# lidq92/LBDRN-MSIC

Measured on AMD Instinct MI355X. Metric: Mpixels/s encode+decode (and bpp/PSNR parity) on D2/K5/bc64/nl2, higher is better.
Workload: dtype f32; 1 GPU; synthetic 8-band 2048x2048 uint16 tile per step, K=5 D=2 bc=64 nl=2 bs=8192 e=10 (BASELINE.json configs[1] by default); encode fit + 16-bit weight truncation + decode; tiles_per_gpu=50, tiles_in_flight_per_gpu=4, tiles_per_launch=2, parallelism=image-sharded x1

## Files before the change

### include/lbdrn_hip.h

```cpp
#ifndef LBDRN_HIP_H
#define LBDRN_HIP_H

#include <stddef.h>
#include <stdint.h>

#ifdef __cplusplus
extern "C" {
#endif
#if defined(__GNUC__)
#pragma GCC visibility push(default)
#endif

#define LBDRN_ABI_VERSION 2

typedef enum lbdrn_status {
    LBDRN_OK = 0,
    LBDRN_E_ARG = -1,
    LBDRN_E_DEVICE = -2,
    LBDRN_E_UNSUPPORTED = -3,
    LBDRN_E_WORKSPACE = -4
} lbdrn_status;

typedef struct lbdrn_geom {
    int32_t C, H, W;
    int32_t K;
    int32_t D;
    int32_t msb_max;
    int32_t use_colors;
    int32_t relative;
    int32_t P;
    int32_t reserved;
    const float *rowtab;
    const float *coltab;
} lbdrn_geom;

typedef struct lbdrn_net {
    int32_t F, bc, C, nl;
    int32_t act;
} lbdrn_net;
enum { LBDRN_ACT_SINE = 0, LBDRN_ACT_RELU = 1 };

const char *lbdrn_last_error(void);
int lbdrn_abi_version(void);
int lbdrn_device_check(void);
int64_t lbdrn_param_count(const lbdrn_net *net);
int32_t lbdrn_feature_dim(const lbdrn_geom *g);

int lbdrn_split_bits(const uint16_t *img, int32_t C, int32_t H, int32_t W, int32_t K,
                     uint16_t *msb, int32_t *msb_max, void *stream);

int lbdrn_labels(const uint16_t *img, int32_t C, int32_t H, int32_t W, int32_t K,
                 const int64_t *idx, int64_t n, float *labels, void *stream);

int lbdrn_features(const lbdrn_geom *g, const uint16_t *msb, const int64_t *idx, int64_t n,
                   float *features, void *stream);

size_t lbdrn_forward_workspace(const lbdrn_net *net, int64_t B);
int lbdrn_forward(const lbdrn_net *net, const float *params, const float *x, int64_t B, float *y,
                  void *workspace, size_t workspace_bytes, void *stream);

size_t lbdrn_tape_bytes(const lbdrn_net *net, int64_t B);
int lbdrn_forward_tape(const lbdrn_net *net, const float *params, const float *x, int64_t B, float *y,
                       void *tape, size_t tape_bytes, void *stream);
size_t lbdrn_backward_workspace(const lbdrn_net *net, int64_t B);
int lbdrn_backward(const lbdrn_net *net, const float *params, const float *x, int64_t B, const void *tape,
                   size_t tape_bytes, const float *y, const float *dy, float *grads, float *dx, void *workspace,
                   size_t workspace_bytes, void *stream);

#define LBDRN_PATH_AUTO 0
#define LBDRN_PATH_GENERIC 1
#define LBDRN_PATH_MFMA 2
size_t lbdrn_apply_workspace(const lbdrn_geom *g, const lbdrn_net *net);
int lbdrn_decode_fused(const lbdrn_geom *g, const lbdrn_net *net, const uint16_t *msb,
                       const float *params, uint16_t *out, float *y_out, void *workspace,
                       size_t workspace_bytes, int32_t path, void *stream);

#define LBDRN_EVAL_BACKGROUND 0x200
#define LBDRN_EVAL_FAST 0x400
#define LBDRN_EVAL_X16 0x1000
int lbdrn_eval_sse(const lbdrn_geom *g, const lbdrn_net *net, const uint16_t *img,
                   const uint16_t *msb, const float *params, double *sse, void *workspace,
                   size_t workspace_bytes, int32_t path, void *stream);

size_t lbdrn_train_workspace(const lbdrn_geom *g, const lbdrn_net *net, int32_t batch_size);
#define LBDRN_TRAIN_ALONE 0x800
int lbdrn_train_prepare(const lbdrn_geom *g, const lbdrn_net *net, const uint16_t *img,
                        const uint16_t *msb, int32_t batch_size, void *workspace,
                        size_t workspace_bytes, int32_t path, void *stream);
int lbdrn_train_epoch(const lbdrn_geom *g, const lbdrn_net *net, const uint16_t *img,
                      const uint16_t *msb, const int64_t *perm, int64_t n, int32_t batch_size,
                      float *params, float *exp_avg, float *exp_avg_sq, int64_t adam_step0,
                      double lr, float *losses, void *workspace, size_t workspace_bytes,
                      int32_t path, void *stream);

int lbdrn_train_group_max(void);
int32_t lbdrn_train_group_size(const lbdrn_geom *g, const lbdrn_net *net);
int32_t lbdrn_train_step_features(const lbdrn_geom *g, const lbdrn_net *net);
int lbdrn_train_epoch_group(int32_t count, const lbdrn_geom *const *g, const lbdrn_net *net,
                            const uint16_t *const *img, const uint16_t *const *msb, const int64_t *const *perm,
                            int64_t n, int32_t batch_size, float *const *params, float *const *exp_avg,
                            float *const *exp_avg_sq, int64_t adam_step0, double lr, float *const *losses,
                            void *const *workspace, size_t workspace_bytes, int32_t path, void *stream);

int lbdrn_train_profile_mode(int32_t mode);

size_t lbdrn_randperm_workspace(int64_t n, int32_t count);
int lbdrn_randperm(const uint64_t *seeds, int32_t count, int64_t n, int64_t *perm, void *workspace,
                   size_t workspace_bytes, void *stream);
int64_t lbdrn_mt19937_jump_poly(int32_t segment, uint32_t *poly624);

size_t lbdrn_plane_bound(int32_t C, int32_t H, int32_t W);
size_t lbdrn_plane_workspace(int32_t C, int32_t H, int32_t W);
int lbdrn_plane_encode(const uint16_t *planes, int32_t C, int32_t H, int32_t W, void *body, size_t body_capacity,
                       uint64_t *body_bytes, void *workspace, size_t workspace_bytes, void *stream);
int lbdrn_plane_decode(const void *body, size_t body_bytes, int32_t C, int32_t H, int32_t W, uint16_t *planes,
                       int32_t *status, void *workspace, size_t workspace_bytes, void *stream);

int64_t lbdrn_jp2k_block_count(int32_t C, int32_t H, int32_t W);
size_t lbdrn_jp2k_bound(int32_t C, int32_t H, int32_t W);
size_t lbdrn_jp2k_workspace(int32_t C, int32_t H, int32_t W);
int lbdrn_jp2k_encode(const uint16_t *planes, int32_t C, int32_t H, int32_t W, int32_t bits, void *out, size_t capacity,
                      size_t *nbytes, void *workspace, size_t workspace_bytes, void *stream);

size_t lbdrn_weights_bound(int64_t n);
int lbdrn_weights_encode(const float *values, int64_t n, int32_t precision, void *out, size_t capacity,
                         size_t *nbytes);
int lbdrn_weights_info(const void *stream, size_t nbytes, int64_t *n, int32_t *precision);
int lbdrn_weights_decode(const void *stream, size_t nbytes, float *values, int64_t capacity);

int lbdrn_train_step(const lbdrn_net *net, const float *x, const float *t, int32_t B,
                     float *params, float *exp_avg, float *exp_avg_sq, int64_t adam_step,
                     double lr, int32_t apply_adam, float *loss, float *grads, void *workspace,
                     size_t workspace_bytes, void *stream);

#if defined(__GNUC__)
#pragma GCC visibility pop
#endif
#ifdef __cplusplus
}
#endif
#endif
```

### lbdrn-msic_amd/csrc/cabi.hip

```cpp
#include <string>

#include "common.hpp"

namespace lbdrn {
const char* last_error();
bool mfma_train_supported(const lbdrn_geom& g, const lbdrn_net& net, int bs = 0);
int mfma_train_step_features(const lbdrn_geom& g, const lbdrn_net& net);
bool mfma_train_takes_groups(const lbdrn_geom& g, const lbdrn_net& net);
size_t mfma_train_workspace(const lbdrn_geom& g, const lbdrn_net& net, int bs);
int mfma_train_prepare(const lbdrn_geom& g, const lbdrn_net& net, const uint16_t* img,
                       const uint16_t* msb, int bs, void* ws, size_t ws_bytes, hipStream_t s);
int mfma_train_epoch(const lbdrn_geom& g, const lbdrn_net& net, const uint16_t* img,
                     const uint16_t* msb, const int64_t* perm, int64_t n, int bs, float* params,
                     float* m, float* v, int64_t step0, double lr, float* losses, void* ws,
                     size_t ws_bytes, hipStream_t s, bool alone);
int train_profile_mode(int mode);
size_t randperm_workspace(int64_t n, int count);
size_t plane_bound(int C, int H, int W);
size_t plane_workspace(int C, int H, int W);
int plane_encode(const uint16_t* planes, int C, int H, int W, void* body, size_t body_cap, uint64_t* body_bytes,
                 void* ws, size_t ws_bytes, hipStream_t s);
int plane_decode(const void* body, size_t body_bytes, int C, int H, int W, uint16_t* planes, int* status, void* ws,
                 size_t ws_bytes, hipStream_t s);
int64_t mt19937_jump_poly(int segment, uint32_t* out);
int randperm_batch(const uint64_t* seeds, int count, int64_t n, int64_t* out, void* ws, size_t ws_bytes,
                   hipStream_t s);
int64_t jp2k_block_count(int C, int H, int W);
size_t jp2k_bound(int C, int H, int W);
size_t jp2k_workspace(int C, int H, int W);
int jp2k_encode(const uint16_t* planes, int C, int H, int W, int bits, uint8_t* out, size_t cap, size_t* nbytes, void* ws,
                size_t ws_bytes, hipStream_t s);
size_t weights_bound(int64_t n);
int weights_encode(const float* values, int64_t n, int precision, uint8_t* out, size_t cap, size_t* nbytes);
int weights_info(const uint8_t* in, size_t nbytes, int64_t* n, int* precision);
int weights_decode(const uint8_t* in, size_t nbytes, float* values, int64_t cap);
}

using namespace lbdrn;

static int device_ok()
{
    static thread_local int cached = 1;
    static thread_local char why[384] = "";
    if (cached < 0) set_error("%s", why);
    if (cached != 1) return cached;
    int n = 0;
    hipError_t e = hipGetDeviceCount(&n);
    if (e != hipSuccess || n < 1) {
        snprintf(why, sizeof(why), "no HIP device available (%s); liblbdrn_hip has no CPU path",
                 e == hipSuccess ? "device count 0" : hipGetErrorString(e));
        set_error("%s", why);
        return cached = LBDRN_E_DEVICE;
    }
    int dev = 0;
    hipDeviceProp_t prop;
    if (hipGetDevice(&dev) != hipSuccess || hipGetDeviceProperties(&prop, dev) != hipSuccess) {
        snprintf(why, sizeof(why), "cannot query the current HIP device");
        set_error("%s", why);
        return cached = LBDRN_E_DEVICE;
    }
    if (std::string(prop.gcnArchName).rfind("gfx950", 0) != 0) {
        snprintf(why, sizeof(why), "device %d is %s; this library is built for gfx950 (MI355X) only", dev, prop.gcnArchName);
        set_error("%s", why);
        return cached = LBDRN_E_DEVICE;
    }
    return cached = 0;
}

#define NEED_DEVICE()                  \
    do {                               \
        if (int rc_ = device_ok()) return rc_; \
    } while (0)

static int net_matches(const lbdrn_geom* g, const lbdrn_net* net)
{
    LBDRN_REQUIRE(net->F == feature_dim(*g), "net.F=%d but the geometry yields %d features", net->F,
                  feature_dim(*g));
    LBDRN_REQUIRE(net->C == g->C, "net.C=%d but the image has %d bands", net->C, g->C);
    LBDRN_REQUIRE(g->msb_max >= 0 && g->msb_max <= 65535, "msb_max=%d out of range", g->msb_max);
    return 0;
}

static int workspace_fits(const char* what, const void* ws, size_t have, size_t need)
{
    if (!ws || have < need) {
        set_error("%s workspace too small: %zu < %zu", what, have, need);
        return LBDRN_E_WORKSPACE;
    }
    return 0;
}

extern "C" {

const char* lbdrn_last_error(void) { return last_error(); }
int lbdrn_abi_version(void) { return LBDRN_ABI_VERSION; }
int lbdrn_device_check(void) { return device_ok(); }

int64_t lbdrn_param_count(const lbdrn_net* net)
{
    if (check_net(net)) return LBDRN_E_ARG;
    return param_count(*net);
}

int32_t lbdrn_feature_dim(const lbdrn_geom* g)
{
    if (!g) return LBDRN_E_ARG;
    return feature_dim(*g);
}

int lbdrn_split_bits(const uint16_t* img, int32_t C, int32_t H, int32_t W, int32_t K, uint16_t* msb,
                     int32_t* msb_max, void* stream)
{
    LBDRN_REQUIRE(img && msb_max, "img and msb_max must not be null");
    LBDRN_REQUIRE(C >= 1 && H >= 1 && W >= 1 && K >= 1 && K <= 15, "bad arguments C=%d H=%d W=%d K=%d", C, H, W, K);
    NEED_DEVICE();
    return generic_split_bits(img, C, H, W, K, msb, msb_max, (hipStream_t)stream);
}

int lbdrn_labels(const uint16_t* img, int32_t C, int32_t H, int32_t W, int32_t K, const int64_t* idx,
                 int64_t n, float* labels, void* stream)
{
    LBDRN_REQUIRE(img && labels, "img and labels must not be null");
    LBDRN_REQUIRE(C >= 1 && H >= 1 && W >= 1 && K >= 1 && K <= 15 && n >= 0, "bad arguments");
    LBDRN_REQUIRE(idx || n <= (int64_t)H * W, "n exceeds the pixel count");
    NEED_DEVICE();
    return generic_labels(img, C, H, W, K, idx, n, labels, (hipStream_t)stream);
}

int lbdrn_features(const lbdrn_geom* g, const uint16_t* msb, const int64_t* idx, int64_t n,
                   float* features, void* stream)
{
    if (int rc = check_geom(g)) return rc;
    LBDRN_REQUIRE(msb && features && n >= 0, "msb/features null or n negative");
    LBDRN_REQUIRE(idx || n <= (int64_t)g->H * g->W, "n exceeds the pixel count");
    NEED_DEVICE();
    return generic_features(*g, msb, idx, n, 0, features, (hipStream_t)stream);
}

size_t lbdrn_forward_workspace(const lbdrn_net* net, int64_t B)
{
    if (check_net(net) || B < 0) return 0;
    return generic_forward_workspace(*net, B);
}

int lbdrn_forward(const lbdrn_net* net, const float* params, const float* x, int64_t B, float* y,
                  void* workspace, size_t workspace_bytes, void* stream)
{
    if (int rc = check_net(net)) return rc;
    LBDRN_REQUIRE(params && x && y && B >= 0, "null pointer or negative batch");
    NEED_DEVICE();
    return generic_forward(*net, params, x, B, y, workspace, workspace_bytes, (hipStream_t)stream);
}

size_t lbdrn_tape_bytes(const lbdrn_net* net, int64_t B)
{
    if (check_net(net) || B < 0) return 0;
    return generic_tape_bytes(*net, B);
}

int lbdrn_forward_tape(const lbdrn_net* net, const float* params, const float* x, int64_t B, float* y, void* tape,
                       size_t tape_bytes, void* stream)
{
    if (int rc = check_net(net)) return rc;
    LBDRN_REQUIRE(params && x && y && B >= 0, "null pointer or negative batch");
    NEED_DEVICE();
    return generic_forward_tape(*net, params, x, B, y, tape, tape_bytes, (hipStream_t)stream);
}

size_t lbdrn_backward_workspace(const lbdrn_net* net, int64_t B)
{
    if (check_net(net) || B < 0) return 0;
    return generic_backward_workspace(*net, B);
}

int lbdrn_backward(const lbdrn_net* net, const float* params, const float* x, int64_t B, const void* tape,
                   size_t tape_bytes, const float* y, const float* dy, float* grads, float* dx, void* workspace,
                   size_t workspace_bytes, void* stream)
{
    if (int rc = check_net(net)) return rc;
    LBDRN_REQUIRE(params && x && y && dy && grads && B >= 0, "null pointer or negative batch");
    NEED_DEVICE();
    return generic_backward(*net, params, x, B, tape, tape_bytes, y, dy, grads, dx, workspace, workspace_bytes,
                            (hipStream_t)stream);
}

size_t lbdrn_apply_workspace(const lbdrn_geom* g, const lbdrn_net* net)
{
    if (check_geom(g) || check_net(net)) return 0;
    size_t a = generic_apply_workspace(*g, *net);
    size_t b = mfma_apply_supported(*g, *net) ? mfma_apply_workspace(*g, *net) : 0;
    return a > b ? a : b;
}

static int pick_apply(const lbdrn_geom* g, const lbdrn_net* net, int32_t path, bool* use_mfma)
{
    const bool ok = mfma_apply_supported(*g, *net);
    if (path == LBDRN_PATH_MFMA && !ok) {
        set_error("fused MFMA apply kernel does not support bc=%d nl=%d C=%d D=%d", net->bc, net->nl,
                  net->C, g->D);
        return LBDRN_E_UNSUPPORTED;
    }
    LBDRN_REQUIRE(path >= LBDRN_PATH_AUTO && path <= LBDRN_PATH_MFMA, "unknown path %d", path);
    *use_mfma = ok && path != LBDRN_PATH_GENERIC;
    return 0;
}

int lbdrn_decode_fused(const lbdrn_geom* g, const lbdrn_net* net, const uint16_t* msb,
                       const float* params, uint16_t* out, float* y_out, void* workspace,
                       size_t workspace_bytes, int32_t path, void* stream)
{
    if (int rc = check_geom(g)) return rc;
    if (int rc = check_net(net)) return rc;
    if (int rc = net_matches(g, net)) return rc;
    LBDRN_REQUIRE(msb && params && out, "msb, params and out must not be null");
    NEED_DEVICE();
    bool use_mfma = false;
    if (int rc = pick_apply(g, net, path, &use_mfma)) return rc;
    if (int rc = workspace_fits("apply", workspace, workspace_bytes, lbdrn_apply_workspace(g, net))) return rc;
    if (use_mfma)
        return mfma_decode(*g, *net, msb, params, out, y_out, workspace, workspace_bytes, (hipStream_t)stream);
    return generic_decode(*g, *net, msb, params, out, y_out, workspace, workspace_bytes, (hipStream_t)stream);
}

int lbdrn_eval_sse(const lbdrn_geom* g, const lbdrn_net* net, const uint16_t* img, const uint16_t* msb,
                   const float* params, double* sse, void* workspace, size_t workspace_bytes,
                   int32_t path, void* stream)
{
    if (int rc = check_geom(g)) return rc;
    if (int rc = check_net(net)) return rc;
    if (int rc = net_matches(g, net)) return rc;
    LBDRN_REQUIRE(img && msb && params && sse, "img, msb, params and sse must not be null");
    NEED_DEVICE();
    const bool background = (path & LBDRN_EVAL_BACKGROUND) != 0, fast = (path & LBDRN_EVAL_FAST) != 0;
    const bool x16 = fast && (path & LBDRN_EVAL_X16) != 0;
    path &= ~(LBDRN_EVAL_BACKGROUND | LBDRN_EVAL_FAST | LBDRN_EVAL_X16);
    bool use_mfma = false;
    if (int rc = pick_apply(g, net, path, &use_mfma)) return rc;
    if (int rc = workspace_fits("apply", workspace, workspace_bytes, lbdrn_apply_workspace(g, net))) return rc;
    if (use_mfma)
        return mfma_eval_sse(*g, *net, img, msb, params, sse, workspace, workspace_bytes, background, fast, x16,
                             (hipStream_t)stream);
    return generic_eval_sse(*g, *net, img, msb, params, sse, workspace, workspace_bytes, (hipStream_t)stream);
}

size_t lbdrn_train_workspace(const lbdrn_geom* g, const lbdrn_net* net, int32_t batch_size)
{
    if (check_geom(g) || check_net(net) || batch_size < 1) return 0;
    size_t a = generic_train_workspace(*net, batch_size);
    size_t b = mfma_train_supported(*g, *net, batch_size) ? mfma_train_workspace(*g, *net, batch_size) : 0;
    return a > b ? a : b;
}

int lbdrn_train_prepare(const lbdrn_geom* g, const lbdrn_net* net, const uint16_t* img,
                        const uint16_t* msb, int32_t batch_size, void* workspace, size_t workspace_bytes,
                        int32_t path, void* stream)
{
    if (int rc = check_geom(g)) return rc;
    if (int rc = check_net(net)) return rc;
    if (int rc = net_matches(g, net)) return rc;
    LBDRN_REQUIRE(img && msb && batch_size >= 1, "null pointer or bad batch size");
    LBDRN_REQUIRE(path >= LBDRN_PATH_AUTO && path <= LBDRN_PATH_MFMA, "unknown path %d", path);
    NEED_DEVICE();
    const bool ok = mfma_train_supported(*g, *net, batch_size);
    if (path == LBDRN_PATH_MFMA && !ok) {
        set_error("fused MFMA train kernel does not support this shape or minibatch size");
        return LBDRN_E_UNSUPPORTED;
    }
    if (int rc = workspace_fits("train", workspace, workspace_bytes, lbdrn_train_workspace(g, net, batch_size))) return rc;
    if (ok && path != LBDRN_PATH_GENERIC)
        return mfma_train_prepare(*g, *net, img, msb, batch_size, workspace, workspace_bytes, (hipStream_t)stream);
    return 0;
}

int lbdrn_train_epoch(const lbdrn_geom* g, const lbdrn_net* net, const uint16_t* img,
                      const uint16_t* msb, const int64_t* perm, int64_t n, int32_t batch_size,
                      float* params, float* exp_avg, float* exp_avg_sq, int64_t adam_step0, double lr,
                      float* losses, void* workspace, size_t workspace_bytes, int32_t path,
                      void* stream)
{
    if (int rc = check_geom(g)) return rc;
    if (int rc = check_net(net)) return rc;
    if (int rc = net_matches(g, net)) return rc;
    LBDRN_REQUIRE(img && msb && perm && params && exp_avg && exp_avg_sq, "null pointer");
    LBDRN_REQUIRE(n >= 0 && batch_size >= 1 && adam_step0 >= 0, "bad n/batch_size/adam_step0");
    NEED_DEVICE();
    const bool alone = (path & LBDRN_TRAIN_ALONE) != 0;
    path &= ~LBDRN_TRAIN_ALONE;
    const bool ok = mfma_train_supported(*g, *net, batch_size);
    if (path == LBDRN_PATH_MFMA && !ok) {
        set_error("fused MFMA train kernel does not support this shape or minibatch size");
        return LBDRN_E_UNSUPPORTED;
    }
    LBDRN_REQUIRE(path >= LBDRN_PATH_AUTO && path <= LBDRN_PATH_MFMA, "unknown path %d", path);
    if (int rc = workspace_fits("train", workspace, workspace_bytes, lbdrn_train_workspace(g, net, batch_size))) return rc;
    if (ok && path != LBDRN_PATH_GENERIC)
        return mfma_train_epoch(*g, *net, img, msb, perm, n, batch_size, params, exp_avg, exp_avg_sq,
                                adam_step0, lr, losses, workspace, workspace_bytes, (hipStream_t)stream, alone);
    return generic_train_epoch(*g, *net, img, msb, perm, n, batch_size, params, exp_avg, exp_avg_sq,
                               adam_step0, lr, losses, workspace, workspace_bytes, (hipStream_t)stream);
}

int lbdrn_train_group_max(void) { return 4; }

int32_t lbdrn_train_group_size(const lbdrn_geom* g, const lbdrn_net* net)
{
    if (!g || !net) return 1;
    return mfma_train_takes_groups(*g, *net) ? lbdrn_train_group_max() : 1;
}

int32_t lbdrn_train_step_features(const lbdrn_geom* g, const lbdrn_net* net)
{
    if (!g || !net) return 0;
    return mfma_train_step_features(*g, *net);
}

int lbdrn_train_epoch_group(int32_t count, const lbdrn_geom* const* g, const lbdrn_net* net, const uint16_t* const* img,
                            const uint16_t* const* msb, const int64_t* const* perm, int64_t n, int32_t batch_size,
                            float* const* params, float* const* exp_avg, float* const* exp_avg_sq, int64_t adam_step0,
                            double lr, float* const* losses, void* const* workspace, size_t workspace_bytes, int32_t path,
                            void* stream)
{
    LBDRN_REQUIRE(count >= 1 && count <= lbdrn_train_group_max(), "group of %d fits (1..%d)", count, lbdrn_train_group_max());
    LBDRN_REQUIRE(g && img && msb && perm && params && exp_avg && exp_avg_sq && workspace, "null pointer array");
    if (int rc = check_net(net)) return rc;
    for (int f = 0; f < count; ++f) {
        LBDRN_REQUIRE(g[f] && img[f] && msb[f] && perm[f] && params[f] && exp_avg[f] && exp_avg_sq[f], "null pointer (fit %d)", f);
        if (int rc = check_geom(g[f])) return rc;
        if (int rc = net_matches(g[f], net)) return rc;
        LBDRN_REQUIRE(g[f]->C == g[0]->C && g[f]->H == g[0]->H && g[f]->W == g[0]->W && g[f]->K == g[0]->K &&
                      g[f]->D == g[0]->D && g[f]->P == g[0]->P && g[f]->use_colors == g[0]->use_colors &&
                      g[f]->relative == g[0]->relative, "the fits of a group must have one shape (fit %d differs)", f);
    }
    LBDRN_REQUIRE(n >= 0 && batch_size >= 1 && adam_step0 >= 0, "bad n/batch_size/adam_step0");
    const int32_t hint = count == 1 ? (path & LBDRN_TRAIN_ALONE) : 0;
    path &= ~LBDRN_TRAIN_ALONE;
    LBDRN_REQUIRE(path >= LBDRN_PATH_AUTO && path <= LBDRN_PATH_MFMA, "unknown path %d", path);
    NEED_DEVICE();
    for (int f = 0; f < count; ++f)
        if (int rc = workspace_fits("train", workspace[f], workspace_bytes, lbdrn_train_workspace(g[f], net, batch_size))) return rc;
    if (count > 1 && path != LBDRN_PATH_GENERIC && mfma_train_supported(*g[0], *net, batch_size)) {
        const int rc = mfma_train_epoch_group(count, *g[0], *net, perm, n, batch_size, params, exp_avg, exp_avg_sq,
                                              adam_step0, lr, losses, workspace, workspace_bytes, (hipStream_t)stream, false);
        if (rc != LBDRN_E_UNSUPPORTED) return rc;
    }
    for (int f = 0; f < count; ++f)
        if (int rc = lbdrn_train_epoch(g[f], net, img[f], msb[f], perm[f], n, batch_size, params[f], exp_avg[f],
                                       exp_avg_sq[f], adam_step0, lr, losses ? losses[f] : nullptr, workspace[f],
                                       workspace_bytes, path | hint, stream))
            return rc;
    return 0;
}

int lbdrn_train_profile_mode(int32_t mode)
{
    LBDRN_REQUIRE(mode >= 0 && mode <= 5, "mode must be 0 .. 5");
    return train_profile_mode(mode);
}

size_t lbdrn_randperm_workspace(int64_t n, int32_t count)
{
    if (n < 0 || count < 1 || count > 32) return 0;
    return randperm_workspace(n, count);
}

int lbdrn_randperm(const uint64_t* seeds, int32_t count, int64_t n, int64_t* perm, void* workspace,
                   size_t workspace_bytes, void* stream)
{
    LBDRN_REQUIRE(n >= 0 && (perm || n == 0), "bad n or null output");
    NEED_DEVICE();
    return randperm_batch(seeds, count, n, perm, workspace, workspace_bytes, (hipStream_t)stream);
}

int64_t lbdrn_mt19937_jump_poly(int32_t segment, uint32_t* poly624)
{
    LBDRN_REQUIRE(poly624, "null output");
    return mt19937_jump_poly(segment, poly624);
}

size_t lbdrn_plane_bound(int32_t C, int32_t H, int32_t W) { return plane_bound(C, H, W); }
size_t lbdrn_plane_workspace(int32_t C, int32_t H, int32_t W) { return plane_workspace(C, H, W); }

int lbdrn_plane_encode(const uint16_t* planes, int32_t C, int32_t H, int32_t W, void* body, size_t body_capacity,
                       uint64_t* body_bytes, void* workspace, size_t workspace_bytes, void* stream)
{
    LBDRN_REQUIRE(C >= 1 && H >= 1 && W >= 1 && C <= 65535, "bad raster geometry");
    NEED_DEVICE();
    return plane_encode(planes, C, H, W, body, body_capacity, body_bytes, workspace, workspace_bytes,
                        (hipStream_t)stream);
}

int lbdrn_plane_decode(const void* body, size_t body_bytes, int32_t C, int32_t H, int32_t W, uint16_t* planes,
                       int32_t* status, void* workspace, size_t workspace_bytes, void* stream)
{
    LBDRN_REQUIRE(C >= 1 && H >= 1 && W >= 1 && C <= 65535, "bad raster geometry");
    NEED_DEVICE();
    return plane_decode(body, body_bytes, C, H, W, planes, status, workspace, workspace_bytes, (hipStream_t)stream);
}

int64_t lbdrn_jp2k_block_count(int32_t C, int32_t H, int32_t W) { return jp2k_block_count(C, H, W); }
size_t lbdrn_jp2k_bound(int32_t C, int32_t H, int32_t W) { return jp2k_bound(C, H, W); }
size_t lbdrn_jp2k_workspace(int32_t C, int32_t H, int32_t W) { return jp2k_workspace(C, H, W); }

int lbdrn_jp2k_encode(const uint16_t* planes, int32_t C, int32_t H, int32_t W, int32_t bits, void* out, size_t capacity,
                      size_t* nbytes, void* workspace, size_t workspace_bytes, void* stream)
{
    if (int rc = device_ok()) return rc;
    return jp2k_encode(planes, C, H, W, bits, (uint8_t*)out, capacity, nbytes, workspace, workspace_bytes, (hipStream_t)stream);
}

size_t lbdrn_weights_bound(int64_t n) { return n < 0 ? 0 : weights_bound(n); }

int lbdrn_weights_encode(const float* values, int64_t n, int32_t precision, void* out, size_t capacity, size_t* nbytes)
{
    LBDRN_REQUIRE((values || n == 0) && out && nbytes && n >= 0 && n < ((int64_t)1 << 32), "null pointer or bad count");
    LBDRN_REQUIRE(precision == 0 || (precision >= 2 && precision <= 32), "precision %d is not 0 or 2..32", precision);
    return weights_encode(values, n, precision, (uint8_t*)out, capacity, nbytes);
}

int lbdrn_weights_info(const void* stream, size_t nbytes, int64_t* n, int32_t* precision)
{
    LBDRN_REQUIRE(stream && n && precision, "null pointer");
    int prec = 0;
    const int rc = weights_info((const uint8_t*)stream, nbytes, n, &prec);
    *precision = prec;
    return rc;
}

int lbdrn_weights_decode(const void* stream, size_t nbytes, float* values, int64_t capacity)
{
    LBDRN_REQUIRE(stream && (values || capacity == 0) && capacity >= 0, "null pointer or bad capacity");
    return weights_decode((const uint8_t*)stream, nbytes, values, capacity);
}

int lbdrn_train_step(const lbdrn_net* net, const float* x, const float* t, int32_t B, float* params,
                     float* exp_avg, float* exp_avg_sq, int64_t adam_step, double lr,
                     int32_t apply_adam, float* loss, float* grads, void* workspace,
                     size_t workspace_bytes, void* stream)
{
    if (int rc = check_net(net)) return rc;
    LBDRN_REQUIRE(x && t && params, "x, t and params must not be null");
    LBDRN_REQUIRE(!apply_adam || (exp_avg && exp_avg_sq && adam_step >= 1), "Adam state missing or adam_step < 1");
    NEED_DEVICE();
    return generic_train_step(*net, x, t, B, params, exp_avg, exp_avg_sq, adam_step, lr, apply_adam,
                              loss, grads, workspace, workspace_bytes, (hipStream_t)stream);
}

}
```

### lbdrn-msic_amd/csrc/train_mfma.hip

```cpp
#include <atomic>
#include <cmath>
#include <cstdlib>
#include <utility>
#include <vector>

#include "common.hpp"
#include "lbdrn_math.hpp"

namespace lbdrn {

typedef float f32x4 __attribute__((ext_vector_type(4)));

constexpr int MAX_GROUP = 4;
constexpr int TB = 32;
constexpr int TBC = 64;
constexpr int HP = 68;
constexpr int TP = 36;
constexpr int OP = 20;
constexpr int RED_SLICES = 8;
constexpr int RED_LANES = 32;
constexpr int SLAB_ROT = 4;
constexpr int TRAIN_THREADS = 512;

constexpr int WB = 64;
constexpr int WAVE_THREADS = 256;
constexpr int WOP = 16;
__host__ __device__ constexpr int wave_xp(int LQ) { return LQ == 16 ? 80 : LQ == 32 ? 144 : LQ == 48 || LQ == 52 ? 208 : 272; }
constexpr int TBC_W = 64;
constexpr int WPT = 68;

struct FeatMap {
    int Fe;
    int zP, zs2, zc;
};
__host__ __device__ __forceinline__ int feat_of_slot(int j, const FeatMap& m)
{
    if (m.zs2 == 0 || j < m.zP) return j;
    const int cj = j - m.zP, c = cj / (m.zs2 - 1), r = cj - c * (m.zs2 - 1);
    return m.zP + c * m.zs2 + r + (r >= m.zc ? 1 : 0);
}
__host__ __device__ __forceinline__ int slot_of_feat(int k, const FeatMap& m)
{
    if (m.zs2 == 0 || k < m.zP) return k;
    const int ck = k - m.zP, c = ck / m.zs2, r = ck - c * m.zs2;
    if (r == m.zc) return -1;
    return m.zP + c * (m.zs2 - 1) + r - (r > m.zc ? 1 : 0);
}

static FeatMap centre_skipping_map(const lbdrn_geom& g, const lbdrn_net& net)
{
    const int side = 2 * g.D + 1;
    if (g.use_colors && g.relative && g.D > 0 && net.F == 2 * g.P + g.C * side * side)
        return FeatMap{net.F - g.C, 2 * g.P, side * side, g.D * side + g.D};
    return FeatMap{net.F, 0, 0, 0};
}

struct TrainPlan {
    FeatMap fm;
    int LQ;
    int XP;
    int NT0;
    int RP;
    int64_t NP;
    int64_t offW[5], offB[5];
    int pk_w0, pk_wh, pk_wl, pack_floats;
    int wave;
    int pk_wht, pk_wlt;
    int w_dp, w_df;
    int wave_lds_floats;
    int sl_hid, sl_out, sl_bias, slab_floats;
    int lds_x, lds_xt, lds_h, lds_ht, lds_z, lds_zt, lds_zo, lds_zot, lds_pix, lds_red, lds_floats;
};

__host__ __device__ constexpr int stream_rp(int LQ);
constexpr int SPLIT_WIDE_LQ = 96;
struct StreamLds;
static int stream_lds_total(int LQ, int NL);

static bool make_train_plan(const lbdrn_geom& g, const lbdrn_net& net, TrainPlan* out)
{
    if ((net.act != LBDRN_ACT_SINE && net.act != LBDRN_ACT_RELU) || net.bc != TBC || net.nl < 1 || net.nl > 3 || net.C > 16 || net.F < 1) return false;
    if (net.act == LBDRN_ACT_RELU && net.nl > 2) return false;
    TrainPlan p;
    p.RP = (net.F + net.C + 3) / 4 * 4;
    p.LQ = 0;
    p.fm = FeatMap{net.F, 0, 0, 0};
    int kind = net.nl <= 2 ? 2 : 0;
    if (kind == 2) {
        p.fm = centre_skipping_map(g, net);
        for (int lq : {16, 24, 32, 48, 52, 64})
            if (p.fm.Fe <= 4 * lq) { p.LQ = lq; break; }
        if (!p.LQ && net.nl == 2 && p.fm.Fe <= 4 * SPLIT_WIDE_LQ) p.LQ = SPLIT_WIDE_LQ;
        if (!p.LQ || (p.LQ != SPLIT_WIDE_LQ && (size_t)stream_lds_total(p.LQ, net.nl) * 4 > 160 * 1024)) { kind = 0; p.LQ = 0; p.fm = FeatMap{net.F, 0, 0, 0}; }
    }
    if (kind != 2 && net.act != LBDRN_ACT_SINE) return false;
    if (kind != 2)
        for (int lq : {16, 32, 52, 64})
            if (net.F <= 4 * lq && p.RP <= 4 * lq + 4) { p.LQ = lq; break; }
    if (!p.LQ) return false;
    p.XP = 4 * p.LQ + 4;
    p.NT0 = p.LQ == SPLIT_WIDE_LQ ? SPLIT_WIDE_LQ / 4 : (p.fm.Fe + 15) / 16;
    if (kind != 2 && 16 * p.NT0 > p.XP) return false;
    p.NP = param_count(net);
    int64_t o = 0;
    for (int l = 0; l < net.nl; ++l) {
        int nin = l ? TBC : net.F;
        p.offW[l] = o; o += (int64_t)TBC * nin;
        p.offB[l] = o; o += TBC;
    }
    p.offW[net.nl] = o; o += (int64_t)net.C * TBC;
    p.offB[net.nl] = o;
    int k = 0;
    p.pk_w0 = k; k += 4 * p.LQ * 64;
    p.pk_wh = k; k += (net.nl - 1) * 4 * 16 * 64;
    p.pk_wl = k; k += 16 * 64;
    p.pk_wht = k; k += (net.nl - 1) * 4 * 16 * 64;
    p.pk_wlt = k; k += 16 * 64;
    p.pack_floats = k;
    p.w_dp = p.w_df = 0;
    p.wave_lds_floats = 0;
    if (kind == 2) {
        p.RP = stream_rp(p.LQ);
        p.wave_lds_floats = p.LQ == SPLIT_WIDE_LQ ? 0 : stream_lds_total(p.LQ, net.nl);
    }
    p.wave = kind;
    int s = 4 * p.NT0 * 256;
    p.sl_hid = s; s += (net.nl - 1) * 16 * 256;
    p.sl_out = s; s += 4 * 256;
    p.sl_bias = s; s += net.nl * TBC + 16;
    p.slab_floats = (s + 127) / 128 * 128;
    int f = 0;
    p.lds_x = f; f += TB * p.XP;
    p.lds_xt = f; f += 16 * p.NT0 * TP;
    p.lds_h = f; f += net.nl * TB * HP;
    p.lds_ht = f; f += net.nl * TBC * TP;
    p.lds_z = f; f += net.nl * TB * HP;
    p.lds_zt = f; f += net.nl * TBC * TP;
    p.lds_zo = f; f += TB * OP;
    p.lds_zot = f; f += 16 * TP;
    p.lds_pix = f; f += TB;
    p.lds_red = f; f += 16;
    p.lds_floats = f;
    if (kind == 0 && (size_t)f * 4 > 160 * 1024) return false;
    *out = p;
    return true;
}

struct WidePlan;
static bool make_wide_plan(const lbdrn_geom& g, const lbdrn_net& net, WidePlan* out);
static bool wide_supported(const lbdrn_geom& g, const lbdrn_net& net);
static size_t wide_workspace(const lbdrn_geom& g, const lbdrn_net& net, int bs);

static bool slabs_addressable(const TrainPlan& p, int bs);

bool mfma_train_supported(const lbdrn_geom& g, const lbdrn_net& net, int bs)
{
    TrainPlan p;
    if (make_train_plan(g, net, &p)) return bs <= 0 || slabs_addressable(p, bs);
    return wide_supported(g, net);
}

bool mfma_train_takes_groups(const lbdrn_geom& g, const lbdrn_net& net)
{
    TrainPlan p;
    return make_train_plan(g, net, &p) && p.wave == 2;
}


struct TrainWsLayout {
    size_t off_rows, off_pack, off_slab, slab_bytes, off_loss, off_stage, stage_bytes, off_map, total;
};

static TrainWsLayout train_ws_layout(const lbdrn_geom& g, const lbdrn_net& net, const TrainPlan& p, int bs)
{
    TrainWsLayout L;
    size_t o = 0;
    L.off_rows = o; o += align_up((size_t)g.H * g.W * p.RP * sizeof(float), 256);
    L.off_pack = o; o += align_up((size_t)p.pack_floats * sizeof(float), 256);
    const size_t nwg = std::max((size_t)(bs + TB - 1) / TB, 2 * ((size_t)(bs + WB - 1) / WB));
    L.slab_bytes = align_up(nwg * (size_t)p.slab_floats * sizeof(float), 256);
    L.off_slab = o; o += SLAB_ROT * L.slab_bytes;
    L.off_loss = o; o += align_up(nwg * sizeof(double), 256);
    L.stage_bytes = align_up(align_up((size_t)bs, WB) * p.RP * sizeof(float), 256);
    L.off_stage = o; o += 2 * L.stage_bytes;
    L.off_map = o; o += align_up((size_t)p.slab_floats * 4 * sizeof(int), 256);
    L.total = o;
    return L;
}

static bool slabs_addressable(const TrainPlan& p, int bs)
{
    const size_t nwg = std::max((size_t)(bs + TB - 1) / TB, 2 * ((size_t)(bs + WB - 1) / WB));
    return nwg * (size_t)p.slab_floats * sizeof(float) < ((size_t)1 << 31);
}

size_t mfma_train_workspace(const lbdrn_geom& g, const lbdrn_net& net, int bs)
{
    TrainPlan p;
    if (!make_train_plan(g, net, &p)) return wide_workspace(g, net, bs);
    return train_ws_layout(g, net, p, bs).total;
}


__device__ __forceinline__ int row_source(int pos, int LQs, int F, int C, const FeatMap& fm)
{
    if (LQs == 0) return pos < fm.Fe ? feat_of_slot(pos, fm) : pos < fm.Fe + C ? F + (pos - fm.Fe) : -1;
    const int g = pos >> 4;
    if (g < (LQs >> 2)) {
        const int j = ((pos >> 2) & 3) * LQs + 4 * g + (pos & 3);
        return j < fm.Fe ? feat_of_slot(j, fm) : -1;
    }
    const int ch = pos - 4 * LQs;
    return ch < C ? F + ch : -1;
}

__global__ void __launch_bounds__(256)
    k_build_rows(lbdrn_geom g, int F, int RP, int LQs, FeatMap fm, const uint16_t* __restrict__ msb,
                 const uint16_t* __restrict__ img, float* __restrict__ rows)
{
    const int64_t HW = (int64_t)g.H * g.W;
    const int64_t e = (int64_t)blockIdx.x * blockDim.x + threadIdx.x;
    if (e >= HW * RP) return;
    const int64_t pix = e / RP;
    const int f = row_source((int)(e - pix * RP), LQs, F, g.C, fm);
    const int y = (int)(pix / g.W), x = (int)(pix - (int64_t)y * g.W);
    float v = 0.0f;
    if (f < 0) {
    } else if (f < g.P) {
        v = g.rowtab[(int64_t)y * g.P + f];
    } else if (f < 2 * g.P) {
        v = g.coltab[(int64_t)x * g.P + (f - g.P)];
    } else if (f < F) {
        const int side = 2 * g.D + 1;
        int cf = f - 2 * g.P;
        int c = cf / (side * side);
        int r = cf - c * side * side;
        int dy = r / side, dx = r - dy * side;
        const uint16_t* pl = msb + (int64_t)c * HW;
        const float mx = (float)g.msb_max;
        int yy = reflect_fast(y + dy - g.D, g.H), xx = reflect_fast(x + dx - g.D, g.W);
        v = (float)pl[(int64_t)yy * g.W + xx] / mx;
        if (g.relative && g.D > 0) v = v - (float)pl[pix] / mx;
    } else if (f < F + g.C) {
        const int mask = (1 << g.K) - 1;
        v = (float)((int)img[(int64_t)(f - F) * HW + pix] & mask) / (float)mask;
    }
    rows[e] = v;
}

constexpr int BR_TW = 32;
__global__ void __launch_bounds__(256)
    k_build_rows_tiled(lbdrn_geom g, int F, int RP, int LQs, FeatMap fm, const uint16_t* __restrict__ msb,
                       const uint16_t* __restrict__ img, float* __restrict__ rows)
{
    extern __shared__ float br_lds[];
    const int side = 2 * g.D + 1, SW = BR_TW + 2 * g.D;
    const int ncolor = F - 2 * g.P;
    float* tile = br_lds;
    int* nbo = reinterpret_cast<int*>(br_lds + g.C * side * SW);
    int* cto = nbo + ncolor;
    const int64_t HW = (int64_t)g.H * g.W;
    const int tiles_x = (g.W + BR_TW - 1) / BR_TW;
    const int y = blockIdx.x / tiles_x, x0 = (blockIdx.x - y * tiles_x) * BR_TW;
    const int tw = min(BR_TW, g.W - x0);
    const int tid = threadIdx.x;
    if (g.use_colors) {
        const float mx = (float)g.msb_max;
        const int total = g.C * side * SW;
        for (int e = tid; e < total; e += 256) {
            const int c = e / (side * SW), r = e - c * side * SW;
            const int sy = r / SW, sx = r - sy * SW;
            const int yy = reflect_fast(y + sy - g.D, g.H), xx = reflect_fast(min(x0 + sx - g.D, g.W - 1 + g.D), g.W);
            tile[e] = (float)msb[(int64_t)c * HW + (int64_t)yy * g.W + xx] / mx;
        }
        for (int k = tid; k < ncolor; k += 256) {
            const int c = k / (side * side), r = k - c * side * side;
            const int dy = r / side, dx = r - dy * side;
            nbo[k] = (c * side + dy) * SW + dx;
            cto[k] = (c * side + g.D) * SW + g.D;
        }
    }
    __syncthreads();
    const bool rel = g.relative && g.D > 0;
    int2* ptab = reinterpret_cast<int2*>(cto + ncolor);
    float* labs = reinterpret_cast<float*>(ptab + RP);
    {
        const int lmask = (1 << g.K) - 1;
        const float lmaskf = (float)lmask;
        for (int e = tid; e < g.C * BR_TW; e += 256) {
            const int c = e / BR_TW, px = e - c * BR_TW;
            labs[e] = (float)((int)img[(int64_t)c * HW + (int64_t)y * g.W + min(x0 + px, g.W - 1)] & lmask) / lmaskf;
        }
    }
    for (int pos = tid; pos < RP; pos += 256) {
        const int f = row_source(pos, LQs, F, g.C, fm);
        int2 t = make_int2(-1, 0);
        if (f < 0) {
        } else if (f < g.P) t = make_int2(-2, f);
        else if (f < 2 * g.P) t = make_int2(-3, f - g.P);
        else if (f < F) t = make_int2(nbo[f - 2 * g.P], rel ? cto[f - 2 * g.P] : -1);
        else if (f < F + g.C) t = make_int2(-4, f - F);
        ptab[pos] = t;
    }
    __syncthreads();
    float* out = rows + ((int64_t)y * g.W + x0) * RP;
    auto value = [&](int pos, int pix) -> float {
        const int2 t = ptab[pos];
        if (t.x >= 0) {
            const float nb = tile[t.x + pix];
            return t.y >= 0 ? nb - tile[t.y + pix] : nb;
        }
        if (t.x == -1) return 0.0f;
        if (t.x == -2) return g.rowtab[(int64_t)y * g.P + t.y];
        if (t.x == -3) return g.coltab[(int64_t)(x0 + pix) * g.P + t.y];
        return labs[t.y * BR_TW + pix];
    };
    if ((RP & 3) == 0) {
        const int RQ = RP >> 2;
        int pix = tid / RQ, pq = tid - pix * RQ;
        const int dp = 256 / RQ, dq = 256 - dp * RQ;
        while (pix < tw) {
            const int pos = 4 * pq;
            const float4 v = make_float4(value(pos, pix), value(pos + 1, pix), value(pos + 2, pix), value(pos + 3, pix));
            *reinterpret_cast<float4*>(out + (int64_t)pix * RP + pos) = v;
            pix += dp;
            pq += dq;
            if (pq >= RQ) { pq -= RQ; pix += 1; }
        }
    } else {
        int pix = tid / RP, pos = tid - pix * RP;
        const int dp = 256 / RP, df = 256 - dp * RP;
        for (int e = tid; pix < tw; e += 256) {
            out[e] = value(pos, pix);
            pix += dp;
            pos += df;
            if (pos >= RP) { pos -= RP; pix += 1; }
        }
    }
}

__device__ __forceinline__ int2 frag_pos(int64_t idx, const TrainPlan& p, int F, int nl, int C)
{
    if (idx < p.offB[0]) {
        int n = (int)(idx / F), k = slot_of_feat((int)(idx - (int64_t)n * F), p.fm);
        if (k < 0) return make_int2(-1, -1);
        int q = k / p.LQ, s = k - q * p.LQ;
        return make_int2(p.pk_w0 + ((((n >> 4) * (p.LQ >> 2) + (s >> 2)) * 64 + q * 16 + (n & 15)) * 4 + (s & 3)), -1);
    }
    for (int l = 1; l < nl; ++l) {
        if (idx >= p.offW[l] && idx < p.offB[l]) {
            int e = (int)(idx - p.offW[l]);
            int n = e >> 6, k = e & 63;
            if (!p.wave) {
                int sq = k & 15;
                return make_int2(p.pk_wh + (((((l - 1) * 4 + (n >> 4)) * 4 + (sq >> 2)) * 64 + (k >> 4) * 16 + (n & 15)) * 4 + (sq & 3)), -1);
            }
            const int fwd = p.pk_wh + (((((l - 1) * 4 + (n >> 4)) * 4 + (k >> 4)) * 64 + ((k >> 2) & 3) * 16 + (n & 15)) * 4 + (k & 3));
            const int bwd = p.pk_wht + (((((l - 1) * 4 + (k >> 4)) * 4 + (n >> 4)) * 64 + ((n >> 2) & 3) * 16 + (k & 15)) * 4 + (n & 3));
            return make_int2(fwd, bwd);
        }
    }
    if (idx >= p.offW[nl] && idx < p.offB[nl]) {
        int e = (int)(idx - p.offW[nl]);
        int c = e >> 6, k = e & 63;
        if (!p.wave) {
            int sq = k & 15;
            return make_int2(p.pk_wl + (((sq >> 2) * 64 + (k >> 4) * 16 + c) * 4 + (sq & 3)), -1);
        }
        const int fwd = p.pk_wl + (((k >> 4) * 64 + ((k >> 2) & 3) * 16 + c) * 4 + (k & 3));
        const int bwd = p.pk_wlt + (((k >> 4) * 64 + (c >> 2) * 16 + (k & 15)) * 4 + (c & 3));
        return make_int2(fwd, bwd);
    }
    return make_int2(-1, -1);
}

__device__ __forceinline__ int64_t slab_to_param(int e, const TrainPlan& p, int F, int nl, int C)
{
    if (e >= p.sl_bias) {
        int b = e - p.sl_bias;
        if (b < nl * TBC) return p.offB[b >> 6] + (b & 63);
        int ch = b - nl * TBC;
        return ch < C ? p.offB[nl] + ch : -1;
    }
    const int tile = e >> 8, lane = (e >> 2) & 63, r = e & 3;
    const int row = 4 * (lane >> 4) + r, col = lane & 15;
    if (e < p.sl_hid) {
        int w = tile / p.NT0, nt = tile - w * p.NT0;
        int k = 16 * nt + col;
        return k < p.fm.Fe ? p.offW[0] + (int64_t)(16 * w + row) * F + feat_of_slot(k, p.fm) : -1;
    }
    if (e < p.sl_out) {
        int t2 = tile - 4 * p.NT0;
        int l = 1 + (t2 >> 4), w = (t2 >> 2) & 3, nt = t2 & 3;
        return p.offW[l] + (int64_t)(16 * w + row) * TBC + 16 * nt + col;
    }
    int w = tile - (p.sl_out >> 8);
    return row < C ? p.offW[nl] + (int64_t)row * TBC + 16 * w + col : -1;
}

__global__ void __launch_bounds__(256)
    k_pack_train(const float* __restrict__ params, TrainPlan p, int F, int nl, int C, float* __restrict__ packed)
{
    int64_t idx = (int64_t)blockIdx.x * blockDim.x + threadIdx.x;
    if (idx >= p.NP) return;
    const int2 pos = frag_pos(idx, p, F, nl, C);
    if (pos.x >= 0) packed[pos.x] = params[idx];
    if (pos.y >= 0) packed[pos.y] = params[idx];
}

__global__ void __launch_bounds__(256)
    k_build_map(TrainPlan p, int F, int nl, int C, int4* __restrict__ map)
{
    int e = blockIdx.x * blockDim.x + threadIdx.x;
    if (e >= p.slab_floats) return;
    int64_t idx = e < p.sl_bias + nl * TBC + 16 ? slab_to_param(e, p, F, nl, C) : -1;
    const int2 pos = idx >= 0 ? frag_pos(idx, p, F, nl, C) : make_int2(-1, -1);
    map[e] = make_int4((int)idx, pos.x, pos.y, 0);
}

constexpr int RED_AUX = 0x00;
#ifdef LBDRN_TIMELINE
constexpr int TL_SLOTS = 2048;
__device__ __forceinline__ void timeline_store(unsigned long long* tl, int slot, bool drain)
{
    if (!tl || slot >= TL_SLOTS) return;
    unsigned long long t;
    if (drain) asm volatile("s_waitcnt vmcnt(0)" ::: "memory");
    asm volatile("s_memrealtime %0\n\ts_waitcnt lgkmcnt(0)" : "=s"(t)::"memory");
    tl[slot] = t;
}
#endif
struct ReduceFit {
    const float* slabs;
    float *params, *m, *v, *packed;
    const double* loss_part;
    float* loss_out;
};
struct ReduceArgs {
    ReduceFit fit[MAX_GROUP];
    unsigned long long* tl;
    int nloss;
};

__global__ void __launch_bounds__(RED_SLICES * RED_LANES)
    k_reduce_adam(ReduceArgs R, int nwg, int slab_floats, const int4* __restrict__ map, float step_size, float bc2_sqrt,
                  double loss_count, int pairs)
{
    __shared__ __attribute__((aligned(16))) float part[RED_SLICES][4 * RED_LANES];
    __builtin_amdgcn_s_setprio(3);
#ifdef LBDRN_TIMELINE
    if (threadIdx.x == 0 && blockIdx.x == 0 && blockIdx.y == 0) timeline_store(R.tl, 1, false);
#endif
    const ReduceFit& F = R.fit[blockIdx.y];
    const float* __restrict__ slabs = F.slabs;
    float* __restrict__ params = F.params;
    float* __restrict__ m = F.m;
    float* __restrict__ v = F.v;
    float* __restrict__ packed = F.packed;
    const int l16 = threadIdx.x % RED_LANES, slice = threadIdx.x / RED_LANES;
    const int base = blockIdx.x * (4 * RED_LANES);
    int4 me = make_int4(-1, -1, -1, 0);
    float pm = 0.f, pv = 0.f, pp = 0.f;
    if (threadIdx.x < 4 * RED_LANES) {
        me = map[base + threadIdx.x];
        const int j = me.x < 0 ? 0 : me.x;
        pm = m[j]; pv = v[j]; pp = params[j];
    }
    const int per = (nwg + RED_SLICES - 1) / RED_SLICES;
    const int w0 = slice * per, w1 = min(nwg, w0 + per);
    float4 acc = make_float4(0.f, 0.f, 0.f, 0.f);
    const __amdgpu_buffer_rsrc_t srs = __builtin_amdgcn_make_buffer_rsrc(const_cast<float*>(slabs), (short)0,
                                                                         (int)((size_t)nwg * (pairs ? 2 : 1) * slab_floats * 4), 0x00020000);
    const int voff = (base + 4 * l16) * 4;
    auto slab4 = [&](int slab) -> float4 {
        typedef int v4i __attribute__((ext_vector_type(4)));
        const v4i x = __builtin_amdgcn_raw_buffer_load_b128(srs, voff + slab * slab_floats * 4, 0, RED_AUX);
        return make_float4(__int_as_float(x[0]), __int_as_float(x[1]), __int_as_float(x[2]), __int_as_float(x[3]));
    };
    int w = w0;
    if (pairs) {
        for (; w + 8 <= w1; w += 8) {
            float4 t[8], o[8];
#pragma unroll
            for (int u = 0; u < 8; ++u) {
                t[u] = slab4(2 * (w + u));
                o[u] = slab4(2 * (w + u) + 1);
            }
#pragma unroll
            for (int u = 0; u < 8; ++u) { acc.x += t[u].x + o[u].x; acc.y += t[u].y + o[u].y; acc.z += t[u].z + o[u].z; acc.w += t[u].w + o[u].w; }
        }
        for (; w < w1; ++w) {
            const float4 t = slab4(2 * w), o = slab4(2 * w + 1);
            acc.x += t.x + o.x; acc.y += t.y + o.y; acc.z += t.z + o.z; acc.w += t.w + o.w;
        }
    }
    for (; w + 16 <= w1; w += 16) {
        float4 t[16];
#pragma unroll
        for (int u = 0; u < 16; ++u) t[u] = slab4(w + u);
#pragma unroll
        for (int u = 0; u < 16; ++u) { acc.x += t[u].x; acc.y += t[u].y; acc.z += t[u].z; acc.w += t[u].w; }
    }
    for (; w < w1; ++w) {
        const float4 t = slab4(w);
        acc.x += t.x; acc.y += t.y; acc.z += t.z; acc.w += t.w;
    }
    *reinterpret_cast<float4*>(&part[slice][4 * l16]) = acc;
    __syncthreads();
    if (threadIdx.x < 4 * RED_LANES && me.x >= 0) {
        float g = part[0][threadIdx.x];
#pragma unroll
        for (int s = 1; s < RED_SLICES; ++s) g += part[s][threadIdx.x];
        const float w1c = (float)(1.0 - 0.9), b2 = 0.999f, w2c = (float)(1.0 - 0.999), eps = 1e-8f;
        float mi = pm + w1c * (g - pm);
        float vi = pv * b2 + w2c * (g * g);
        float denom = __builtin_sqrtf(vi) / bc2_sqrt + eps;
        float pi = pp + (-step_size) * (mi / denom);
        m[me.x] = mi;
        v[me.x] = vi;
        params[me.x] = pi;
        if (me.y >= 0) packed[me.y] = pi;
        if (me.z >= 0) packed[me.z] = pi;
    }
    if (blockIdx.x == 0 && threadIdx.x == 0 && F.loss_out) {
        double s = 0.0;
        if (pairs) for (int k = 0; k + 1 < R.nloss; k += 2) s += F.loss_part[k] + F.loss_part[k + 1];
        else for (int k = 0; k < R.nloss; ++k) s += F.loss_part[k];
        *F.loss_out = (float)(s / loss_count);
    }
#ifdef LBDRN_TIMELINE
    __syncthreads();
    if (threadIdx.x == 0 && blockIdx.y == 0) timeline_store(R.tl, 514 + blockIdx.x, true);
#endif
}

static void launch_reduce(const ReduceArgs& R, int blocks, int count, bool pairs, int nwg, int slab_floats, const int4* map,
                          float step_size, float bc2_sqrt, double loss_count, hipStream_t s)
{
    k_reduce_adam<<<dim3((unsigned)blocks, (unsigned)count), RED_SLICES * RED_LANES, 0, s>>>(R, nwg, slab_floats, map, step_size, bc2_sqrt,
                                                                                            loss_count, pairs ? 1 : 0);
}


struct TrainFit {
    const float* rows;
    const int64_t* perm;
    const float* params;
    const float* packed;
    float* slabs;
    double* loss_part;
};
struct TrainArgs {
    lbdrn_net net;
    TrainPlan p;
    int64_t npix;
    int batch_n;
    float inv;
    TrainFit fit[MAX_GROUP];
    const float* stage_in;
    float* stage_out;
    const int64_t* perm_next;
    int next_n;
    int touch_row_bytes;
    unsigned long long* stamps;
    unsigned long long* tl;
};
constexpr int TOUCH_ROW_BYTES = 256;


#ifdef LBDRN_TRAIN_STAMPS
#define STAMP(k)                                                                        \
    do {                                                                                \
        __builtin_amdgcn_sched_barrier(0);                                              \
        asm volatile("s_memtime %0\n\ts_waitcnt lgkmcnt(0)" : "=s"(stamp[k])::"memory"); \
        __builtin_amdgcn_sched_barrier(0);                                              \
    } while (0)
#else
#define STAMP(k)
#endif

#define MFMA16(a, b, c) __builtin_amdgcn_mfma_f32_16x16x4f32((a), (b), (c), 0, 0, 0)

typedef int v4i32 __attribute__((ext_vector_type(4)));
struct WtBuf {
    __amdgpu_buffer_rsrc_t r;
    float* base;
    __device__ __forceinline__ WtBuf(float* p, size_t bytes) : base(p)
    {
        r = __builtin_amdgcn_make_buffer_rsrc(p, (short)0, (int)bytes, 0x00020000);
    }
    __device__ __forceinline__ void store_plain(int float_off, float a, float b, float c, float d) const
    {
        *reinterpret_cast<float4*>(base + float_off) = make_float4(a, b, c, d);
    }
    __device__ __forceinline__ void store(int float_off, float a, float b, float c, float d) const
    {
        v4i32 v = {__float_as_int(a), __float_as_int(b), __float_as_int(c), __float_as_int(d)};
        __builtin_amdgcn_raw_buffer_store_b128(v, r, float_off * 4, 0, 16 );
    }
};

template <int N>
__device__ __forceinline__ void lds_load(const float* src, float (&dst)[N])
{
#pragma unroll
    for (int g = 0; g < N / 4; ++g) {
        float4 v = *reinterpret_cast<const float4*>(src + 4 * g);
        dst[4 * g] = v.x; dst[4 * g + 1] = v.y; dst[4 * g + 2] = v.z; dst[4 * g + 3] = v.w;
    }
}

template <int LQ, int NL>
__global__ void __launch_bounds__(TRAIN_THREADS, 2) k_train_mfma(TrainArgs A)
{
    extern __shared__ __attribute__((aligned(16))) float lds[];
    const TrainPlan& p = A.p;
    const TrainFit& Ft = A.fit[0];
    const int tid = threadIdx.x, lane = tid & 63, w8 = tid >> 6;
    const int w = w8 & 3, st = w8 >> 2;
    const int i = lane & 15, q = lane >> 4;
    const int C = A.net.C, F = A.net.F;
    constexpr int XP = 4 * LQ + 4;
    float* Xs = lds + p.lds_x;
    float* XT = lds + p.lds_xt;
    float* Hs = lds + p.lds_h;
    float* HT = lds + p.lds_ht;
    float* Zs = lds + p.lds_z;
    float* ZT = lds + p.lds_zt;
    float* Zo = lds + p.lds_zo;
    float* ZoT = lds + p.lds_zot;
    int* pixs = reinterpret_cast<int*>(lds + p.lds_pix);
    double* red = reinterpret_cast<double*>(lds + p.lds_red);
    const int wg = blockIdx.x;
    const int first = wg * TB;
    const int nvalid = min(TB, A.batch_n - first);
    const int srow = i + 16 * st;
    float* slab = Ft.slabs + (size_t)wg * p.slab_floats;
    const WtBuf slabw(slab, (size_t)p.slab_floats * 4);
#ifdef LBDRN_TRAIN_STAMPS
    unsigned long long stamp[16] = {};
    asm volatile("s_memrealtime %0\n\ts_waitcnt lgkmcnt(0)" : "=s"(stamp[12])::"memory");
#endif
    STAMP(0);

    const bool staged = A.stage_in != nullptr;
    int64_t mypix = 0;
    if (!staged && tid < TB) mypix = Ft.perm[first + min(tid, nvalid - 1)];
    const int rs = tid >> 4, rsub = tid & 15;
    constexpr int NLD = (XP / 4 + 15) / 16;
    const int rp4 = p.RP >> 2;
    float4 v[NLD];
    if (staged) {
        const float* src = A.stage_in + ((size_t)wg * TB + rs) * p.RP;
#pragma unroll
        for (int u = 0; u < NLD; ++u) v[u] = *reinterpret_cast<const float4*>(src + 4 * min(rsub + 16 * u, rp4 - 1));
    }
    int64_t nextpix = -1;
    if (A.stage_out && first < A.next_n) nextpix = A.perm_next[min(first + rs, A.next_n - 1)];

    float a0[LQ];
    {
        const float4* wf0 = reinterpret_cast<const float4*>(Ft.packed + p.pk_w0) + (size_t)w * (LQ / 4) * 64 + lane;
#pragma unroll
        for (int g = 0; g < LQ / 4; ++g) {
            const float4 t = wf0[g * 64];
            a0[4 * g] = t.x; a0[4 * g + 1] = t.y; a0[4 * g + 2] = t.z; a0[4 * g + 3] = t.w;
        }
    }
    float ah[NL > 1 ? NL - 1 : 1][16];
#pragma unroll
    for (int l = 1; l < NL; ++l) {
        const float4* wfh = reinterpret_cast<const float4*>(Ft.packed + p.pk_wh) + (size_t)((l - 1) * 4 + w) * 4 * 64 + lane;
#pragma unroll
        for (int g = 0; g < 4; ++g) {
            const float4 t = wfh[g * 64];
            ah[l - 1][4 * g] = t.x; ah[l - 1][4 * g + 1] = t.y; ah[l - 1][4 * g + 2] = t.z; ah[l - 1][4 * g + 3] = t.w;
        }
    }
    float al[16];
    {
        const float4* wfl = reinterpret_cast<const float4*>(Ft.packed + p.pk_wl) + lane;
#pragma unroll
        for (int g = 0; g < 4; ++g) {
            const float4 t = wfl[g * 64];
            al[4 * g] = t.x; al[4 * g + 1] = t.y; al[4 * g + 2] = t.z; al[4 * g + 3] = t.w;
        }
    }
    float atl[4];
#pragma unroll
    for (int s = 0; s < 4; ++s) {
        int ch = 4 * q + s;
        atl[s] = ch < C ? Ft.params[p.offW[NL] + (int64_t)ch * TBC + 16 * w + i] : 0.0f;
    }
    float ath[NL > 1 ? NL - 1 : 1][16];
#pragma unroll
    for (int l = 1; l < NL; ++l)
#pragma unroll
        for (int s = 0; s < 16; ++s) ath[l - 1][s] = Ft.params[p.offW[l] + (int64_t)(16 * q + s) * TBC + 16 * w + i];
    f32x4 bias[NL];
#pragma unroll
    for (int l = 0; l < NL; ++l) {
        float4 b4 = *reinterpret_cast<const float4*>(Ft.params + p.offB[l] + 16 * w + 4 * q);
        bias[l][0] = b4.x; bias[l][1] = b4.y; bias[l][2] = b4.z; bias[l][3] = b4.w;
    }
    f32x4 bias_last;
#pragma unroll
    for (int r = 0; r < 4; ++r) bias_last[r] = (4 * q + r) < C ? Ft.params[p.offB[NL] + 4 * q + r] : 0.0f;

    if (!staged) {
        if (tid < TB) {
            int64_t pix = mypix < 0 ? 0 : (mypix >= A.npix ? A.npix - 1 : mypix);
            pixs[tid] = (int)pix;
        }
        __syncthreads();
    }
    STAMP(1);
    float4 vnext[NLD];
    {
        const int s = rs, sub = rsub;
        float* xr = Xs + s * XP;
        const int nt16 = 16 * p.NT0;
        if (!staged) {
            const float* src = Ft.rows + (size_t)pixs[s] * p.RP;
#pragma unroll
            for (int u = 0; u < NLD; ++u) v[u] = *reinterpret_cast<const float4*>(src + 4 * min(sub + 16 * u, rp4 - 1));
        }
        {
            const int64_t np = nextpix < 0 ? 0 : (nextpix >= A.npix ? A.npix - 1 : nextpix);
            const float* nsrc = Ft.rows + (size_t)np * p.RP;
#pragma unroll
            for (int u = 0; u < NLD; ++u) vnext[u] = *reinterpret_cast<const float4*>(nsrc + 4 * min(sub + 16 * u, rp4 - 1));
        }
#pragma unroll
        for (int u = 0; u < NLD; ++u) {
            const int c4 = sub + 16 * u;
            if (c4 < rp4) {
                *reinterpret_cast<float4*>(xr + 4 * c4) = v[u];
                const float e4[4] = {v[u].x, v[u].y, v[u].z, v[u].w};
#pragma unroll
                for (int e = 0; e < 4; ++e)
                    if (4 * c4 + e < nt16) XT[(4 * c4 + e) * TP + s] = e4[e];
            }
        }
        for (int f = p.RP + sub; f < XP; f += 16) xr[f] = 0.0f;
        for (int f = p.RP + sub; f < nt16; f += 16) XT[f * TP + s] = 0.0f;
    }
    __syncthreads();
    STAMP(2);

    f32x4 acc = bias[0];
    {
        float bx[LQ];
        lds_load<LQ>(Xs + srow * XP + q * LQ, bx);
#pragma unroll
        for (int s = 0; s < LQ; ++s) acc = MFMA16(a0[s], bx[s], acc);
    }
    STAMP(3);
    f32x4 cs[NL];
    auto activate_store = [&](int l) {
        float hv[4];
#pragma unroll
        for (int r = 0; r < 4; ++r) {
            float sn, co;
            canon_sincos(30.0f * acc[r], sn, co);
            hv[r] = sn;
            cs[l][r] = co;
        }
        *reinterpret_cast<float4*>(Hs + (size_t)l * TB * HP + srow * HP + 16 * w + 4 * q) =
            make_float4(hv[0], hv[1], hv[2], hv[3]);
#pragma unroll
        for (int r = 0; r < 4; ++r) HT[(size_t)l * TBC * TP + (16 * w + 4 * q + r) * TP + srow] = hv[r];
    };
    activate_store(0);
    __syncthreads();
    STAMP(4);

#pragma unroll
    for (int l = 1; l < NL; ++l) {
        acc = bias[l];
        float bh[16];
        lds_load<16>(Hs + (size_t)(l - 1) * TB * HP + srow * HP + 16 * q, bh);
#pragma unroll
        for (int s = 0; s < 16; ++s) acc = MFMA16(ah[l - 1][s], bh[s], acc);
        activate_store(l);
        __syncthreads();
    }
    STAMP(5);

    double lsum = 0.0;
    if (w == 0) {
        f32x4 oe = bias_last, oo = {0.f, 0.f, 0.f, 0.f};
        float bo[16];
        lds_load<16>(Hs + (size_t)(NL - 1) * TB * HP + srow * HP + 16 * q, bo);
#pragma unroll
        for (int s = 0; s < 16; s += 2) {
            oe = MFMA16(al[s], bo[s], oe);
            oo = MFMA16(al[s + 1], bo[s + 1], oo);
        }
        const bool live = srow < nvalid;
        const float* labrow = Xs + srow * XP + F + 4 * q;
        float dzo[4];
#pragma unroll
        for (int r = 0; r < 4; ++r) {
            const bool ok = live && (4 * q + r) < C;
            float y = canon_sigmoid(oe[r] + oo[r]);
            float d = y - (ok ? labrow[r] : 0.0f);
            lsum += ok ? (double)(d * d) : 0.0;
            dzo[r] = ok ? ((2.0f * d) * A.inv) * (y * (1.0f - y)) : 0.0f;
        }
        *reinterpret_cast<float4*>(Zo + srow * OP + 4 * q) = make_float4(dzo[0], dzo[1], dzo[2], dzo[3]);
#pragma unroll
        for (int r = 0; r < 4; ++r) ZoT[(4 * q + r) * TP + srow] = dzo[r];
        for (int o = 32; o > 0; o >>= 1) lsum += __shfl_down(lsum, o);
        if (lane == 0) red[st] = lsum;
    }
    __syncthreads();
    if (tid == 0) Ft.loss_part[wg] = red[0] + red[1];
    STAMP(6);
    if (nextpix >= 0) {
        const WtBuf stw(A.stage_out + (size_t)wg * TB * p.RP, (size_t)TB * p.RP * 4);
#pragma unroll
        for (int u = 0; u < NLD; ++u) {
            const int c4 = rsub + 16 * u;
            if (c4 < rp4) stw.store(rs * p.RP + 4 * c4, vnext[u].x, vnext[u].y, vnext[u].z, vnext[u].w);
        }
    }

    auto backprop_store = [&](int l) {
        float dz[4];
#pragma unroll
        for (int r = 0; r < 4; ++r) dz[r] = (acc[r] * cs[l][r]) * 30.0f;
        *reinterpret_cast<float4*>(Zs + (size_t)l * TB * HP + srow * HP + 16 * w + 4 * q) =
            make_float4(dz[0], dz[1], dz[2], dz[3]);
#pragma unroll
        for (int r = 0; r < 4; ++r) ZT[(size_t)l * TBC * TP + (16 * w + 4 * q + r) * TP + srow] = dz[r];
    };

    {
        const f32x4 zero = {0.f, 0.f, 0.f, 0.f};
        acc = zero;
        float bz[4];
        lds_load<4>(Zo + srow * OP + 4 * q, bz);
#pragma unroll
        for (int s = 0; s < 4; ++s) acc = MFMA16(atl[s], bz[s], acc);
        backprop_store(NL - 1);
    }
    __syncthreads();
#pragma unroll
    for (int l = NL - 1; l >= 1; --l) {
        const f32x4 zero = {0.f, 0.f, 0.f, 0.f};
        acc = zero;
        float bz[16];
        lds_load<16>(Zs + (size_t)l * TB * HP + srow * HP + 16 * q, bz);
#pragma unroll
        for (int s = 0; s < 16; ++s) acc = MFMA16(ath[l - 1][s], bz[s], acc);
        backprop_store(l - 1);
        __syncthreads();
    }
    STAMP(7);

    auto grad_tiles = [&](const float* zt, const float* bt, int ntiles, int out, bool early) {
        float az[8];
        lds_load<8>(zt + (16 * w + i) * TP + 8 * q, az);
        for (int nt = st; nt < ntiles; nt += 4) {
            const int nt1 = nt + 2;
            const bool two = nt1 < ntiles;
            float b0[8], b1[8];
            lds_load<8>(bt + (16 * nt + i) * TP + 8 * q, b0);
            lds_load<8>(bt + (16 * (two ? nt1 : nt) + i) * TP + 8 * q, b1);
            const f32x4 zero = {0.f, 0.f, 0.f, 0.f};
            f32x4 g0 = zero, g1 = zero;
#pragma unroll
            for (int s = 0; s < 8; ++s) {
                g0 = MFMA16(az[s], b0[s], g0);
                g1 = MFMA16(az[s], b1[s], g1);
            }
            if (early) {
                slabw.store(out + ((w * ntiles + nt) * 64 + lane) * 4, g0[0], g0[1], g0[2], g0[3]);
                if (two) slabw.store(out + ((w * ntiles + nt1) * 64 + lane) * 4, g1[0], g1[1], g1[2], g1[3]);
            } else {
                slabw.store_plain(out + ((w * ntiles + nt) * 64 + lane) * 4, g0[0], g0[1], g0[2], g0[3]);
                if (two) slabw.store_plain(out + ((w * ntiles + nt1) * 64 + lane) * 4, g1[0], g1[1], g1[2], g1[3]);
            }
        }
    };
    grad_tiles(ZT, XT, p.NT0, 0, true);
    STAMP(10);
#pragma unroll
    for (int l = 1; l < NL; ++l)
        grad_tiles(ZT + (size_t)l * TBC * TP, HT + (size_t)(l - 1) * TBC * TP, 4, p.sl_hid + (l - 1) * 16 * 256, false);
    if (st == 0) {
        float az[8], bv[8];
        lds_load<8>(ZoT + i * TP + 8 * q, az);
        lds_load<8>(HT + (size_t)(NL - 1) * TBC * TP + (16 * w + i) * TP + 8 * q, bv);
        const f32x4 zero = {0.f, 0.f, 0.f, 0.f};
        f32x4 g0 = zero, g1 = zero;
#pragma unroll
        for (int s = 0; s < 8; s += 2) {
            g0 = MFMA16(az[s], bv[s], g0);
            g1 = MFMA16(az[s + 1], bv[s + 1], g1);
        }
        slabw.store_plain(p.sl_out + (w * 64 + lane) * 4, g0[0] + g1[0], g0[1] + g1[1], g0[2] + g1[2], g0[3] + g1[3]);
    }
    STAMP(11);
    for (int u = tid; u < NL * TBC + 16; u += TRAIN_THREADS) {
        float zz[TB];
        lds_load<TB>(u < NL * TBC ? ZT + (size_t)u * TP : ZoT + (size_t)(u - NL * TBC) * TP, zz);
        float v = 0.0f;
#pragma unroll
        for (int s = 0; s < TB; ++s) v += zz[s];
        slab[p.sl_bias + u] = v;
    }
    for (int u = p.sl_bias + NL * TBC + 16 + tid; u < p.slab_floats; u += TRAIN_THREADS) slab[u] = 0.0f;
    STAMP(8);
#ifdef LBDRN_TRAIN_STAMPS
    asm volatile("s_waitcnt vmcnt(0)" ::: "memory");
    STAMP(9);
    asm volatile("s_memrealtime %0\n\ts_waitcnt lgkmcnt(0)" : "=s"(stamp[13])::"memory");
    if (tid == 0 && A.stamps)
        for (int k = 0; k < 16; ++k) A.stamps[(size_t)wg * 16 + k] = stamp[k];
#endif
}

__device__ __forceinline__ float train_sigmoid(float z) { return fast_sigmoid(z); }
template <int ACT> __device__ __forceinline__ void train_act(float z, float& h, float& d);
template <int ACT> __device__ __forceinline__ float train_act_back(float dh, float d)
{
    if constexpr (ACT == LBDRN_ACT_RELU) return d != 0.0f ? dh : 0.0f;
    else return (dh * d) * 30.0f;
}
__device__ __forceinline__ void train_sincos(float x, float& sn, float& cs) { fast_sincos(x, sn, cs); }
template <int ACT> __device__ __forceinline__ void train_act(float z, float& h, float& d)
{
    if constexpr (ACT == LBDRN_ACT_RELU) { h = z > 0.0f ? z : 0.0f; d = z > 0.0f ? 1.0f : 0.0f; }
    else train_sincos(30.0f * z, h, d);
}

__device__ __forceinline__ float row_sum16(float x)
{
    x += __int_as_float(__builtin_amdgcn_update_dpp(0, __float_as_int(x), 0x111, 0xf, 0xf, true));
    x += __int_as_float(__builtin_amdgcn_update_dpp(0, __float_as_int(x), 0x112, 0xf, 0xf, true));
    x += __int_as_float(__builtin_amdgcn_update_dpp(0, __float_as_int(x), 0x114, 0xf, 0xf, true));
    x += __int_as_float(__builtin_amdgcn_update_dpp(0, __float_as_int(x), 0x118, 0xf, 0xf, true));
    return x;
}

__device__ __forceinline__ float wave_sum(float x)
{
    const int xi = __float_as_int(row_sum16(x));
    const float a = __int_as_float(__builtin_amdgcn_readlane(xi, 15)), b = __int_as_float(__builtin_amdgcn_readlane(xi, 31));
    const float c = __int_as_float(__builtin_amdgcn_readlane(xi, 47)), d = __int_as_float(__builtin_amdgcn_readlane(xi, 63));
    return (a + b) + (c + d);
}

template <class K>
static int configure_lds_once(K kern, int bytes, std::atomic<unsigned long long>& configured)
{
    int dev = 0;
    (void)hipGetDevice(&dev);
    const unsigned long long bit = 1ull << (dev & 63);
    if (!(configured.load(std::memory_order_relaxed) & bit)) {
        LBDRN_HIP_TRY(hipFuncSetAttribute(reinterpret_cast<const void*>(kern), hipFuncAttributeMaxDynamicSharedMemorySize, bytes));
        configured.fetch_or(bit, std::memory_order_relaxed);
    }
    return 0;
}

static thread_local int g_prof_mode = 0;
int train_profile_mode(int mode)
{
    g_prof_mode = mode;
    return 0;
}

#include "train_stream.inc"

static int stream_lds_total(int LQ, int NL) { return stream_lds(LQ, NL).total; }

#include "train_split.inc"

#include "train_wide.inc"

int mfma_train_step_features(const lbdrn_geom& g, const lbdrn_net& net)
{
    TrainPlan p;
    if (make_train_plan(g, net, &p)) return p.fm.Fe;
    WidePlan wp;
    return make_wide_plan(g, net, &wp) ? wide_plan_features(wp) : net.F;
}

static bool wide_supported(const lbdrn_geom& g, const lbdrn_net& net)
{
    WidePlan p;
    return make_wide_plan(g, net, &p);
}
static size_t wide_workspace(const lbdrn_geom& g, const lbdrn_net& net, int bs)
{
    WidePlan p;
    if (!make_wide_plan(g, net, &p)) return 0;
    return wide_ws_layout(g, net, p, bs).total;
}


template <int LQ, int NL>
static int launch_train(const TrainArgs& A, int nwg, hipStream_t s)
{
    auto kern = k_train_mfma<LQ, NL>;
    const size_t lds_bytes = (size_t)A.p.lds_floats * 4;
    static std::atomic<unsigned long long> configured{0};
    if (int rc = configure_lds_once(kern, 160 * 1024, configured)) return rc;
    kern<<<nwg, TRAIN_THREADS, lds_bytes, s>>>(A);
    LBDRN_LAUNCH_CHECK();
    return 0;
}

template <int LQ>
static int dispatch_nl(const TrainArgs& A, int nwg, hipStream_t s)
{
    if (A.net.nl == 1) return launch_train<LQ, 1>(A, nwg, s);
    if (A.net.nl == 2) return launch_train<LQ, 2>(A, nwg, s);
    return launch_train<LQ, 3>(A, nwg, s);
}

template <int LQ, int NL, int NT0C, int ACT>
static int launch_stream_act(const TrainArgs& A, int nwg, int count, hipStream_t s)
{
    auto kern = k_train_stream<LQ, NL, STREAM_PD, NT0C, ACT>;
    static std::atomic<unsigned long long> configured{0};
    if (int rc = configure_lds_once(kern, A.p.wave_lds_floats * 4, configured)) return rc;
    kern<<<dim3((unsigned)nwg, (unsigned)count), STREAM_THREADS, (size_t)A.p.wave_lds_floats * 4, s>>>(A);
    LBDRN_LAUNCH_CHECK();
    return 0;
}

template <int LQ, int NL, int NT0C>
static int launch_stream(const TrainArgs& A, int nwg, int count, hipStream_t s)
{
    return A.net.act == LBDRN_ACT_RELU ? launch_stream_act<LQ, NL, NT0C, LBDRN_ACT_RELU>(A, nwg, count, s)
                                       : launch_stream_act<LQ, NL, NT0C, LBDRN_ACT_SINE>(A, nwg, count, s);
}

static int dispatch_stream(const TrainArgs& A, int nwg, int count, hipStream_t s)
{
    const bool one = A.net.nl == 1;
    switch (A.p.LQ) {
        case 16: return one ? launch_stream<16, 1, 0>(A, nwg, count, s) : launch_stream<16, 2, 0>(A, nwg, count, s);
        case 24:
            if (!one && A.p.NT0 == 6) return launch_stream<24, 2, 6>(A, nwg, count, s);
            return one ? launch_stream<24, 1, 0>(A, nwg, count, s) : launch_stream<24, 2, 0>(A, nwg, count, s);
        case 32: return one ? launch_stream<32, 1, 0>(A, nwg, count, s) : launch_stream<32, 2, 0>(A, nwg, count, s);
        case 48:
            if (!one && A.p.NT0 == 12) return launch_stream<48, 2, 12>(A, nwg, count, s);
            return one ? launch_stream<48, 1, 0>(A, nwg, count, s) : launch_stream<48, 2, 0>(A, nwg, count, s);
        case 52:
            if (!one && A.p.NT0 == 13) return launch_stream<52, 2, 13>(A, nwg, count, s);
            return one ? launch_stream<52, 1, 0>(A, nwg, count, s) : launch_stream<52, 2, 0>(A, nwg, count, s);
        default:
            if (!one && A.p.NT0 == 16) return launch_stream<64, 2, 16>(A, nwg, count, s);
            return one ? launch_stream<64, 1, 0>(A, nwg, count, s) : launch_stream<64, 2, 0>(A, nwg, count, s);
    }
}

static bool split_available(const TrainPlan& p, const lbdrn_net& net)
{
    return p.wave == 2 && net.nl == 2 && ((p.LQ == 48 && p.NT0 == 12) || (p.LQ == 64 && p.NT0 == 16) || (p.LQ == 24 && p.NT0 == 6) ||
                                          (p.LQ == SPLIT_WIDE_LQ && p.NT0 == SPLIT_WIDE_LQ / 4));
}
static bool split_only(const TrainPlan& p) { return p.LQ == SPLIT_WIDE_LQ; }

template <int LQ, int NT0C, int ACT>
static int launch_split_act(const TrainArgs& A, int nwg, int count, hipStream_t s)
{
    auto kern = k_train_split<LQ, NT0C, ACT>;
    constexpr int bytes = split_lds(LQ).total * 4;
    static std::atomic<unsigned long long> configured{0};
    if (int rc = configure_lds_once(kern, bytes, configured)) return rc;
    kern<<<dim3((unsigned)nwg, (unsigned)count), WAVE_THREADS, (size_t)bytes, s>>>(A);
    LBDRN_LAUNCH_CHECK();
    return 0;
}

template <int LQ, int NT0C>
static int launch_split(const TrainArgs& A, int nwg, int count, hipStream_t s)
{
    return A.net.act == LBDRN_ACT_RELU ? launch_split_act<LQ, NT0C, LBDRN_ACT_RELU>(A, nwg, count, s)
                                       : launch_split_act<LQ, NT0C, LBDRN_ACT_SINE>(A, nwg, count, s);
}

static int dispatch_split(const TrainArgs& A, int nwg, int count, hipStream_t s)
{
    if (A.p.LQ == SPLIT_WIDE_LQ) return launch_split<SPLIT_WIDE_LQ, SPLIT_WIDE_LQ / 4>(A, nwg, count, s);
    return A.p.LQ == 48 ? launch_split<48, 12>(A, nwg, count, s) : A.p.LQ == 24 ? launch_split<24, 6>(A, nwg, count, s) : launch_split<64, 16>(A, nwg, count, s);
}

static int dispatch_train(const TrainArgs& A, int nwg, int count, hipStream_t s)
{
    if (A.p.wave == 2) return dispatch_stream(A, nwg, count, s);
    switch (A.p.LQ) {
        case 16: return dispatch_nl<16>(A, nwg, s);
        case 32: return dispatch_nl<32>(A, nwg, s);
        case 52: return dispatch_nl<52>(A, nwg, s);
        default: return dispatch_nl<64>(A, nwg, s);
    }
}

int mfma_train_prepare(const lbdrn_geom& g, const lbdrn_net& net, const uint16_t* img,
                       const uint16_t* msb, int bs, void* ws, size_t ws_bytes, hipStream_t s)
{
    TrainPlan p;
    size_t need = 0, off_rows = 0;
    int LQs = 0;
    if (make_train_plan(g, net, &p)) {
        const TrainWsLayout L = train_ws_layout(g, net, p, bs);
        need = L.total; off_rows = L.off_rows;
        if (p.wave == 2) LQs = p.LQ;
    } else {
        WidePlan wp;
        if (!make_wide_plan(g, net, &wp)) {
            set_error("shape not supported by the MFMA train kernels");
            return LBDRN_E_UNSUPPORTED;
        }
        const WideWsLayout L = wide_ws_layout(g, net, wp, bs);
        need = L.total; off_rows = L.off_rows;
        p.RP = wp.RP;
        p.fm = wp.fm;
    }
    if (!ws || ws_bytes < need) {
        set_error("train workspace too small: %zu < %zu", ws_bytes, need);
        return LBDRN_E_WORKSPACE;
    }
    float* rows = (float*)((char*)ws + off_rows);
    const int64_t total = (int64_t)g.H * g.W * p.RP;
    LBDRN_REQUIRE((total + 255) / 256 < ((int64_t)1 << 31), "image too large for one launch");
    const int side = 2 * g.D + 1;
    const size_t ncol = (size_t)std::max(net.F - 2 * g.P, 0);
    const size_t tile_lds = ((size_t)g.C * side * (BR_TW + 2 * g.D) + 2 * ncol + 2 * (size_t)p.RP + (size_t)g.C * BR_TW) * 4;
    const int64_t nblk = (int64_t)g.H * ((g.W + BR_TW - 1) / BR_TW);
    if (tile_lds <= 48 * 1024 && g.D < g.H && g.D < g.W && nblk < ((int64_t)1 << 31)) {
        k_build_rows_tiled<<<(unsigned)nblk, 256, tile_lds, s>>>(g, net.F, p.RP, LQs, p.fm, msb, img, rows);
    } else {
        k_build_rows<<<(unsigned)((total + 255) / 256), 256, 0, s>>>(g, net.F, p.RP, LQs, p.fm, msb, img, rows);
    }
    LBDRN_LAUNCH_CHECK();
    return 0;
}


int mfma_train_epoch_group(int count, const lbdrn_geom& g, const lbdrn_net& net, const int64_t* const* perm, int64_t n,
                           int bs, float* const* params, float* const* m, float* const* v, int64_t step0, double lr,
                           float* const* losses, void* const* ws, size_t ws_bytes, hipStream_t s, bool alone)
{
    TrainArgs A;
    if (!make_train_plan(g, net, &A.p)) {
        if (count != 1) { set_error("groups of fits run on the bc = 64 fused step only"); return LBDRN_E_UNSUPPORTED; }
        return wide_train_epoch(g, net, perm[0], n, bs, params[0], m[0], v[0], step0, lr, losses ? losses[0] : nullptr,
                                ws[0], ws_bytes, s);
    }
    if (count < 1 || count > MAX_GROUP || (count > 1 && A.p.wave != 2)) {
        set_error("a group of %d fits is not supported by this shape's train kernel", count);
        return LBDRN_E_UNSUPPORTED;
    }
    if (!slabs_addressable(A.p, bs)) {
        set_error("minibatch of %d rows: one step's gradient slabs pass 2 GiB, the fused step does not address them", bs);
        return LBDRN_E_UNSUPPORTED;
    }
    const TrainWsLayout L = train_ws_layout(g, net, A.p, bs);
    if (ws_bytes < L.total) {
        set_error("train workspace too small: %zu < %zu", ws_bytes, L.total);
        return LBDRN_E_WORKSPACE;
    }
    A.net = net; A.npix = (int64_t)g.H * g.W;
    ReduceArgs R;
    for (int f = 0; f < MAX_GROUP; ++f) {
        const int k = f < count ? f : 0;
        if (!ws[k]) { set_error("null train workspace"); return LBDRN_E_WORKSPACE; }
        float* packed = (float*)((char*)ws[k] + L.off_pack);
        A.fit[f].rows = (float*)((char*)ws[k] + L.off_rows);
        A.fit[f].params = params[k];
        A.fit[f].packed = packed;
        A.fit[f].slabs = (float*)((char*)ws[k] + L.off_slab);
        A.fit[f].loss_part = (double*)((char*)ws[k] + L.off_loss);
        A.fit[f].perm = perm[k];
        R.fit[f].slabs = A.fit[f].slabs; R.fit[f].params = params[k]; R.fit[f].m = m[k]; R.fit[f].v = v[k];
        R.fit[f].packed = packed; R.fit[f].loss_part = A.fit[f].loss_part; R.fit[f].loss_out = nullptr;
        if (f < count) {
            LBDRN_HIP_TRY(hipMemsetAsync(packed, 0, (size_t)A.p.pack_floats * sizeof(float), s));
            k_pack_train<<<(unsigned)((A.p.NP + 255) / 256), 256, 0, s>>>(params[k], A.p, net.F, net.nl, net.C, packed);
            LBDRN_LAUNCH_CHECK();
        }
    }
    int4* map = (int4*)((char*)ws[0] + L.off_map);
    k_build_map<<<(unsigned)((A.p.slab_floats + 255) / 256), 256, 0, s>>>(A.p, net.F, net.nl, net.C, map);
    LBDRN_LAUNCH_CHECK();
    float* stage[2] = {(float*)((char*)ws[0] + L.off_stage), (float*)((char*)ws[0] + L.off_stage + L.stage_bytes)};
    A.stamps = nullptr;
#ifdef LBDRN_TRAIN_STAMPS
    const int max_wg = (bs + TB - 1) / TB;
    LBDRN_HIP_TRY(hipMalloc(&A.stamps, (size_t)max_wg * 8 * 16 * sizeof(unsigned long long)));
#endif
    A.tl = nullptr; R.tl = nullptr;
#ifdef LBDRN_TIMELINE
    const int tl_steps = (int)((n + bs - 1) / bs);
    unsigned long long* tl_buf = nullptr;
    {
        LBDRN_HIP_TRY(hipMalloc(&tl_buf, (size_t)tl_steps * TL_SLOTS * sizeof(unsigned long long)));
        LBDRN_HIP_TRY(hipMemset(tl_buf, 0, (size_t)tl_steps * TL_SLOTS * sizeof(unsigned long long)));
    }
#endif
    const int rows_per_wg = A.p.wave ? WB : TB;
    const bool split = (alone && count == 1 && split_available(A.p, net)) || split_only(A.p);
    const int red_blocks = A.p.slab_floats / (4 * RED_LANES);
    int64_t step = step0;
    int si = 0;
    for (int64_t first = 0; first < n; first += bs, ++si) {
        const int B = (int)std::min<int64_t>(bs, n - first);
        const int nwg = (B + rows_per_wg - 1) / rows_per_wg;
        for (int f = 0; f < MAX_GROUP; ++f) {
            const int k = f < count ? f : 0;
            A.fit[f].perm = perm[k] + first;
            R.fit[f].loss_out = (f < count && losses && losses[k]) ? losses[k] + si : nullptr;
        }
        A.batch_n = B;
        for (int f = 0; f < MAX_GROUP; ++f) {
            const int k = f < count ? f : 0;
            A.fit[f].slabs = (float*)((char*)ws[k] + L.off_slab + (size_t)(si % SLAB_ROT) * L.slab_bytes);
            R.fit[f].slabs = A.fit[f].slabs;
        }
#ifdef LBDRN_TIMELINE
        A.tl = tl_buf + (size_t)TL_SLOTS * si; R.tl = A.tl;
#endif
        A.inv = 1.0f / ((float)B * (float)net.C);
        const int64_t nextB = std::max<int64_t>(0, std::min<int64_t>(bs, n - first - bs));
        A.stage_in = si > 0 ? stage[si & 1] : nullptr;
        A.stage_out = nextB > 0 ? stage[(si + 1) & 1] : nullptr;
        if (A.p.wave) A.stage_in = nullptr, A.stage_out = nullptr;
        A.perm_next = perm[0] + first + bs;
        A.next_n = (int)nextB;
        A.touch_row_bytes = (alone && count == 1) ? TOUCH_ROW_BYTES : 0;
        const bool split_now = split && (B >= 2 || split_only(A.p));
        auto train_launch = [&]() { return split_now ? dispatch_split(A, 2 * nwg, count, s) : dispatch_train(A, nwg, count, s); };
        if (int rc = train_launch()) return rc;
        if (g_prof_mode == 2)
            if (int rc = train_launch()) return rc;
        ++step;
        const double bc1 = 1.0 - std::pow(0.9, (double)step), bc2 = 1.0 - std::pow(0.999, (double)step);
        R.nloss = split_now ? 2 * nwg : nwg;
        if (g_prof_mode != 3 && g_prof_mode != 4)
                launch_reduce(R, red_blocks, count, split_now, nwg, A.p.slab_floats, map, (float)(lr / bc1), (float)std::sqrt(bc2), (double)B * net.C, s);
        if (g_prof_mode == 1) {
            ReduceArgs R0 = R;
            for (int f = 0; f < MAX_GROUP; ++f) R0.fit[f].loss_out = nullptr;
            launch_reduce(R0, red_blocks, count, split_now, nwg, A.p.slab_floats, map, 0.0f, (float)std::sqrt(bc2), (double)B * net.C, s);
        }
        LBDRN_LAUNCH_CHECK();
    }
#ifdef LBDRN_TIMELINE
    {
        LBDRN_HIP_TRY(hipStreamSynchronize(s));
        std::vector<unsigned long long> h((size_t)tl_steps * TL_SLOTS);
        LBDRN_HIP_TRY(hipMemcpy(h.data(), tl_buf, h.size() * sizeof(unsigned long long), hipMemcpyDeviceToHost));
        (void)hipFree(tl_buf);
        double tr = 0, g1 = 0, rd = 0, g2 = 0; int cnt = 0;
        auto last = [&](int k, int lo, int hi) { unsigned long long m = 0; for (int j = lo; j < hi; ++j) m = std::max(m, h[(size_t)k * TL_SLOTS + j]); return m; };
        for (int k = 8; k + 1 < tl_steps; ++k) {
            const unsigned long long ts = h[(size_t)k * TL_SLOTS], rs = h[(size_t)k * TL_SLOTS + 1], te = last(k, 2, 514), re = last(k, 514, TL_SLOTS);
            const unsigned long long ts2 = h[(size_t)(k + 1) * TL_SLOTS];
            tr += (double)(te - ts); g1 += (double)((long long)(rs - te)); rd += (double)(re - rs); g2 += (double)((long long)(ts2 - re));
            ++cnt;
        }
        const double u = 0.01 / std::max(cnt, 1);
        fprintf(stderr, "[lbdrn timeline] per step over %d steps: train first start -> last end %.2f us | -> reduce starts %.2f | reduce %.2f | -> next train starts %.2f | step %.2f us\n",
                cnt, tr * u, g1 * u, rd * u, g2 * u, (tr + g1 + rd + g2) * u);
    }
#endif
#ifdef LBDRN_TRAIN_STAMPS
    if (A.p.wave) {
        LBDRN_HIP_TRY(hipStreamSynchronize(s));
        const int nw = ((int)std::min<int64_t>(bs, n) + rows_per_wg - 1) / rows_per_wg * 4 * (A.p.wave == 2 ? count : 1) * (split ? 2 : 1);
        std::vector<unsigned long long> h((size_t)nw * 16);
        LBDRN_HIP_TRY(hipMemcpy(h.data(), A.stamps, h.size() * sizeof(unsigned long long), hipMemcpyDeviceToHost));
        (void)hipFree(A.stamps);
        double d[14] = {}, clk = 0, span = 0;
        unsigned long long t0min = ~0ull, t1max = 0;
        for (int k = 0; k < nw; ++k) {
            for (int j = 1; j <= 13; ++j) d[j] += (double)(h[k * 16 + j] - h[k * 16 + j - 1]);
            clk += (double)(h[k * 16 + 13] - h[k * 16 + 0]) / (double)(h[k * 16 + 15] - h[k * 16 + 14]) * 100.0;
            span += (double)(h[k * 16 + 13] - h[k * 16 + 0]);
            t0min = std::min(t0min, h[k * 16 + 14]);
            t1max = std::max(t1max, h[k * 16 + 15]);
        }
        if (split)
            fprintf(stderr, "[lbdrn stamps, split kernel] clock %.0f MHz; wave lifetime %.0f cycles; first start -> last end %.2f us; "
                            "mean cycles: requests out %.0f | layer 0 (waits for W0 and the rows in it) %.0f | act0 %.0f | barrier, h0 read %.0f | hidden + act1 %.0f | "
                            "barrier, h1 read %.0f | out + loss %.0f | dh1, dz1 parked %.0f | barrier, dh0, dz0 parked %.0f | barrier, gradient operands read %.0f | "
                            "gradient products, stores, bias sums %.0f | drain %.0f\n",
                    clk / nw, span / nw, (double)(t1max - t0min) / 100.0, d[1] / nw, d[2] / nw, d[3] / nw, d[4] / nw, d[5] / nw, d[6] / nw,
                    d[7] / nw, d[8] / nw, d[9] / nw, d[10] / nw, (d[11] + d[12]) / nw, d[13] / nw);
        else
        fprintf(stderr, A.p.wave == 2 ?
                        "[lbdrn stamps, stream kernel] clock %.0f MHz; wave lifetime %.0f cycles; first start -> last end %.2f us; "
                        "mean cycles: indices + first requests out %.0f | first stage landed %.0f | layer 0 under the stream %.0f | all landed, barrier %.0f | "
                        "act0 %.0f | hidden+act %.0f | out+loss %.0f | backward %.0f | barrier 3 %.0f | dW0 strips %.0f | dW tail+hidden %.0f | "
                        "bias sums %.0f | drain %.0f\n" :
                        "[lbdrn stamps, wave kernel] clock %.0f MHz; wave lifetime %.0f cycles; first start -> last end %.2f us; "
                        "mean cycles: W0 DMA + rows->LDS %.0f | barrier 1 %.0f | small-matrix requests + layer0 %.0f | barrier 2 %.0f | "
                        "act0 %.0f | hidden+act %.0f | out+loss %.0f | backward %.0f | barrier 3 %.0f | dW0 strips %.0f | dW tail+hidden %.0f | "
                        "bias sums %.0f | drain %.0f\n",
                clk / nw, span / nw, (double)(t1max - t0min) / 100.0, d[1] / nw, d[2] / nw, d[3] / nw, d[4] / nw, d[5] / nw, d[6] / nw,
                d[7] / nw, d[8] / nw, d[9] / nw, d[10] / nw, d[11] / nw, d[12] / nw, d[13] / nw);
    } else {
        LBDRN_HIP_TRY(hipStreamSynchronize(s));
        std::vector<unsigned long long> h((size_t)max_wg * 16);
        LBDRN_HIP_TRY(hipMemcpy(h.data(), A.stamps, h.size() * sizeof(unsigned long long), hipMemcpyDeviceToHost));
        (void)hipFree(A.stamps);
        double sum[12] = {}, d10 = 0, d11 = 0, d8 = 0, clk = 0;
        for (int wq = 0; wq < max_wg; ++wq) {
            for (int k = 1; k < 10; ++k)
                if (k != 8) sum[k] += (double)(h[wq * 16 + k] - h[wq * 16 + (k == 9 ? 8 : k - 1)]);
            d10 += (double)(h[wq * 16 + 10] - h[wq * 16 + 7]);
            d11 += (double)(h[wq * 16 + 11] - h[wq * 16 + 10]);
            d8 += (double)(h[wq * 16 + 8] - h[wq * 16 + 11]);
            clk += (double)(h[wq * 16 + 9] - h[wq * 16 + 0]) / (double)(h[wq * 16 + 13] - h[wq * 16 + 12]) * 100.0;
        }
        fprintf(stderr, "[lbdrn stamps] in-kernel clock %.0f MHz; mean cycles/phase: perm %.0f rows %.0f L0 %.0f act0 %.0f "
                        "hidden %.0f out+loss %.0f backprop %.0f dW0 %.0f dWhid+out %.0f bias %.0f drain %.0f\n",
                clk / max_wg, sum[1] / max_wg, sum[2] / max_wg, sum[3] / max_wg, sum[4] / max_wg, sum[5] / max_wg,
                sum[6] / max_wg, sum[7] / max_wg, d10 / max_wg, d11 / max_wg, d8 / max_wg, sum[9] / max_wg);
    }
#endif
    return 0;
}

int mfma_train_epoch(const lbdrn_geom& g, const lbdrn_net& net, const uint16_t* img,
                     const uint16_t* msb, const int64_t* perm, int64_t n, int bs, float* params,
                     float* m, float* v, int64_t step0, double lr, float* losses, void* ws,
                     size_t ws_bytes, hipStream_t s, bool alone)
{
    return mfma_train_epoch_group(1, g, net, &perm, n, bs, &params, &m, &v, step0, lr, &losses, &ws, ws_bytes, s, alone);
}

}
```

### lbdrn-msic_amd/csrc/train_split.inc

```
constexpr int SPB = 32;
constexpr int SP_HP = 68;
constexpr int SP_OP = 20;
constexpr int SP_PT = 36;
constexpr int SP_SM = 40;

constexpr int SP_RING = 12;
__host__ __device__ constexpr bool split_ring(int LQ) { return LQ > 64; }
__host__ __device__ constexpr int split_w0_groups(int LQ) { return split_ring(LQ) ? SP_RING : LQ / 4; }
__host__ __device__ constexpr int split_small_through(int k, int SPI) { return k * SPI < SP_SM / 4 ? k * SPI : SP_SM / 4; }

struct SplitLds { int w0, sm, x, xt, h0, red, idx, bias, h1, e, zo, zt, total; };
__host__ __device__ constexpr SplitLds split_lds(int LQ)
{
    SplitLds L{};
    const int G0 = LQ / 4, RG = split_w0_groups(LQ);
    int o = 0;
    const int over = 2 * SPB * SP_HP + SPB * SP_OP + 2 * 64 * SP_PT;
    L.w0 = o; o += RG * 4 * 256 > over ? RG * 4 * 256 : over;
    L.sm = o; o += SP_SM * 256;
    L.xt = (G0 + 1) * SGP + 16;
    L.x = o; o += 2 * L.xt;
    L.h0 = o; o += SPB * SP_HP;
    L.red = o; o += 4 + 4 * 16 + 12;
    L.idx = o; o += 4 * 256;
    L.bias = o; o += 4 * 64;
    L.total = o;
    int a = L.w0;
    L.h1 = a; a += SPB * SP_HP;
    L.e = a; a += SPB * SP_HP;
    L.zo = a; a += SPB * SP_OP;
    L.zt = a; a += 2 * 64 * SP_PT;
    if (a > L.sm) L.total = -1;
    return L;
}

__device__ __forceinline__ float split_sum8(float x)
{
    x += __int_as_float(__builtin_amdgcn_update_dpp(0, __float_as_int(x), 0x111, 0xf, 0xf, true));
    x += __int_as_float(__builtin_amdgcn_update_dpp(0, __float_as_int(x), 0x112, 0xf, 0xf, true));
    x += __int_as_float(__builtin_amdgcn_update_dpp(0, __float_as_int(x), 0x118, 0xf, 0xf, true));
    return x;
}
__host__ __device__ constexpr int split_slot(int r) { return (r & ~5) | ((r & 1) << 2) | ((r >> 2) & 1); }

__host__ __device__ constexpr int split_row_requests(int lo, int hi, int u)
{
    int c = 0;
    for (int g = lo; g < hi; ++g) c += (g & 1) == u;
    return c;
}

template <int LQ, int NT0C, int ACT>
__global__ void __launch_bounds__(WAVE_THREADS, 1) k_train_split(TrainArgs A)
{
    extern __shared__ __attribute__((aligned(16))) float lds[];
    const TrainPlan& p = A.p;
    const TrainFit& F = A.fit[blockIdx.y];
    constexpr int NL = 2, G0 = LQ / 4, NGR = G0 + 1, HP = SP_HP, OP = SP_OP, PT = SP_PT, RPM = stream_rp(LQ);
    constexpr SplitLds L = split_lds(LQ);
    static_assert(L.total > 0 && L.total * 4 <= 160 * 1024, "LDS map does not fit");
    static_assert(16 * NT0C == 4 * LQ && G0 >= 4, "the first layer's strips fill its slots");
    constexpr int NFS = NT0C / 4, REM = NT0C % 4, NIT = NFS + REM, GA = split_w0_groups(LQ) / 2;
    static_assert(NFS >= 1 && REM <= 2, "strip counts of the shapes this is instantiated for");
    constexpr int SPI = (SP_SM / 4 + G0 - 2) / (G0 - 1);
    constexpr bool RING = split_ring(LQ);
    constexpr int RG = split_w0_groups(LQ), HR = RG / 2, W0B = RG - GA;
    static_assert(!RING || (G0 == 2 * RG && GA == HR), "the ring holds half of W_0, its quarters land one behind the other");
    const int tid = threadIdx.x, lane = tid & 63;
    const int wv = __builtin_amdgcn_readfirstlane(tid >> 6);
    const int st = wv >> 1, uh = wv & 1;
    const int i = lane & 15, q = lane >> 4;
    const int C = A.net.C;
    const float* W0s = lds + L.w0;
    const float* SMs = lds + L.sm;
    const float* Xs = lds + L.x;
    float* H0 = lds + L.h0;
    float* H1 = lds + L.h1;
    float* E = lds + L.e;
    float* Zo = lds + L.zo;
    float* ZT = lds + L.zt;
    float* red = lds + L.red;
    const unsigned lds0 = (unsigned)(size_t)(__attribute__((address_space(3))) void*)lds;
    const int wg = blockIdx.x, grp = wg >> 1, par = wg & 1;
    const int qb = (i >> 2) & 1, jr = (i & 3) + 4 * (i >> 3);
    const int rho = 16 * (2 * st + qb) + 2 * jr + par;
    const int grow = grp * WB + rho;
    const bool live = grow < A.batch_n;
    const int srow = 16 * st + i;
    const int sig = 8 * (2 * st + qb) + jr;
    const int t0 = 2 * uh;
    float* slab = F.slabs + (size_t)wg * p.slab_floats;
    const WtBuf slabw(slab, (size_t)p.slab_floats * 4);
#ifdef LBDRN_TRAIN_STAMPS
    unsigned long long stamp[16] = {};
    asm volatile("s_memrealtime %0\n\ts_waitcnt lgkmcnt(0)" : "=s"(stamp[14])::"memory");
#endif
#ifdef LBDRN_TIMELINE
    if (lane == 0 && wv == 0 && wg == 0 && blockIdx.y == 0) timeline_store(A.tl, 0, false);
#endif
    STAMP(0);

    {
        const void* a0 = F.perm; const void* a1 = F.params; const void* a2 = F.packed; const void* a3 = F.rows;
        int b0 = p.pk_w0, b1 = p.pk_wh, b2 = p.pk_wht, b3 = p.pk_wl, b4 = p.pk_wlt, b5 = A.batch_n;
        long long c0 = p.offB[0], c1 = p.offB[1], c2 = p.offB[2], c3 = A.npix;
        asm volatile("" ::"s"(a0), "s"(a1), "s"(a2), "s"(a3), "s"(b0), "s"(b1), "s"(b2), "s"(b3), "s"(b4), "s"(b5), "s"(c0), "s"(c1), "s"(c2), "s"(c3));
    }
    if constexpr (RING) {
        const int64_t* isrc = F.perm + min(grp * WB + lane, A.batch_n - 1);
        stream_dma_dword(reinterpret_cast<const float*>(isrc), lds0 + 4u * (unsigned)(L.idx + 256 * wv));
    } else {
        const int64_t* isrc = F.perm + min(grp * WB + 2 * (lane & 31), A.batch_n - 2);
        stream_dma(reinterpret_cast<const float*>(isrc), lds0 + 4u * (unsigned)(L.idx + 256 * wv));
    }
    {
        const int l = wv < 3 ? wv : 2, n = l < 2 ? 64 : C;
        const float* bsrc = F.params + p.offB[l] + min(lane, n - 1);
        stream_dma_dword(bsrc, lds0 + 4u * (unsigned)(L.bias + 64 * wv));
    }
    const float* fsrc = F.packed + lane * 4;
    auto w0_requests = [&](int g_lo, int g_hi) {
#pragma unroll
        for (int g = g_lo; g < g_hi; ++g)
            stream_dma(fsrc + p.pk_w0 + 256 * (wv * G0 + g), lds0 + 4u * (unsigned)(L.w0 + ((g % RG) * 4 + wv) * 256));
    };
    w0_requests(0, GA);
    stream_wait_vm<GA + 1>();
    int64_t raw;
    if constexpr (RING) {
        raw = reinterpret_cast<const int*>(lds + L.idx + 256 * wv)[min(grow, A.batch_n - 1) - grp * WB];
    } else {
        const int g = min(grow, A.batch_n - 1), l = (g - grp * WB) >> 1;
        const int pos = 2 * l + (g - min(grp * WB + 2 * l, A.batch_n - 2));
        raw = reinterpret_cast<const int64_t*>(lds + L.idx + 256 * wv)[pos];
    }
    const int pix = (int)(raw < 0 ? 0 : (raw >= A.npix ? A.npix - 1 : raw));
    const float* rsrc = F.rows + (size_t)__shfl(pix, 16 * q + split_slot(lane >> 2)) * RPM + 4 * (lane & 3);
    auto row_requests = [&](int g_lo, int g_hi) {
#pragma unroll
        for (int g = g_lo; g < g_hi; ++g)
            if ((g & 1) == uh) stream_dma(rsrc + 16 * g, lds0 + 4u * (unsigned)(L.x + st * L.xt + g * SGP));
    };
    row_requests(0, GA);
    w0_requests(GA, RG);
    row_requests(GA, NGR);
    auto small_request = [&](int b) {
        const int blk = 4 * b + wv;
        const int src = blk < 16 ? p.pk_wh + 256 * blk : blk < 32 ? p.pk_wht + 256 * (blk - 16) : blk < 36 ? p.pk_wl + 256 * (blk - 32) : p.pk_wlt + 256 * (blk - 36);
        stream_dma(fsrc + src, lds0 + 4u * (unsigned)(L.sm + 256 * blk));
    };
    long long touched = 0;
    if (A.next_n > 0 && wv == 0 && lane < 8) touched = F.perm[A.batch_n + min(grp * WB + 8 * lane, A.next_n - 1)];
    STAMP(1);
    constexpr int ROWS_B0 = split_row_requests(GA, NGR, 0), ROWS_B1 = split_row_requests(GA, NGR, 1);
    if (uh == 0) stream_wait_vm<W0B + ROWS_B0>(); else stream_wait_vm<W0B + ROWS_B1>();
    stream_barrier();
    STAMP(2);

    auto sel4 = [](const float4& x, int e) -> float { return e == 0 ? x.x : e == 1 ? x.y : e == 2 ? x.z : x.w; };
    f32x4 bias0[2], bias1[2], bias_last;
    {
        const float* B = lds + L.bias;
#pragma unroll
        for (int tt = 0; tt < 2; ++tt) {
            const float4 b4 = *reinterpret_cast<const float4*>(B + 16 * (t0 + tt) + 4 * q);
            const float4 c4 = *reinterpret_cast<const float4*>(B + 64 + 16 * (t0 + tt) + 4 * q);
            bias0[tt][0] = b4.x; bias0[tt][1] = b4.y; bias0[tt][2] = b4.z; bias0[tt][3] = b4.w;
            bias1[tt][0] = c4.x; bias1[tt][1] = c4.y; bias1[tt][2] = c4.z; bias1[tt][3] = c4.w;
        }
        const float4 l4 = *reinterpret_cast<const float4*>(B + 128 + 4 * q);
        bias_last[0] = 4 * q + 0 < C ? l4.x : 0.0f; bias_last[1] = 4 * q + 1 < C ? l4.y : 0.0f;
        bias_last[2] = 4 * q + 2 < C ? l4.z : 0.0f; bias_last[3] = 4 * q + 3 < C ? l4.w : 0.0f;
    }
    f32x4 acc[2] = {bias0[0], bias0[1]};
    {
        const float* wbase = W0s + t0 * 256 + lane * 4;
        const float* xbase = Xs + st * L.xt + (4 * split_slot(i) + q) * 4;
        float4 aq[2][2], bq[2];
        auto reads = [&](int g) {
            aq[g & 1][0] = *reinterpret_cast<const float4*>(wbase + (g % RG) * 1024);
            aq[g & 1][1] = *reinterpret_cast<const float4*>(wbase + (g % RG) * 1024 + 256);
            bq[g & 1] = *reinterpret_cast<const float4*>(xbase + g * SGP);
        };
        auto mfmas = [&](int g) {
#pragma unroll
            for (int e = 0; e < 4; ++e)
#pragma unroll
                for (int tt = 0; tt < 2; ++tt) acc[tt] = MFMA16(sel4(aq[g & 1][tt], e), sel4(bq[g & 1], e), acc[tt]);
        };
        reads(0);
#pragma unroll
        for (int g = 1; g < G0; ++g) {
            if (g == GA) {
                stream_wait_vm<((GA - 1) * SPI < SP_SM / 4 ? (GA - 1) * SPI : SP_SM / 4)>();
                stream_barrier();
            }
            if constexpr (RING) {
                if (g == GA + 1 || g == 2 * HR + 1) {
                    asm volatile("s_waitcnt lgkmcnt(0)" ::: "memory");
                    stream_barrier();
                    const int q0 = g == GA + 1 ? 2 * HR : 3 * HR;
                    w0_requests(q0, q0 + HR);
                }
                if (g == 2 * HR) {
                    stream_wait_vm<split_small_through(2 * HR - 1, SPI) - split_small_through(GA, SPI)>();
                    stream_barrier();
                }
                if (g == 3 * HR) {
                    stream_wait_vm<split_small_through(3 * HR - 1, SPI) - split_small_through(2 * HR, SPI)>();
                    stream_barrier();
                }
            }
#pragma unroll
            for (int b = (g - 1) * SPI; b < g * SPI; ++b)
                if (b < SP_SM / 4) small_request(b);
            reads(g);
            mfmas(g - 1);
#pragma unroll
            for (int k = 0; k < 3; ++k) {
                __builtin_amdgcn_sched_group_barrier(0x100, 1, 0);
                __builtin_amdgcn_sched_group_barrier(0x008, 2, 0);
            }
            __builtin_amdgcn_sched_group_barrier(0x008, 2, 0);
            __builtin_amdgcn_sched_barrier(0);
        }
        mfmas(G0 - 1);
        __builtin_amdgcn_sched_barrier(0);
    }
    const float4 lab = *reinterpret_cast<const float4*>(Xs + st * L.xt + G0 * SGP + (4 * split_slot(i) + q) * 4);
    STAMP(3);
    float hf[4][4];
    f32x4 cs[NL][2];
    auto activate = [&](int l, float* H) {
#pragma unroll
        for (int tt = 0; tt < 2; ++tt) {
            float sn[4];
#pragma unroll
            for (int r = 0; r < 4; ++r) {
                float co;
                train_act<ACT>(acc[tt][r], sn[r], co);
                cs[l][tt][r] = co;
            }
            *reinterpret_cast<float4*>(H + srow * HP + 16 * (t0 + tt) + 4 * q) = make_float4(sn[0], sn[1], sn[2], sn[3]);
        }
    };
    auto all_units = [&](const float* H, float (&dst)[4][4]) {
#pragma unroll
        for (int t = 0; t < 4; ++t) {
            const float4 x = *reinterpret_cast<const float4*>(H + srow * HP + 16 * t + 4 * q);
            dst[t][0] = x.x; dst[t][1] = x.y; dst[t][2] = x.z; dst[t][3] = x.w;
        }
    };
    auto small = [&](int blk) -> float4 { return *reinterpret_cast<const float4*>(SMs + 256 * blk + lane * 4); };
    activate(0, H0);
    stream_wait_vm<0>();
    __syncthreads();
    all_units(H0, hf);
    float4 wh[2][4];
#pragma unroll
    for (int tt = 0; tt < 2; ++tt)
#pragma unroll
        for (int tk = 0; tk < 4; ++tk) wh[tt][tk] = small((t0 + tt) * 4 + tk);
    STAMP(4);

    acc[0] = bias1[0]; acc[1] = bias1[1];
#pragma unroll
    for (int tk = 0; tk < 4; ++tk)
#pragma unroll
        for (int r = 0; r < 4; ++r)
#pragma unroll
            for (int tt = 0; tt < 2; ++tt) acc[tt] = MFMA16(sel4(wh[tt][tk], r), hf[tk][r], acc[tt]);
    float4 wl[4], wlt[2];
#pragma unroll
    for (int tk = 0; tk < 4; ++tk) wl[tk] = small(32 + tk);
#pragma unroll
    for (int tt = 0; tt < 2; ++tt) wlt[tt] = small(36 + t0 + tt);
    activate(1, H1);
    STAMP(5);
    __syncthreads();
    all_units(H1, hf);
    STAMP(6);

    float dzo[4];
    {
        f32x4 oe = bias_last, oo = {0.f, 0.f, 0.f, 0.f};
#pragma unroll
        for (int tk = 0; tk < 4; ++tk) {
            const float4 x = wl[tk];
            oe = MFMA16(x.x, hf[tk][0], oe);
            oo = MFMA16(x.y, hf[tk][1], oo);
            oe = MFMA16(x.z, hf[tk][2], oe);
            oo = MFMA16(x.w, hf[tk][3], oo);
        }
        const float labv[4] = {lab.x, lab.y, lab.z, lab.w};
        float lsum = 0.0f;
#pragma unroll
        for (int r = 0; r < 4; ++r) {
            const bool ok = live && (4 * q + r) < C;
            const float y = train_sigmoid(oe[r] + oo[r]);
            const float d = y - ((4 * q + r) < C ? labv[r] : 0.0f);
            lsum += ok ? d * d : 0.0f;
            dzo[r] = ok ? ((2.0f * d) * A.inv) * (y * (1.0f - y)) : 0.0f;
        }
        if (uh == 0) {
            *reinterpret_cast<float4*>(Zo + srow * OP + 4 * q) = make_float4(dzo[0], dzo[1], dzo[2], dzo[3]);
            const int li = __float_as_int(split_sum8(lsum));
            auto rl = [&](int l) { return __int_as_float(__builtin_amdgcn_readlane(li, l)); };
            const float l0 = (rl(11) + rl(27)) + (rl(43) + rl(59)), l1 = (rl(15) + rl(31)) + (rl(47) + rl(63));
            if (lane == 0) { red[2 * st] = l0; red[2 * st + 1] = l1; }
            float bs[4];
#pragma unroll
            for (int r = 0; r < 4; ++r) bs[r] = split_sum8(dzo[r]);
            if (i == 11 || i == 15)
                *reinterpret_cast<float4*>(red + 4 + 16 * (2 * st + (i == 15)) + 4 * q) = make_float4(bs[0], bs[1], bs[2], bs[3]);
        }
    }
    STAMP(7);

    float dzf[4][4], dzm[2][4];
    auto backprop = [&](int l) {
#pragma unroll
        for (int tt = 0; tt < 2; ++tt)
#pragma unroll
            for (int r = 0; r < 4; ++r) {
                dzm[tt][r] = train_act_back<ACT>(acc[tt][r], cs[l][tt][r]);
                ZT[(size_t)l * 64 * PT + (16 * (t0 + tt) + 4 * q + r) * PT + sig] = dzm[tt][r];
            }
    };
    float4 wht[2][4];
    {
        const f32x4 zero = {0.f, 0.f, 0.f, 0.f};
        acc[0] = zero; acc[1] = zero;
#pragma unroll
        for (int s4 = 0; s4 < 4; ++s4)
#pragma unroll
            for (int tt = 0; tt < 2; ++tt) acc[tt] = MFMA16(sel4(wlt[tt], s4), dzo[s4], acc[tt]);
#pragma unroll
        for (int tt = 0; tt < 2; ++tt)
#pragma unroll
            for (int to = 0; to < 4; ++to) wht[tt][to] = small(16 + (t0 + tt) * 4 + to);
        backprop(1);
#pragma unroll
        for (int tt = 0; tt < 2; ++tt)
            *reinterpret_cast<float4*>(E + srow * HP + 16 * (t0 + tt) + 4 * q) = make_float4(dzm[tt][0], dzm[tt][1], dzm[tt][2], dzm[tt][3]);
    }
    STAMP(8);
    __syncthreads();
    all_units(E, dzf);
    __builtin_amdgcn_sched_barrier(0);

    const int w = wv;
    const int rq = 16 * (q >> 1) + 4 * (q & 1);
    auto ldcol = [&](const float* base, int pitch, float (&dst)[8]) {
#pragma unroll
        for (int j = 0; j < 8; ++j) dst[j] = base[(rq + (j & 3) + 8 * (j >> 2)) * pitch];
    };
    auto ldx = [&](int nt, float (&dst)[8]) {
        const int f = 16 * nt + i;
        const int kq = f / LQ, fl = f - kq * LQ;
        const float* base = Xs + (q >> 1) * L.xt + (fl >> 2) * SGP + kq * 4 + (fl & 3);
#pragma unroll
        for (int j = 0; j < 8; ++j) dst[j] = base[16 * split_slot(4 * (q & 1) + (j & 3) + 8 * (j >> 2))];
    };
    auto ldrow8 = [&](const float* row, float (&dst)[8]) {
#pragma unroll
        for (int g = 0; g < 2; ++g) {
            const float4 x = *reinterpret_cast<const float4*>(row + 4 * g);
            dst[4 * g] = x.x; dst[4 * g + 1] = x.y; dst[4 * g + 2] = x.z; dst[4 * g + 3] = x.w;
        }
    };
    auto put = [&](int off, const f32x4& g) {
        slabw.store(off + lane * 4, g[0], g[1], g[2], g[3]);
    };
    const f32x4 zero4 = {0.f, 0.f, 0.f, 0.f};
    const float* ZT1 = ZT + 64 * PT;
    float az[4][8], a1[4][8], azw[8], a1w[8], ao[8], bo[8], bh[8], bb[NFS][8], br[REM > 0 ? REM : 1][8];
    auto item = [&](auto n_) {
        constexpr int n = decltype(n_)::value;
        if constexpr (n < NFS) ldx(w + 4 * n, bb[n]);
        else if constexpr (n < NIT) ldx(4 * NFS + (n - NFS), br[n - NFS]);
    };
#pragma unroll
    for (int t = 0; t < 4; ++t) ldrow8(ZT1 + (16 * t + i) * PT + 8 * q, a1[t]);
    ldrow8(ZT1 + (16 * w + i) * PT + 8 * q, a1w);
    ldcol(Zo + i, OP, ao);
    ldcol(H1 + 16 * w + i, HP, bo);
    ldcol(H0 + 16 * w + i, HP, bh);
    item(std::integral_constant<int, 0>{});
    {
        acc[0] = zero4; acc[1] = zero4;
#pragma unroll
        for (int to = 0; to < 4; ++to)
#pragma unroll
            for (int r = 0; r < 4; ++r)
#pragma unroll
                for (int tt = 0; tt < 2; ++tt) acc[tt] = MFMA16(sel4(wht[tt][to], r), dzf[to][r], acc[tt]);
        stream_deal<32, 32, 0>();
        backprop(0);
    }
    STAMP(9);
    __syncthreads();
    if (tid == 0) F.loss_part[wg] = ((double)red[0] + (double)red[1]) + ((double)red[2] + (double)red[3]);
    STAMP(10);
#pragma unroll
    for (int t = 0; t < 4; ++t) ldrow8(ZT + (16 * t + i) * PT + 8 * q, az[t]);
    ldrow8(ZT + (16 * w + i) * PT + 8 * q, azw);
    item(std::integral_constant<int, 1>{});
    f32x4 go = zero4, g1[4] = {zero4, zero4, zero4, zero4};
#pragma unroll
    for (int j = 0; j < 8; ++j) {
        go = MFMA16(ao[j], bo[j], go);
#pragma unroll
        for (int t = 0; t < 4; ++t) g1[t] = MFMA16(a1[t][j], bh[j], g1[t]);
    }
    stream_deal<40, (NIT > 1 ? 18 : 10), 0>();
    f32x4 gs[2][4];
    stream_for<NFS>([&](auto k_) {
        constexpr int k = decltype(k_)::value;
#pragma unroll
        for (int t = 0; t < 4; ++t) gs[k & 1][t] = zero4;
        item(std::integral_constant<int, k + 2>{});
#pragma unroll
        for (int j = 0; j < 8; ++j)
#pragma unroll
            for (int t = 0; t < 4; ++t) gs[k & 1][t] = MFMA16(az[t][j], bb[k][j], gs[k & 1][t]);
        if constexpr (k == 0) {
            put(p.sl_out + w * 256, go);
#pragma unroll
            for (int t = 0; t < 4; ++t) put(p.sl_hid + (t * 4 + w) * 256, g1[t]);
            stream_deal<32, (k + 2 < NIT ? 8 : 0), 5>();
        } else {
#pragma unroll
            for (int t = 0; t < 4; ++t) put((t * NT0C + w + 4 * (k - 1)) * 256, gs[(k - 1) & 1][t]);
            stream_deal<32, (k + 2 < NIT ? 8 : 0), 4>();
        }
    });
    if constexpr (REM > 0) {
        f32x4 grem[REM];
#pragma unroll
        for (int r = 0; r < REM; ++r) grem[r] = zero4;
#pragma unroll
        for (int j = 0; j < 8; ++j)
#pragma unroll
            for (int r = 0; r < REM; ++r) grem[r] = MFMA16(azw[j], br[r][j], grem[r]);
#pragma unroll
        for (int t = 0; t < 4; ++t) put((t * NT0C + w + 4 * (NFS - 1)) * 256, gs[(NFS - 1) & 1][t]);
        stream_deal<REM * 8, 0, 4>();
#pragma unroll
        for (int r = 0; r < REM; ++r) put((w * NT0C + 4 * NFS + r) * 256, grem[r]);
    } else {
#pragma unroll
        for (int t = 0; t < 4; ++t) put((t * NT0C + w + 4 * (NFS - 1)) * 256, gs[(NFS - 1) & 1][t]);
    }
    {
        float s0 = 0.f, s1 = 0.f;
#pragma unroll
        for (int j = 0; j < 8; ++j) { s0 += azw[j]; s1 += a1w[j]; }
        s0 += __shfl_xor(s0, 16); s1 += __shfl_xor(s1, 16);
        s0 += __shfl_xor(s0, 32); s1 += __shfl_xor(s1, 32);
        if (lane < 16) {
            slab[p.sl_bias + 16 * w + lane] = s0;
            slab[p.sl_bias + TBC_W + 16 * w + lane] = s1;
        }
    }
    if (w == 3 && lane < 16)
        slab[p.sl_bias + NL * TBC_W + lane] = (red[4 + lane] + red[20 + lane]) + (red[36 + lane] + red[52 + lane]);
    asm volatile("" ::"v"(touched));
    STAMP(11); STAMP(12);
#ifdef LBDRN_TIMELINE
    if (lane == 0 && uh == 0 && blockIdx.y == 0) timeline_store(A.tl, 2 + 2 * wg + st, true);
#endif
#ifdef LBDRN_TRAIN_STAMPS
    asm volatile("s_waitcnt vmcnt(0)" ::: "memory");
    STAMP(13);
    asm volatile("s_memrealtime %0\n\ts_waitcnt lgkmcnt(0)" : "=s"(stamp[15])::"memory");
    if (lane == 0 && A.stamps)
        for (int k = 0; k < 16; ++k) A.stamps[(((size_t)blockIdx.y * gridDim.x + wg) * 4 + wv) * 16 + k] = stamp[k];
#endif
}
```

### lbdrn-msic_amd/csrc/train_stream.inc

```
constexpr int SGP = 260;
__host__ __device__ constexpr int stream_groups(int LQ) { return LQ / 4 + 1; }
__host__ __device__ constexpr int stream_rp(int LQ) { return 16 * stream_groups(LQ); }
__host__ __device__ constexpr int stream_wpx(int LQ)
{
    const int n = stream_groups(LQ) * SGP;
    return n + ((16 - n % 32) + 32) % 32;
}
constexpr int SHP = 68, SOP = 20;
constexpr int SHSZ = WB * SHP + 48;
constexpr int SZOSZ = WB * SOP + 48;
constexpr int SZTSZ = TBC_W * WPT;

constexpr int SRED = 8 + 2 * 64;
struct StreamLds { int x, stage, h0, red, h1, zo, zt, wh, wht, idx, total, small; };
__host__ __device__ constexpr StreamLds stream_lds(int LQ, int NL)
{
    StreamLds L{};
    const int G0 = LQ / 4, NST = (G0 + 2) / 2;
    L.x = 0;
    L.stage = 4 * stream_wpx(LQ);
    const int stage_end = L.stage + 4 * G0 * 256;
    const bool alias = 2 * (NST - 1) - 1 >= (SHSZ + SRED + 1023) / 1024 - 1;
    int r = alias ? L.stage + ((SHSZ + SRED + 3) & ~3) : L.stage;
    L.h1 = r; r += (NL - 1) * SHSZ;
    L.zo = r; r += SZOSZ;
    L.zt = r; r += NL * SZTSZ;
    const int small_floats = (NL - 1) * 16 * 256;
    int total = r > stage_end ? r : stage_end;
    L.small = 0;
    if (NL > 1) {
        const int wht = r > stage_end + small_floats ? r : stage_end + small_floats;
        const int h0_extra = alias ? 0 : SHSZ + SRED;
        if ((wht + small_floats + h0_extra) * 4 <= 160 * 1024) {
            L.small = 1;
            L.wh = stage_end;
            L.wht = wht;
            total = wht + small_floats;
        }
    }
    if (alias) { L.h0 = L.stage; L.red = L.stage + SHSZ; }
    else { L.h0 = total; L.red = total + SHSZ; total += SHSZ + SRED; }
    L.idx = total; total += 256;
    L.total = total;
    return L;
}

__host__ __device__ constexpr int stream_row_cnt(int LQ, int s)
{
    int c = 0;
    for (int g = 2 * s; g < 2 * s + 2; ++g) c += g < LQ / 4 + 1;
    return c;
}
__host__ __device__ constexpr int stream_frag_cnt(int LQ, int s)
{
    int c = 0;
    for (int g = 2 * s; g < 2 * s + 2; ++g) c += g < LQ / 4;
    return c;
}
__host__ __device__ constexpr int stream_small_batch(int LQ, int NL, int PD, int k)
{
    const int NST = (LQ / 4 + 2) / 2;
    if (!stream_lds(LQ, NL).small || k + PD < NST) return 0;
    const int nsw = (NL - 1) * 32, per = (nsw + PD - 1) / PD, done = per * (k + PD - NST);
    return done >= nsw ? 0 : (nsw - done < per ? nsw - done : per);
}
__host__ __device__ constexpr int stream_vg(int LQ, int NL, int k)
{
    const int NST = (LQ / 4 + 2) / 2;
    if (stream_lds(LQ, NL).small) return k == NST - 1 ? 8 : 0;
    const int nv = (NL - 1) * 32 + 8;
    const int per = (nv + NST - 1) / NST, done = per * k;
    return done >= nv ? 0 : (nv - done < per ? nv - done : per);
}
__host__ __device__ constexpr int stream_allow(int LQ, int NL, int PD, int s)
{
    const int NST = (LQ / 4 + 2) / 2;
    int total = 0, last = 0;
    for (int k = 0; k < PD && k < NST; ++k) { total += 4 * stream_frag_cnt(LQ, k); if (k == s) last = total; }
    for (int k = 0; k < PD && k < NST; ++k) { total += 4 * stream_row_cnt(LQ, k); if (k == s) last = total; }
    for (int it = 0; it < s; ++it) {
        if (it + PD < NST) {
            total += 4 * stream_row_cnt(LQ, it + PD) + 4 * stream_frag_cnt(LQ, it + PD);
            if (it + PD == s) last = total;
        } else {
            total += stream_small_batch(LQ, NL, PD, it);
        }
    }
    return total - last;
}

template <int N>
__device__ __forceinline__ void stream_wait_vm()
{
    static_assert(N >= 0 && N < 64, "vmcnt is a 6-bit counter");
    asm volatile("s_waitcnt vmcnt(%0)" ::"n"(N) : "memory");
}
__device__ __forceinline__ void stream_barrier() { asm volatile("s_barrier" ::: "memory"); }
#pragma clang diagnostic push
#pragma clang diagnostic ignored "-Winline-asm"
__device__ __forceinline__ void stream_dma(const float* g, unsigned lds_byte)
{
    asm volatile("s_mov_b32 m0, %0\n\tglobal_load_lds_dwordx4 %1, off" ::"s"(lds_byte), "v"(g) : "memory", "m0");
}
__device__ __forceinline__ void stream_dma_dword(const float* g, unsigned lds_byte)
{
    asm volatile("s_mov_b32 m0, %0\n\tglobal_load_lds_dword %1, off" ::"s"(lds_byte), "v"(g) : "memory", "m0");
}
#pragma clang diagnostic pop
template <int... Is, class F>
__device__ __forceinline__ void stream_for_impl(std::integer_sequence<int, Is...>, F&& f)
{
    (f(std::integral_constant<int, Is>{}), ...);
}
template <int N, class F>
__device__ __forceinline__ void stream_for(F&& f)
{
    stream_for_impl(std::make_integer_sequence<int, N>{}, f);
}

constexpr int TAIL_PLAIN = 1;
constexpr int STREAM_PD = 3;

constexpr int STREAM_THREADS = WAVE_THREADS + 64;

#ifdef LBDRN_STAMP_DW
#define SE(k) do { if ((k) == 9) STAMP(0); } while (0)
#define SD(k) STAMP(k)
#else
#define SE(k) STAMP(k)
#define SD(k)
#endif

template <int M, int R, int S>
__device__ __forceinline__ void stream_deal()
{
    constexpr int RR = R < M ? R : M;
#pragma unroll
    for (int k = 0; k < RR; ++k) {
        __builtin_amdgcn_sched_group_barrier(0x008, 1, 0);
        __builtin_amdgcn_sched_group_barrier(0x100, 1, 0);
    }
    constexpr int left = M - RR, per = S > 0 ? (left / (S + 1) > 0 ? left / (S + 1) : 1) : 0;
#pragma unroll
    for (int k = 0; k < S; ++k) {
        __builtin_amdgcn_sched_group_barrier(0x008, per, 0);
        __builtin_amdgcn_sched_group_barrier(0x040, 1, 0);
    }
    if constexpr (left - S * per > 0) __builtin_amdgcn_sched_group_barrier(0x008, left - S * per, 0);
    __builtin_amdgcn_sched_barrier(0);
}

__device__ __forceinline__ float stream_sum8(float x)
{
    x += __int_as_float(__builtin_amdgcn_update_dpp(0, __float_as_int(x), 0x112, 0xf, 0xf, true));
    x += __int_as_float(__builtin_amdgcn_update_dpp(0, __float_as_int(x), 0x114, 0xf, 0xf, true));
    x += __int_as_float(__builtin_amdgcn_update_dpp(0, __float_as_int(x), 0x118, 0xf, 0xf, true));
    return x;
}
__device__ __forceinline__ f32x4 stream_join(const f32x4& even, const f32x4& odd)
{
    f32x4 g = {even[0] + odd[0], even[1] + odd[1], even[2] + odd[2], even[3] + odd[3]};
    return g;
}

template <int LQ, int NL, int PD, int NT0C, int ACT>
__global__ void __launch_bounds__(STREAM_THREADS, 1) k_train_stream(TrainArgs A)
{
    extern __shared__ __attribute__((aligned(16))) float lds[];
    const TrainPlan& p = A.p;
    const TrainFit& F = A.fit[blockIdx.y];
    constexpr int G0 = LQ / 4, NGR = G0 + 1, NST = (NGR + 1) / 2, WPX = stream_wpx(LQ), RPM = stream_rp(LQ);
    constexpr int HP = SHP, OP = SOP, PT = WPT;
    constexpr StreamLds L = stream_lds(LQ, NL);
    constexpr bool SMALL = L.small != 0;
    constexpr int NH = (NL - 1) * 16;
    static_assert(L.total * 4 <= 160 * 1024, "LDS map does not fit");
    const int tid = threadIdx.x, lane = tid & 63;
    const int w = __builtin_amdgcn_readfirstlane(tid >> 6);
    const int i = lane & 15, q = lane >> 4;
    const int C = A.net.C;
    float* Xs = lds + L.x;
    const float* ST = lds + L.stage;
    float* H0 = lds + L.h0;
    float* red = lds + L.red;
    float* ZT = lds + L.zt;
    float* Zo = lds + L.zo;
    auto Hl = [&](int l) -> float* { return l == 0 ? H0 : lds + L.h1 + (size_t)(l - 1) * SHSZ; };
    const unsigned lds0 = (unsigned)(size_t)(__attribute__((address_space(3))) void*)lds;
    const int wg = blockIdx.x, first = wg * WB;
    const int nvalid = min(WB, A.batch_n - first);
    const int srow = 16 * w + i;
    float* slab = F.slabs + (size_t)wg * p.slab_floats;
    const WtBuf slabw(slab, (size_t)p.slab_floats * 4);
    if (w == 4) {
        const float* fsrc = F.packed + p.pk_w0 + lane * 4;
        auto issue_frags = [&](int s) {
#pragma unroll
            for (int g = 2 * s; g < 2 * s + 2; ++g)
                if (g < G0)
#pragma unroll
                    for (int t = 0; t < 4; ++t) stream_dma(fsrc + 256 * (t * G0 + g), lds0 + 4u * (unsigned)(L.stage + (g * 4 + t) * 256));
        };
        if (A.batch_n >= 2) {
            const int64_t* isrc = F.perm + min(first + 2 * (lane & 31), A.batch_n - 2);
            stream_dma(reinterpret_cast<const float*>(isrc), lds0 + 4u * (unsigned)L.idx);
        } else {
            stream_dma_dword(reinterpret_cast<const float*>(F.perm) + (lane & 1), lds0 + 4u * (unsigned)L.idx);
        }
        stream_for<PD>([&](auto s_) { if (decltype(s_)::value < NST) issue_frags(decltype(s_)::value); });
        {
            constexpr int up = 4 * (stream_frag_cnt(LQ, 0) + (PD > 1 ? stream_frag_cnt(LQ, 1) : 0) + (PD > 2 ? stream_frag_cnt(LQ, 2) : 0) +
                                    (PD > 3 ? stream_frag_cnt(LQ, 3) : 0));
            static_assert(PD <= 4, "prefetch depth");
            stream_wait_vm<up>();
        }
        int64_t raw;
        {
            const int g = min(first + lane, A.batch_n - 1), l = (g - first) >> 1;
            raw = reinterpret_cast<const int64_t*>(lds + L.idx)[2 * l + (g - max(min(first + 2 * l, A.batch_n - 2), 0))];
        }
        const int pix = (int)(raw < 0 ? 0 : (raw >= A.npix ? A.npix - 1 : raw));
        const float* rsrc[4];
#pragma unroll
        for (int v = 0; v < 4; ++v) rsrc[v] = F.rows + (size_t)__shfl(pix, 16 * v + (lane >> 2)) * RPM + 4 * (lane & 3);
        auto issue_rows = [&](int s) {
#pragma unroll
            for (int g = 2 * s; g < 2 * s + 2; ++g)
                if (g < NGR)
#pragma unroll
                    for (int v = 0; v < 4; ++v) stream_dma(rsrc[v] + 16 * g, lds0 + 4u * (unsigned)(L.x + v * WPX + g * SGP));
        };
        stream_for<PD>([&](auto s_) { if (decltype(s_)::value < NST) issue_rows(decltype(s_)::value); });
        auto issue_small = [&](int k) {
            constexpr int nsw = 2 * NH, per = (nsw + PD - 1) / PD;
            const int b = k + PD - NST;
#pragma unroll
            for (int u = 0; u < per; ++u) {
                const int j = b * per + u;
                if (j < NH) stream_dma(F.packed + p.pk_wh + lane * 4 + 256 * j, lds0 + 4u * (unsigned)(L.wh + 256 * j));
                else if (j < nsw) stream_dma(F.packed + p.pk_wht + lane * 4 + 256 * (j - NH), lds0 + 4u * (unsigned)(L.wht + 256 * (j - NH)));
            }
        };
        stream_for<NST>([&](auto s_) {
            constexpr int s = decltype(s_)::value;
            stream_wait_vm<stream_allow(LQ, NL, PD, s)>();
            stream_barrier();
            if (s + PD < NST) { issue_rows(s + PD); issue_frags(s + PD); }
            else if (SMALL) issue_small(s);
        });
        stream_wait_vm<0>();
        stream_barrier();
        if (A.next_n > 0) {
            const long long t = F.perm[A.batch_n + min(first + lane, A.next_n - 1)];
            const int touch_bytes = min(A.touch_row_bytes, RPM * 4);
            if (touch_bytes > 0) {
                const int pn = (int)(t < 0 ? 0 : (t >= A.npix ? A.npix - 1 : t));
                const float* rn = F.rows + (size_t)pn * RPM;
                float acc = 0.f;
#pragma unroll
                for (int k = 0; k < 7; ++k) acc += rn[min(128 * k, touch_bytes - 4) / 4];
                asm volatile("" ::"v"(acc));
            } else {
                asm volatile("" ::"v"(t));
            }
        }
        return;
    }
#ifdef LBDRN_TRAIN_STAMPS
    unsigned long long stamp[16] = {};
    asm volatile("s_memrealtime %0\n\ts_waitcnt lgkmcnt(0)" : "=s"(stamp[14])::"memory");
#endif
#ifdef LBDRN_TIMELINE
    if (lane == 0 && w == 0 && wg == 0 && blockIdx.y == 0) timeline_store(A.tl, 0, false);
#endif
    SE(0);

    f32x4 bias[NL][4];
#pragma unroll
    for (int l = 0; l < NL; ++l)
#pragma unroll
        for (int t = 0; t < 4; ++t) {
            const float4 b4 = *reinterpret_cast<const float4*>(F.params + p.offB[l] + 16 * t + 4 * q);
            bias[l][t][0] = b4.x; bias[l][t][1] = b4.y; bias[l][t][2] = b4.z; bias[l][t][3] = b4.w;
        }
    f32x4 bias_last;
#pragma unroll
    for (int r = 0; r < 4; ++r) bias_last[r] = (4 * q + r) < C ? F.params[p.offB[NL] + 4 * q + r] : 0.0f;
    SE(1);

    const __amdgpu_buffer_rsrc_t wrs = __builtin_amdgcn_make_buffer_rsrc(const_cast<float*>(F.packed), (short)0,
                                                                         p.pack_floats * 4, 0x00020000);
    const int lane16 = lane * 16;
    auto ldw = [&](int float_base, int block) -> float4 {
        const v4i32 x = __builtin_amdgcn_raw_buffer_load_b128(wrs, lane16, float_base * 4 + block * 1024, 0);
        return make_float4(__int_as_float(x[0]), __int_as_float(x[1]), __int_as_float(x[2]), __int_as_float(x[3]));
    };
    float4 wh[NL > 1 ? NL - 1 : 1][4][4];
    float4 wl[4];
    float4 wlt[4];
    float4 wht[NL > 1 ? NL - 1 : 1][4][4];
    auto vg_load = [&](int j) {
        constexpr int NHV = SMALL ? 0 : NH;
        if (j < NHV) wh[j / 16][(j >> 2) & 3][j & 3] = ldw(p.pk_wh, j);
        else if (j < 2 * NHV) { const int k = j - NHV; wht[k / 16][(k >> 2) & 3][k & 3] = ldw(p.pk_wht, k); }
        else if (j < 2 * NHV + 4) wl[j - 2 * NHV] = ldw(p.pk_wl, j - 2 * NHV);
        else if (j < 2 * NHV + 8) wlt[j - 2 * NHV - 4] = ldw(p.pk_wlt, j - 2 * NHV - 4);
    };

    f32x4 acc[4];
#pragma unroll
    for (int t = 0; t < 4; ++t) acc[t] = bias[0][t];
    {
        const float* wbase = ST + lane * 4;
        const float* xbase = Xs + w * WPX + (i * 4 + q) * 4;
        float4 aq[2][4], bq[2];
        auto reads = [&](int g) {
#pragma unroll
            for (int t = 0; t < 4; ++t) aq[g & 1][t] = *reinterpret_cast<const float4*>(wbase + (g * 4 + t) * 256);
            bq[g & 1] = *reinterpret_cast<const float4*>(xbase + g * SGP);
        };
        auto mfmas = [&](int g) {
            const float bx[4] = {bq[g & 1].x, bq[g & 1].y, bq[g & 1].z, bq[g & 1].w};
#pragma unroll
            for (int e = 0; e < 4; ++e)
#pragma unroll
                for (int t = 0; t < 4; ++t) {
                    const float4 x = aq[g & 1][t];
                    acc[t] = MFMA16(e == 0 ? x.x : e == 1 ? x.y : e == 2 ? x.z : x.w, bx[e], acc[t]);
                }
        };
        int vgj = 0;
        stream_for<NST>([&](auto s_) {
            constexpr int s = decltype(s_)::value;
            stream_barrier();
#ifdef LBDRN_TRAIN_STAMPS
            if (s == 0) { SE(1); SE(2); }
#endif
#pragma unroll
            for (int u = 0; u < stream_vg(LQ, NL, s); ++u) vg_load(vgj + u);
            vgj += stream_vg(LQ, NL, s);
            __builtin_amdgcn_sched_barrier(0);
#pragma unroll
            for (int g = 2 * s; g < 2 * s + 2; ++g)
                if (g < G0) {
                    reads(g);
                    if (g > 0) {
                        mfmas(g - 1);
#pragma unroll
                        for (int k = 0; k < 5; ++k) {
                            __builtin_amdgcn_sched_group_barrier(0x100, 1, 0);
                            __builtin_amdgcn_sched_group_barrier(0x008, 2, 0);
                        }
                        __builtin_amdgcn_sched_group_barrier(0x008, 6, 0);
                    }
                    __builtin_amdgcn_sched_barrier(0);
                }
        });
        mfmas(G0 - 1);
        __builtin_amdgcn_sched_barrier(0);
    }
    SE(3);
    float h[4][4];
    f32x4 cs[NL][4];
    auto activate_tile = [&](int l, int t) {
#pragma unroll
        for (int r = 0; r < 4; ++r) {
            float sn, co;
            train_act<ACT>(acc[t][r], sn, co);
            h[t][r] = sn;
            cs[l][t][r] = co;
        }
        *reinterpret_cast<float4*>(Hl(l) + srow * HP + 16 * w + 16 * t + 4 * q) = make_float4(h[t][0], h[t][1], h[t][2], h[t][3]);
    };
    auto activate = [&](int l) {
#pragma unroll
        for (int t = 0; t < 4; ++t) activate_tile(l, t);
    };
    activate_tile(0, 0);
    activate_tile(0, 1);
    __builtin_amdgcn_sched_barrier(0);
    stream_barrier();
    SE(4);
    if constexpr (SMALL) {
#pragma unroll
        for (int l = 1; l < NL; ++l)
#pragma unroll
            for (int j = 0; j < 16; ++j)
                wh[l - 1][j >> 2][j & 3] = *reinterpret_cast<const float4*>(lds + L.wh + ((l - 1) * 16 + j) * 256 + lane * 4);
    }
    activate_tile(0, 2);
    activate_tile(0, 3);
    SE(5);

#pragma unroll
    for (int l = 1; l < NL; ++l) {
#pragma unroll
        for (int t = 0; t < 4; ++t) acc[t] = bias[l][t];
#pragma unroll
        for (int tk = 0; tk < 4; ++tk) {
#pragma unroll
            for (int r = 0; r < 4; ++r)
#pragma unroll
                for (int to = 0; to < 4; ++to) {
                    const float4 x = wh[l - 1][to][tk];
                    const float a = r == 0 ? x.x : r == 1 ? x.y : r == 2 ? x.z : x.w;
                    acc[to] = MFMA16(a, h[tk][r], acc[to]);
                }
        }
        if constexpr (SMALL) {
            if (l == NL - 1) {
                asm volatile("s_waitcnt lgkmcnt(0)" ::: "memory");
                stream_barrier();
            }
        }
        activate(l);
    }
    if constexpr (SMALL) {
#pragma unroll
        for (int l = 1; l < NL; ++l)
#pragma unroll
            for (int j = 0; j < 16; ++j)
                wht[l - 1][j >> 2][j & 3] = *reinterpret_cast<const float4*>(lds + L.wht + ((l - 1) * 16 + j) * 256 + lane * 4);
    }
    SE(6);

    float dzo[4];
    {
        f32x4 oe = bias_last, oo = {0.f, 0.f, 0.f, 0.f};
#pragma unroll
        for (int tk = 0; tk < 4; ++tk) {
            const float4 x = wl[tk];
            oe = MFMA16(x.x, h[tk][0], oe);
            oo = MFMA16(x.y, h[tk][1], oo);
            oe = MFMA16(x.z, h[tk][2], oe);
            oo = MFMA16(x.w, h[tk][3], oo);
        }
        const bool live = srow < nvalid;
        const float4 lab = *reinterpret_cast<const float4*>(Xs + w * WPX + G0 * SGP + (i * 4 + q) * 4);
        const float labv[4] = {lab.x, lab.y, lab.z, lab.w};
        float lsum = 0.0f;
#pragma unroll
        for (int r = 0; r < 4; ++r) {
            const bool ok = live && (4 * q + r) < C;
            const float y = train_sigmoid(oe[r] + oo[r]);
            const float d = y - ((4 * q + r) < C ? labv[r] : 0.0f);
            lsum += ok ? d * d : 0.0f;
            dzo[r] = ok ? ((2.0f * d) * A.inv) * (y * (1.0f - y)) : 0.0f;
        }
        *reinterpret_cast<float4*>(Zo + srow * OP + 16 * w + 4 * q) = make_float4(dzo[0], dzo[1], dzo[2], dzo[3]);
        {
            const int li = __float_as_int(stream_sum8(lsum));
            auto rl = [&](int l) { return __int_as_float(__builtin_amdgcn_readlane(li, l)); };
            const float l0 = (rl(14) + rl(30)) + (rl(46) + rl(62)), l1 = (rl(15) + rl(31)) + (rl(47) + rl(63));
            if (lane == 0) { red[w] = l0; red[4 + w] = l1; }
        }
        float bs[4];
#pragma unroll
        for (int r = 0; r < 4; ++r) bs[r] = stream_sum8(dzo[r]);
        if (i >= 14) *reinterpret_cast<float4*>(red + 8 + 64 * (i - 14) + 16 * w + 4 * q) = make_float4(bs[0], bs[1], bs[2], bs[3]);
    }
    SE(7);

    float dz[4][4];
    auto backprop = [&](int l) {
#pragma unroll
        for (int t = 0; t < 4; ++t)
#pragma unroll
            for (int r = 0; r < 4; ++r) {
                dz[t][r] = train_act_back<ACT>(acc[t][r], cs[l][t][r]);
                ZT[(size_t)l * SZTSZ + (16 * t + 4 * q + r) * PT + srow] = dz[t][r];
            }
    };
    {
        const f32x4 zero = {0.f, 0.f, 0.f, 0.f};
#pragma unroll
        for (int t = 0; t < 4; ++t) acc[t] = zero;
#pragma unroll
        for (int s = 0; s < 4; ++s)
#pragma unroll
            for (int t = 0; t < 4; ++t) {
                const float4 x = wlt[t];
                const float a = s == 0 ? x.x : s == 1 ? x.y : s == 2 ? x.z : x.w;
                acc[t] = MFMA16(a, dzo[s], acc[t]);
            }
        backprop(NL - 1);
    }
    auto ldrow = [&](const float* row, float (&dst)[16]) {
#pragma unroll
        for (int g = 0; g < 4; ++g) {
            const float4 x = *reinterpret_cast<const float4*>(row + 4 * g);
            dst[4 * g] = x.x; dst[4 * g + 1] = x.y; dst[4 * g + 2] = x.z; dst[4 * g + 3] = x.w;
        }
    };
    auto ldx = [&](int nt, float (&dst)[16]) {
        const int f = 16 * nt + i;
        const int kq = f / LQ, fl = f - kq * LQ;
        const float* base = Xs + q * WPX + (fl >> 2) * SGP + kq * 4 + (fl & 3);
#pragma unroll
        for (int s = 0; s < 16; ++s) dst[s] = base[16 * s];
    };
    auto ldh = [&](const float* H, int strip, float (&dst)[16]) {
        const float* base = H + (16 * q) * HP + 16 * q + 16 * strip + i;
#pragma unroll
        for (int s = 0; s < 16; ++s) dst[s] = base[s * HP];
    };
    auto put = [&](int off, const f32x4& g, bool early) {
        if (early) slabw.store(off + lane * 4, g[0], g[1], g[2], g[3]);
        else slabw.store_plain(off + lane * 4, g[0], g[1], g[2], g[3]);
    };
    const f32x4 zero4 = {0.f, 0.f, 0.f, 0.f};
    if constexpr (NT0C > 0) {
        static_assert(NL == 2, "the straight-line schedule is written for two hidden layers");
        constexpr int NFS = NT0C / 4, REM = NT0C % 4;
        static_assert(NFS >= 1 && NFS <= 4 && REM <= 2, "strip counts of the shapes this is instantiated for");
        constexpr int NIT = NFS + REM;
        const float* ZT1 = ZT + SZTSZ;
        __syncthreads();
        float ao[16], bo[16], bh[16], a1[4][16];
        {
            const float* base = Zo + (16 * q) * OP + 16 * q + i;
#pragma unroll
            for (int s = 0; s < 16; ++s) ao[s] = base[s * OP];
        }
        ldh(Hl(1), w, bo);
        ldh(Hl(0), w, bh);
        ldrow(ZT1 + (0 + i) * PT + 16 * q, a1[0]);
        ldrow(ZT1 + (16 + i) * PT + 16 * q, a1[1]);
        {
            const f32x4 zero = {0.f, 0.f, 0.f, 0.f};
#pragma unroll
            for (int t = 0; t < 4; ++t) acc[t] = zero;
#pragma unroll
            for (int to = 0; to < 4; ++to)
#pragma unroll
                for (int r = 0; r < 4; ++r)
#pragma unroll
                    for (int ti = 0; ti < 4; ++ti) {
                        const float4 x = wht[0][ti][to];
                        const float a = r == 0 ? x.x : r == 1 ? x.y : r == 2 ? x.z : x.w;
                        acc[ti] = MFMA16(a, dz[to][r], acc[ti]);
                    }
            stream_deal<64, 56, 0>();
            backprop(0);
        }
        SE(8);
        __syncthreads();
        if (tid == 0) F.loss_part[wg] = (((double)red[0] + (double)red[1]) + ((double)red[2] + (double)red[3])) +
                                        (((double)red[4] + (double)red[5]) + ((double)red[6] + (double)red[7]));
        SE(9);
        float az[4][16], azw[16], a1w[16], bb[NFS][16], br[REM > 0 ? REM : 1][16];
        auto item = [&](auto n_) {
            constexpr int n = decltype(n_)::value;
            if constexpr (n < NFS) ldx(w + 4 * n, bb[n]);
            else if constexpr (n < NIT) ldx(4 * NFS + (n - NFS), br[n - NFS]);
        };
        ldrow(ZT1 + (32 + i) * PT + 16 * q, a1[2]);
        ldrow(ZT1 + (48 + i) * PT + 16 * q, a1[3]);
#pragma unroll
        for (int t = 0; t < 4; ++t) ldrow(ZT + (16 * t + i) * PT + 16 * q, az[t]);
        item(std::integral_constant<int, 0>{});
        f32x4 go[2] = {zero4, zero4}, g1[4][2] = {{zero4, zero4}, {zero4, zero4}, {zero4, zero4}, {zero4, zero4}};
#pragma unroll
        for (int s = 0; s < 16; ++s) {
            go[s & 1] = MFMA16(ao[s], bo[s], go[s & 1]);
            g1[0][s & 1] = MFMA16(a1[0][s], bh[s], g1[0][s & 1]);
            g1[1][s & 1] = MFMA16(a1[1][s], bh[s], g1[1][s & 1]);
        }
        stream_deal<48, 40, 0>();
        item(std::integral_constant<int, 1>{});
        ldrow(ZT + (16 * w + i) * PT + 16 * q, azw);
        ldrow(ZT1 + (16 * w + i) * PT + 16 * q, a1w);
#pragma unroll
        for (int s = 0; s < 16; ++s) {
            g1[2][s & 1] = MFMA16(a1[2][s], bh[s], g1[2][s & 1]);
            g1[3][s & 1] = MFMA16(a1[3][s], bh[s], g1[3][s & 1]);
        }
        put(p.sl_out + w * 256, stream_join(go[0], go[1]), true);
        put(p.sl_hid + (0 * 4 + w) * 256, stream_join(g1[0][0], g1[0][1]), true);
        put(p.sl_hid + (1 * 4 + w) * 256, stream_join(g1[1][0], g1[1][1]), true);
        stream_deal<32, (NIT > 1 ? 24 : 8), 3>();
        SD(1);
        f32x4 gs[2][4][2];
        stream_for<NFS>([&](auto k_) {
            constexpr int k = decltype(k_)::value;
#pragma unroll
            for (int t = 0; t < 4; ++t) gs[k & 1][t][0] = gs[k & 1][t][1] = zero4;
            constexpr int nreads = k + 2 < NIT ? 16 : 0;
            item(std::integral_constant<int, k + 2>{});
#pragma unroll
            for (int s = 0; s < 16; ++s)
#pragma unroll
                for (int t = 0; t < 4; ++t) gs[k & 1][t][s & 1] = MFMA16(az[t][s], bb[k][s], gs[k & 1][t][s & 1]);
            if constexpr (k == 0) {
                put(p.sl_hid + (2 * 4 + w) * 256, stream_join(g1[2][0], g1[2][1]), true);
                put(p.sl_hid + (3 * 4 + w) * 256, stream_join(g1[3][0], g1[3][1]), true);
                stream_deal<64, nreads, 2>();
            } else {
#pragma unroll
                for (int t = 0; t < 4; ++t)
                    put((t * NT0C + w + 4 * (k - 1)) * 256, stream_join(gs[(k - 1) & 1][t][0], gs[(k - 1) & 1][t][1]), k - 1 < NFS - TAIL_PLAIN);
                stream_deal<64, nreads, 4>();
            }
#ifdef LBDRN_STAMP_DW
            if (k == 0) { SD(2); stamp[3] = stamp[2]; } else if (k == 1) { SD(4); stamp[5] = stamp[4]; } else if (k == 2) { SD(6); stamp[7] = stamp[6]; }
#endif
        });
        f32x4 grem[REM > 0 ? REM : 1][2];
#pragma unroll
        for (int r = 0; r < (REM > 0 ? REM : 1); ++r) grem[r][0] = grem[r][1] = zero4;
        if constexpr (REM > 0) {
#pragma unroll
            for (int s = 0; s < 16; ++s)
#pragma unroll
                for (int r = 0; r < REM; ++r) grem[r][s & 1] = MFMA16(azw[s], br[r][s], grem[r][s & 1]);
        }
#pragma unroll
        for (int t = 0; t < 4; ++t)
            put((t * NT0C + w + 4 * (NFS - 1)) * 256, stream_join(gs[(NFS - 1) & 1][t][0], gs[(NFS - 1) & 1][t][1]), false);
        stream_deal<REM * 16, 0, 4>();
        {
            float s0[2] = {0.f, 0.f}, s1[2] = {0.f, 0.f};
#pragma unroll
            for (int s = 0; s < 16; ++s) { s0[s & 1] += azw[s]; s1[s & 1] += a1w[s]; }
#pragma unroll
            for (int h = 0; h < 2; ++h) {
                s0[h] += __shfl_xor(s0[h], 16); s1[h] += __shfl_xor(s1[h], 16);
                s0[h] += __shfl_xor(s0[h], 32); s1[h] += __shfl_xor(s1[h], 32);
            }
            if (lane < 16) {
                slab[p.sl_bias + 16 * w + lane] = s0[0] + s0[1];
                slab[p.sl_bias + TBC_W + 16 * w + lane] = s1[0] + s1[1];
            }
        }
        if constexpr (REM > 0) {
#pragma unroll
            for (int r = 0; r < REM; ++r) put((w * NT0C + 4 * NFS + r) * 256, stream_join(grem[r][0], grem[r][1]), false);
        }
#ifdef LBDRN_STAMP_DW
        SD(8); stamp[9] = stamp[8];
#endif
        STAMP(10); STAMP(11);
        if (w == 3 && lane < 16)
            slab[p.sl_bias + NL * TBC_W + lane] = ((red[8 + lane] + red[24 + lane]) + (red[40 + lane] + red[56 + lane])) +
                                                  ((red[72 + lane] + red[88 + lane]) + (red[104 + lane] + red[120 + lane]));
    } else {
    #pragma unroll
        for (int l = NL - 1; l >= 1; --l) {
            const f32x4 zero = {0.f, 0.f, 0.f, 0.f};
    #pragma unroll
            for (int t = 0; t < 4; ++t) acc[t] = zero;
    #pragma unroll
            for (int to = 0; to < 4; ++to)
    #pragma unroll
                for (int r = 0; r < 4; ++r)
    #pragma unroll
                    for (int ti = 0; ti < 4; ++ti) {
                        const float4 x = wht[l - 1][ti][to];
                        const float a = r == 0 ? x.x : r == 1 ? x.y : r == 2 ? x.z : x.w;
                        acc[ti] = MFMA16(a, dz[to][r], acc[ti]);
                    }
            backprop(l - 1);
        }
        SE(8);
        __syncthreads();
        if (tid == 0) F.loss_part[wg] = (((double)red[0] + (double)red[1]) + ((double)red[2] + (double)red[3])) +
                                        (((double)red[4] + (double)red[5]) + ((double)red[6] + (double)red[7]));
        SE(9);

        const int NT0 = p.NT0, NF = NT0 & ~3, rem = NT0 - NF;
        float az[4][16], b[16], bn[16];
    #pragma unroll
        for (int t = 0; t < 4; ++t) ldrow(ZT + (16 * t + i) * PT + 16 * q, az[t]);
        ldx(min(w, NT0 - 1), b);
        __builtin_amdgcn_sched_barrier(0);
        SD(1);
        [[maybe_unused]] int strips_done = 0;
        auto strip = [&](int nt, int nreads) {
            f32x4 g[4] = {zero4, zero4, zero4, zero4};
    #pragma unroll
            for (int s = 0; s < 16; ++s)
    #pragma unroll
                for (int t = 0; t < 4; ++t) g[t] = MFMA16(az[t][s], b[s], g[t]);
            if (nreads <= 16) {
    #pragma unroll
                for (int k = 0; k < 16; ++k) {
                    __builtin_amdgcn_sched_group_barrier(0x008, 3, 0);
                    __builtin_amdgcn_sched_group_barrier(0x100, 1, 0);
                }
                __builtin_amdgcn_sched_group_barrier(0x008, 16, 0);
            } else {
    #pragma unroll
                for (int k = 0; k < 52; ++k) {
                    __builtin_amdgcn_sched_group_barrier(0x008, 1, 0);
                    __builtin_amdgcn_sched_group_barrier(0x100, 1, 0);
                }
                __builtin_amdgcn_sched_group_barrier(0x008, 12, 0);
            }
            __builtin_amdgcn_sched_barrier(0);
    #ifdef LBDRN_STAMP_DW
            if (strips_done == 0) SD(2); else if (strips_done == 1) SD(4); else SD(6);
    #endif
    #pragma unroll
            for (int t = 0; t < 4; ++t) put((t * NT0 + nt) * 256, g[t], true);
    #ifdef LBDRN_STAMP_DW
            if (strips_done == 0) SD(3); else if (strips_done == 1) SD(5); else { SD(7); stamp[8] = stamp[7]; stamp[9] = stamp[7]; }
    #endif
            ++strips_done;
        };
        int nt = w;
        for (; nt + 4 < NF; nt += 4) {
            ldx(nt + 4, bn);
            strip(nt, 16);
    #pragma unroll
            for (int s = 0; s < 16; ++s) b[s] = bn[s];
        }
        float azw[16], ao[16], bo[16], br[16];
        ldrow(ZT + (16 * w + i) * PT + 16 * q, azw);
        {
            const float* base = Zo + (16 * q) * OP + 16 * q + i;
    #pragma unroll
            for (int s = 0; s < 16; ++s) ao[s] = base[s * OP];
        }
        ldh(Hl(NL - 1), w, bo);
        ldx(min(NF, NT0 - 1), br);
        if (nt < NF) strip(nt, 52);
        __builtin_amdgcn_sched_barrier(0);
        STAMP(10);
        float a1[NL > 1 ? NL - 1 : 1][4][16], bh[NL > 1 ? NL - 1 : 1][16];
    #pragma unroll
        for (int l = 1; l < NL; ++l) {
    #pragma unroll
            for (int t = 0; t < 4; ++t) ldrow(ZT + (size_t)l * SZTSZ + (16 * t + i) * PT + 16 * q, a1[l - 1][t]);
            ldh(Hl(l - 1), w, bh[l - 1]);
        }
        {
            f32x4 go = zero4, g0 = zero4;
    #pragma unroll
            for (int s = 0; s < 16; ++s) {
                go = MFMA16(ao[s], bo[s], go);
                g0 = MFMA16(azw[s], br[s], g0);
            }
    #pragma unroll
            for (int k = 0; k < 32; ++k) {
                __builtin_amdgcn_sched_group_barrier(0x008, 1, 0);
                __builtin_amdgcn_sched_group_barrier(0x100, 1, 0);
            }
            __builtin_amdgcn_sched_barrier(0);
            put(p.sl_out + w * 256, go, false);
            if (rem >= 1) put((w * NT0 + NF) * 256, g0, false);
        }
        for (int k = 1; k < rem; ++k) {
            ldx(NF + k, br);
            f32x4 g1 = zero4;
    #pragma unroll
            for (int s = 0; s < 16; ++s) g1 = MFMA16(azw[s], br[s], g1);
            put((w * NT0 + NF + k) * 256, g1, false);
        }
    #pragma unroll
        for (int l = 1; l < NL; ++l) {
            f32x4 g[4] = {zero4, zero4, zero4, zero4};
    #pragma unroll
            for (int s = 0; s < 16; ++s)
    #pragma unroll
                for (int t = 0; t < 4; ++t) g[t] = MFMA16(a1[l - 1][t][s], bh[l - 1][s], g[t]);
            __builtin_amdgcn_sched_barrier(0);
    #pragma unroll
            for (int t = 0; t < 4; ++t) put(p.sl_hid + ((l - 1) * 16 + t * 4 + w) * 256, g[t], false);
        }
        STAMP(11);
        if (tid < NL * TBC_W * 2) {
            const int u = tid >> 1, half = tid & 1;
            const float* row = ZT + (size_t)(u >> 6) * SZTSZ + (u & 63) * PT + 32 * half;
            float s0 = 0.f, s1 = 0.f, s2 = 0.f, s3 = 0.f;
    #pragma unroll
            for (int g = 0; g < 8; ++g) {
                const float4 x = *reinterpret_cast<const float4*>(row + 4 * g);
                s0 += x.x; s1 += x.y; s2 += x.z; s3 += x.w;
            }
            const float mine = (s0 + s1) + (s2 + s3);
            const float other = __shfl_xor(mine, 1);
            if (half == 0) slab[p.sl_bias + u] = mine + other;
        }
        if (w == 3 && lane < 16)
            slab[p.sl_bias + NL * TBC_W + lane] = ((red[8 + lane] + red[24 + lane]) + (red[40 + lane] + red[56 + lane])) +
                                                  ((red[72 + lane] + red[88 + lane]) + (red[104 + lane] + red[120 + lane]));
    }
    STAMP(12);
#ifdef LBDRN_TIMELINE
    if (lane == 0 && blockIdx.y == 0) timeline_store(A.tl, 2 + wg * 4 + w, true);
#endif
#ifdef LBDRN_TRAIN_STAMPS
    asm volatile("s_waitcnt vmcnt(0)" ::: "memory");
    STAMP(13);
    asm volatile("s_memrealtime %0\n\ts_waitcnt lgkmcnt(0)" : "=s"(stamp[15])::"memory");
    if (lane == 0 && A.stamps)
        for (int k = 0; k < 16; ++k) A.stamps[(((size_t)blockIdx.y * gridDim.x + wg) * 4 + w) * 16 + k] = stamp[k];
#endif
}
```

### lbdrn-msic_amd/lbdrn_hip/_lib.py

```python
import ctypes
import os

_HERE = os.path.dirname(os.path.abspath(__file__))
_LIB_PATH = os.environ.get("LBDRN_HIP_LIB") or os.path.join(os.path.dirname(_HERE), "liblbdrn_hip.so")

ABI_VERSION = 2
PATH_AUTO, PATH_GENERIC, PATH_MFMA = 0, 1, 2
EVAL_BACKGROUND = 0x200
EVAL_FAST = 0x400
EVAL_X16 = 0x1000
TRAIN_ALONE = 0x800


class LbdrnError(RuntimeError):
    code = None


E_ARG, E_DEVICE, E_UNSUPPORTED, E_WORKSPACE = -1, -2, -3, -4


class Geom(ctypes.Structure):
    _fields_ = [("C", ctypes.c_int32), ("H", ctypes.c_int32), ("W", ctypes.c_int32),
                ("K", ctypes.c_int32), ("D", ctypes.c_int32), ("msb_max", ctypes.c_int32),
                ("use_colors", ctypes.c_int32), ("relative", ctypes.c_int32),
                ("P", ctypes.c_int32), ("reserved", ctypes.c_int32),
                ("rowtab", ctypes.c_void_p), ("coltab", ctypes.c_void_p)]


class Net(ctypes.Structure):
    _fields_ = [("F", ctypes.c_int32), ("bc", ctypes.c_int32), ("C", ctypes.c_int32),
                ("nl", ctypes.c_int32), ("act", ctypes.c_int32)]


_vp, _i32, _i64, _sz, _dbl = (ctypes.c_void_p, ctypes.c_int32, ctypes.c_int64, ctypes.c_size_t,
                              ctypes.c_double)
_GP, _NP = ctypes.POINTER(Geom), ctypes.POINTER(Net)
SIGNATURES = {
    "lbdrn_last_error": (ctypes.c_char_p, []),
    "lbdrn_abi_version": (ctypes.c_int, []),
    "lbdrn_device_check": (ctypes.c_int, []),
    "lbdrn_param_count": (_i64, [_NP]),
    "lbdrn_feature_dim": (_i32, [_GP]),
    "lbdrn_split_bits": (ctypes.c_int, [_vp, _i32, _i32, _i32, _i32, _vp, _vp, _vp]),
    "lbdrn_labels": (ctypes.c_int, [_vp, _i32, _i32, _i32, _i32, _vp, _i64, _vp, _vp]),
    "lbdrn_features": (ctypes.c_int, [_GP, _vp, _vp, _i64, _vp, _vp]),
    "lbdrn_forward_workspace": (_sz, [_NP, _i64]),
    "lbdrn_forward": (ctypes.c_int, [_NP, _vp, _vp, _i64, _vp, _vp, _sz, _vp]),
    "lbdrn_tape_bytes": (_sz, [_NP, _i64]),
    "lbdrn_forward_tape": (ctypes.c_int, [_NP, _vp, _vp, _i64, _vp, _vp, _sz, _vp]),
    "lbdrn_backward_workspace": (_sz, [_NP, _i64]),
    "lbdrn_backward": (ctypes.c_int, [_NP, _vp, _vp, _i64, _vp, _sz, _vp, _vp, _vp, _vp, _vp, _sz, _vp]),
    "lbdrn_apply_workspace": (_sz, [_GP, _NP]),
    "lbdrn_decode_fused": (ctypes.c_int, [_GP, _NP, _vp, _vp, _vp, _vp, _vp, _sz, _i32, _vp]),
    "lbdrn_eval_sse": (ctypes.c_int, [_GP, _NP, _vp, _vp, _vp, _vp, _vp, _sz, _i32, _vp]),
    "lbdrn_train_workspace": (_sz, [_GP, _NP, _i32]),
    "lbdrn_train_prepare": (ctypes.c_int, [_GP, _NP, _vp, _vp, _i32, _vp, _sz, _i32, _vp]),
    "lbdrn_train_epoch": (ctypes.c_int, [_GP, _NP, _vp, _vp, _vp, _i64, _i32, _vp, _vp, _vp, _i64,
                                         _dbl, _vp, _vp, _sz, _i32, _vp]),
    "lbdrn_train_group_max": (ctypes.c_int, []),
    "lbdrn_train_step_features": (_i32, [_GP, _NP]),
    "lbdrn_train_group_size": (_i32, [_GP, _NP]),
    "lbdrn_train_epoch_group": (ctypes.c_int, [_i32, _vp, _NP, _vp, _vp, _vp, _i64, _i32, _vp, _vp, _vp, _i64, _dbl, _vp,
                                               _vp, _sz, _i32, _vp]),
    "lbdrn_train_profile_mode": (ctypes.c_int, [_i32]),
    "lbdrn_randperm_workspace": (_sz, [_i64, _i32]),
    "lbdrn_randperm": (ctypes.c_int, [ctypes.POINTER(ctypes.c_uint64), _i32, _i64, _vp, _vp, _sz, _vp]),
    "lbdrn_mt19937_jump_poly": (_i64, [_i32, _vp]),
    "lbdrn_plane_bound": (_sz, [_i32, _i32, _i32]),
    "lbdrn_plane_workspace": (_sz, [_i32, _i32, _i32]),
    "lbdrn_plane_encode": (ctypes.c_int, [_vp, _i32, _i32, _i32, _vp, _sz, _vp, _vp, _sz, _vp]),
    "lbdrn_plane_decode": (ctypes.c_int, [_vp, _sz, _i32, _i32, _i32, _vp, _vp, _vp, _sz, _vp]),
    "lbdrn_jp2k_block_count": (_i64, [_i32, _i32, _i32]),
    "lbdrn_jp2k_bound": (_sz, [_i32, _i32, _i32]),
    "lbdrn_jp2k_workspace": (_sz, [_i32, _i32, _i32]),
    "lbdrn_jp2k_encode": (ctypes.c_int, [_vp, _i32, _i32, _i32, _i32, _vp, _sz, ctypes.POINTER(ctypes.c_size_t), _vp, _sz, _vp]),
    "lbdrn_weights_bound": (_sz, [_i64]),
    "lbdrn_weights_encode": (ctypes.c_int, [_vp, _i64, _i32, _vp, _sz, ctypes.POINTER(ctypes.c_size_t)]),
    "lbdrn_weights_info": (ctypes.c_int, [_vp, _sz, ctypes.POINTER(_i64), ctypes.POINTER(_i32)]),
    "lbdrn_weights_decode": (ctypes.c_int, [_vp, _sz, _vp, _i64]),
    "lbdrn_train_step": (ctypes.c_int, [_NP, _vp, _vp, _i32, _vp, _vp, _vp, _i64, _dbl, _i32, _vp,
                                        _vp, _vp, _sz, _vp]),
}

_lib = None


def lib_path():
    return _LIB_PATH


def lib():
    global _lib
    if _lib is not None:
        return _lib
    if not os.path.exists(_LIB_PATH):
        raise LbdrnError(
            f"{_LIB_PATH} is missing: build it with `python lbdrn-msic_amd/csrc/build.py` "
            "(hipcc, gfx950).  This package has no CPU fallback.")
    import torch
    L = ctypes.CDLL(_LIB_PATH)
    for name, (res, args) in SIGNATURES.items():
        fn = getattr(L, name)
        fn.restype = res
        fn.argtypes = args
    if L.lbdrn_abi_version() != ABI_VERSION:
        raise LbdrnError(f"liblbdrn_hip ABI {L.lbdrn_abi_version()} != {ABI_VERSION}")
    _lib = L
    return L


def check(rc):
    if rc != 0:
        msg = lib().lbdrn_last_error()
        err = LbdrnError(f"liblbdrn_hip error {rc}: {msg.decode() if msg else ''}")
        err.code = rc
        raise err
```

### lbdrn-msic_amd/lbdrn_hip/ops.py

```python
import ctypes

import numpy as np
import torch

from . import _lib
from ._lib import EVAL_BACKGROUND, EVAL_FAST, EVAL_X16, TRAIN_ALONE, Geom, Net, PATH_AUTO, check, lib


def _call(fn, ref, *args):
    dev = ref.device if isinstance(ref, torch.Tensor) else torch.device(ref)
    if dev.type != "cuda":
        raise _lib.LbdrnError("liblbdrn_hip works on device (HBM) tensors only; there is no CPU path in this package")
    with torch.cuda.device(dev):
        check(fn(*args, ctypes.c_void_p(torch.cuda.current_stream(dev).cuda_stream)))


def _ptr(t):
    return ctypes.c_void_p(t.data_ptr()) if t is not None else None


def _need_cuda(*ts):
    for t in ts:
        if t is not None and not t.is_cuda:
            raise _lib.LbdrnError("liblbdrn_hip works on device (HBM) tensors only; there is no "
                                  "CPU path in this package")


def _u16(t):
    if t.dtype == torch.uint16:
        return t.view(torch.int16)
    assert t.dtype == torch.int16, t.dtype
    return t


class FeatureGeometry:

    def __init__(self, C, H, W, K, D, msb_max, cfg, device):
        from .features import pos_tables
        self.C, self.H, self.W, self.K, self.D, self.msb_max = C, H, W, K, D, int(msb_max)
        self.cfg = cfg
        rowtab, coltab = pos_tables(H, W, cfg)
        self.P = rowtab.shape[1]
        self.rowtab = torch.from_numpy(rowtab).to(device) if self.P else None
        self.coltab = torch.from_numpy(coltab).to(device) if self.P else None
        self.F = cfg.feature_dim(C, D)
        self.c = Geom(C, H, W, K, D, int(msb_max), int(cfg.use_colors), int(cfg.relative), self.P,
                      0, self.rowtab.data_ptr() if self.P else None,
                      self.coltab.data_ptr() if self.P else None)

    def with_max(self, msb_max):
        self.msb_max = int(msb_max)
        self.c.msb_max = int(msb_max)
        return self


ACT_SINE, ACT_RELU = 0, 1


def make_net(F, bc, C, nl, act=ACT_SINE):
    return Net(F, bc, C, nl, act)


def param_count(net):
    return int(lib().lbdrn_param_count(ctypes.byref(net)))


def split_bits(img, K):
    _need_cuda(img)
    img = _u16(img.contiguous())
    C, H, W = img.shape
    msb = torch.empty_like(img)
    mx = torch.zeros(1, dtype=torch.int32, device=img.device)
    _call(lib().lbdrn_split_bits, img, _ptr(img), C, H, W, K, _ptr(msb), _ptr(mx))
    return msb, int(mx.item())


def labels(img, K, idx=None):
    _need_cuda(img, idx)
    img = _u16(img.contiguous())
    C, H, W = img.shape
    n = H * W if idx is None else idx.numel()
    out = torch.empty((n, C), dtype=torch.float32, device=img.device)
    if idx is not None:
        idx = idx.to(torch.int64).contiguous()
    _call(lib().lbdrn_labels, img, _ptr(img), C, H, W, K, _ptr(idx), n, _ptr(out))
    return out


def features(geom, msb, idx=None):
    _need_cuda(msb, idx)
    msb = _u16(msb.contiguous())
    n = geom.H * geom.W if idx is None else idx.numel()
    out = torch.empty((n, geom.F), dtype=torch.float32, device=msb.device)
    if idx is not None:
        idx = idx.to(torch.int64).contiguous()
    _call(lib().lbdrn_features, msb, ctypes.byref(geom.c), _ptr(msb), _ptr(idx), n, _ptr(out))
    return out


def forward(net, params, x):
    _need_cuda(params, x)
    x = x.contiguous().float()
    params = params.contiguous().float()
    B = x.shape[0]
    assert x.shape[1] == net.F and params.numel() == param_count(net)
    y = torch.empty((B, net.C), dtype=torch.float32, device=x.device)
    nbytes = lib().lbdrn_forward_workspace(ctypes.byref(net), B)
    ws = torch.empty(max(nbytes, 1), dtype=torch.uint8, device=x.device)
    _call(lib().lbdrn_forward, x, ctypes.byref(net), _ptr(params), _ptr(x), B, _ptr(y), _ptr(ws), nbytes)
    return y


def forward_tape(net, params, x):
    _need_cuda(params, x)
    x = x.contiguous().float()
    params = params.contiguous().float()
    B = x.shape[0]
    assert x.shape[1] == net.F and params.numel() == param_count(net)
    y = torch.empty((B, net.C), dtype=torch.float32, device=x.device)
    nbytes = lib().lbdrn_tape_bytes(ctypes.byref(net), B)
    tape = torch.empty(max(nbytes, 1), dtype=torch.uint8, device=x.device)
    _call(lib().lbdrn_forward_tape, x, ctypes.byref(net), _ptr(params), _ptr(x), B, _ptr(y), _ptr(tape), nbytes)
    return y, tape


def backward(net, params, x, tape, y, dy, want_dx=False):
    _need_cuda(params, x, tape, y, dy)
    x = x.contiguous().float()
    params = params.contiguous().float()
    dy = dy.contiguous().float()
    B = x.shape[0]
    assert x.shape[1] == net.F and params.numel() == param_count(net)
    assert y.shape == (B, net.C) and dy.shape == (B, net.C) and y.is_contiguous()
    grads = torch.empty(param_count(net), dtype=torch.float32, device=x.device)
    dx = torch.empty((B, net.F), dtype=torch.float32, device=x.device) if want_dx else None
    nbytes = lib().lbdrn_backward_workspace(ctypes.byref(net), B)
    ws = torch.empty(max(nbytes, 1), dtype=torch.uint8, device=x.device)
    _call(lib().lbdrn_backward, x, ctypes.byref(net), _ptr(params), _ptr(x), B, _ptr(tape), tape.numel(), _ptr(y),
          _ptr(dy), _ptr(grads), _ptr(dx), _ptr(ws), nbytes)
    return grads, dx


class ApplyWorkspace:
    def __init__(self, geom, net, device):
        self.nbytes = lib().lbdrn_apply_workspace(ctypes.byref(geom.c), ctypes.byref(net))
        self.buf = torch.empty(max(self.nbytes, 1), dtype=torch.uint8, device=device)


def decode_fused(geom, net, msb, params, want_y=False, path=PATH_AUTO, ws=None):
    _need_cuda(msb, params)
    msb = _u16(msb.contiguous())
    params = params.contiguous().float()
    out = torch.empty_like(msb)
    y = torch.empty((geom.H * geom.W, geom.C), dtype=torch.float32, device=msb.device) if want_y else None
    ws = ws or ApplyWorkspace(geom, net, msb.device)
    _call(lib().lbdrn_decode_fused, msb, ctypes.byref(geom.c), ctypes.byref(net), _ptr(msb), _ptr(params),
                                   _ptr(out), _ptr(y), _ptr(ws.buf), ws.nbytes, path)
    return (out, y) if want_y else out


def eval_sse(geom, net, img, msb, params, path=PATH_AUTO, ws=None, out=None, background=False, fast=False, x16=False):
    _need_cuda(img, msb, params)
    img = _u16(img.contiguous())
    msb = _u16(msb.contiguous())
    params = params.contiguous().float()
    sse = out if out is not None else torch.zeros(1, dtype=torch.float64, device=msb.device)
    ws = ws or ApplyWorkspace(geom, net, msb.device)
    _call(lib().lbdrn_eval_sse, msb, ctypes.byref(geom.c), ctypes.byref(net), _ptr(img), _ptr(msb),
                               _ptr(params), _ptr(sse), _ptr(ws.buf), ws.nbytes,
                               path | (EVAL_BACKGROUND if background else 0) | (EVAL_FAST if fast else 0) |
                               (EVAL_X16 if (fast and x16) else 0))
    return sse


class TrainWorkspace:

    def __init__(self, geom, net, batch_size, device):
        self.geom, self.net, self.batch_size = geom, net, batch_size
        self.nbytes = lib().lbdrn_train_workspace(ctypes.byref(geom.c), ctypes.byref(net), batch_size)
        self.buf = torch.empty(max(self.nbytes, 1), dtype=torch.uint8, device=device)
        self.prepared_for = None

    def prepare(self, img, msb, path=PATH_AUTO):
        img, msb = _u16(img.contiguous()), _u16(msb.contiguous())
        _call(lib().lbdrn_train_prepare, img, ctypes.byref(self.geom.c), ctypes.byref(self.net), _ptr(img),
                                        _ptr(msb), self.batch_size, _ptr(self.buf), self.nbytes, path)
        self.prepared_for = (img.data_ptr(), path)
        return self


def train_epoch(geom, net, img, msb, perm, batch_size, params, exp_avg, exp_avg_sq, adam_step0, lr,
                losses=None, path=PATH_AUTO, ws=None, alone=False):
    _need_cuda(img, msb, perm, params, exp_avg, exp_avg_sq, losses)
    img = _u16(img.contiguous())
    msb = _u16(msb.contiguous())
    assert perm.dtype == torch.int64 and perm.is_contiguous()
    for t in (params, exp_avg, exp_avg_sq):
        assert t.dtype == torch.float32 and t.is_contiguous()
    if ws is None:
        ws = TrainWorkspace(geom, net, batch_size, img.device).prepare(img, msb, path)
    if ws.prepared_for != (img.data_ptr(), path):
        raise _lib.LbdrnError("TrainWorkspace.prepare(img, msb, path) must run once for this image first")
    _call(lib().lbdrn_train_epoch, img, ctypes.byref(geom.c), ctypes.byref(net), _ptr(img), _ptr(msb),
                                  _ptr(perm), perm.numel(), batch_size, _ptr(params), _ptr(exp_avg),
                                  _ptr(exp_avg_sq), adam_step0, float(lr), _ptr(losses), _ptr(ws.buf),
                                  ws.nbytes, path | (TRAIN_ALONE if alone else 0))


def train_group_max():
    return int(lib().lbdrn_train_group_max())


def train_group_size(C, H, W, K, D, cfg, base_channel, num_layers):
    g = Geom(C, H, W, K, D, 1, int(cfg.use_colors), int(cfg.relative), int(cfg.P), 0, None, None)
    net = Net(cfg.feature_dim(C, D), base_channel, C, num_layers, cfg.act)
    return int(lib().lbdrn_train_group_size(ctypes.byref(g), ctypes.byref(net)))


def train_step_features(geom, net):
    return int(lib().lbdrn_train_step_features(ctypes.byref(geom.c), ctypes.byref(net)))


def train_epoch_group(geoms, net, imgs, msbs, perms, batch_size, params, exp_avgs, exp_avg_sqs, adam_step0, lr,
                      losses=None, path=PATH_AUTO, wss=None):
    n = len(imgs)
    _need_cuda(*imgs, *msbs, *perms, *params, *exp_avgs, *exp_avg_sqs)
    imgs = [_u16(t.contiguous()) for t in imgs]
    msbs = [_u16(t.contiguous()) for t in msbs]
    for t in perms:
        assert t.dtype == torch.int64 and t.is_contiguous() and t.numel() == perms[0].numel()
    for t in list(params) + list(exp_avgs) + list(exp_avg_sqs):
        assert t.dtype == torch.float32 and t.is_contiguous()
    for ws, img in zip(wss, imgs):
        if ws.prepared_for != (img.data_ptr(), path) or ws.nbytes != wss[0].nbytes:
            raise _lib.LbdrnError("every fit of a group needs its own TrainWorkspace, prepared for its image")
    arr = lambda ptrs: (ctypes.c_void_p * n)(*ptrs)
    garr = (ctypes.POINTER(Geom) * n)(*[ctypes.pointer(g.c) for g in geoms])
    larr = arr([_ptr(t) for t in losses]) if losses is not None else None
    _call(lib().lbdrn_train_epoch_group, imgs[0], n, ctypes.cast(garr, ctypes.c_void_p), ctypes.byref(net),
          arr([_ptr(t) for t in imgs]), arr([_ptr(t) for t in msbs]), arr([_ptr(t) for t in perms]),
          perms[0].numel(), batch_size, arr([_ptr(t) for t in params]), arr([_ptr(t) for t in exp_avgs]),
          arr([_ptr(t) for t in exp_avg_sqs]), adam_step0, float(lr), larr, arr([_ptr(w.buf) for w in wss]),
          wss[0].nbytes, path)


def train_profile_mode(mode):
    check(lib().lbdrn_train_profile_mode(int(mode)))


def train_step(net, x, t, params, exp_avg, exp_avg_sq, adam_step, lr, apply_adam=True):
    _need_cuda(x, t, params)
    x = x.contiguous().float()
    t = t.contiguous().float()
    B = x.shape[0]
    loss = torch.zeros(1, dtype=torch.float32, device=x.device)
    grads = torch.empty_like(params)
    g = Geom(net.C, 1, 1, 1, 0, 1, 1, 1, 0, 0, None, None)
    nbytes = lib().lbdrn_train_workspace(ctypes.byref(g), ctypes.byref(net), B)
    ws = torch.empty(max(nbytes, 1), dtype=torch.uint8, device=x.device)
    _call(lib().lbdrn_train_step, x, ctypes.byref(net), _ptr(x), _ptr(t), B, _ptr(params), _ptr(exp_avg),
                                 _ptr(exp_avg_sq), adam_step, float(lr), int(apply_adam), _ptr(loss),
                                 _ptr(grads), _ptr(ws), nbytes)
    return loss, grads


def randperm(seeds, n, device):
    scalar = isinstance(seeds, int)
    seeds = [seeds] if scalar else list(seeds)
    out = torch.empty((len(seeds), n), dtype=torch.int64, device=device)
    for c0 in range(0, len(seeds), 32):
        chunk = seeds[c0:c0 + 32]
        arr = (ctypes.c_uint64 * len(chunk))(*[s & 0xFFFFFFFFFFFFFFFF for s in chunk])
        nbytes = lib().lbdrn_randperm_workspace(n, len(chunk))
        ws = torch.empty(max(nbytes, 1), dtype=torch.uint8, device=device)
        _call(lib().lbdrn_randperm, out, arr, len(chunk), n, _ptr(out[c0:]), _ptr(ws), nbytes)
    return out[0] if scalar else out


def plane_encode(planes):
    _need_cuda(planes)
    planes = _u16(planes.contiguous())
    C, H, W = planes.shape
    dev = planes.device
    body = torch.empty(lib().lbdrn_plane_bound(C, H, W), dtype=torch.uint8, device=dev)
    nbytes = torch.zeros(1, dtype=torch.int64, device=dev)
    ws = torch.empty(max(lib().lbdrn_plane_workspace(C, H, W), 1), dtype=torch.uint8, device=dev)
    _call(lib().lbdrn_plane_encode, planes, _ptr(planes), C, H, W, _ptr(body), body.numel(), _ptr(nbytes), _ptr(ws),
                                   ws.numel())
    return body[:int(nbytes.item())].cpu().numpy().tobytes()


def jp2k_encode(planes, bits, out=None):
    _need_cuda(planes)
    planes = _u16(planes.contiguous())
    C, H, W = planes.shape
    dev = planes.device
    cap = lib().lbdrn_jp2k_bound(C, H, W)
    if not cap:
        raise _lib.LbdrnError(f"lbdrn_jp2k_encode: geometry {C} x {H} x {W} is not supported")
    if out is None:
        out = np.empty(cap, np.uint8)
    n = ctypes.c_size_t()
    ws = torch.empty(max(lib().lbdrn_jp2k_workspace(C, H, W), 1), dtype=torch.uint8, device=dev)
    _call(lib().lbdrn_jp2k_encode, planes, _ptr(planes), C, H, W, int(bits), out.ctypes.data_as(ctypes.c_void_p), out.size,
                                  ctypes.byref(n), _ptr(ws), ws.numel())
    return out[:n.value].tobytes()


def plane_decode(body, C, H, W, device):
    raw = torch.frombuffer(bytearray(body), dtype=torch.uint8).to(device)
    planes = torch.empty((C, H, W), dtype=torch.int16, device=device)
    status = torch.zeros(1, dtype=torch.int32, device=device)
    ws = torch.empty(max(lib().lbdrn_plane_workspace(C, H, W), 1), dtype=torch.uint8, device=device)
    _call(lib().lbdrn_plane_decode, planes, _ptr(raw), raw.numel(), C, H, W, _ptr(planes), _ptr(status), _ptr(ws),
                                   ws.numel())
    if int(status.item()):
        raise _lib.LbdrnError("LBB2 payload is inconsistent with its geometry (corrupt or truncated stream)")
    return planes


def to_device_u16(arr, device):
    a = np.ascontiguousarray(arr, dtype=np.uint16)
    return torch.from_numpy(a.view(np.int16)).to(device)


def from_device_u16(t):
    return t.cpu().numpy().view(np.uint16)
```

Baseline: 69.37 Mpixels/s.

## Pre-gather minibatch rows into a staging ring and piggyback gather on reduce launch

Adds a row-staging kernel that gathers the permuted feature rows of the next minibatch into a 4-slot contiguous staging ring. The gather blocks are appended as extra blocks to the reduce/Adam launch, so staging step i+1 overlaps with the reduction of step i. The train kernels (split and stream variants) now read contiguous staged rows instead of loading perm indices into LDS, waiting on them, and doing scattered row gathers. The old next-batch cache-touch prefetch is removed. This costs an extra copy of each minibatch and more workspace, and it makes the reduce launch larger.

```diff
diff --git a/include/lbdrn_hip.h b/include/lbdrn_hip.h
--- a/include/lbdrn_hip.h
+++ b/include/lbdrn_hip.h
@@ -83,6 +83,8 @@
                    size_t workspace_bytes, int32_t path, void *stream);
 
 size_t lbdrn_train_workspace(const lbdrn_geom *g, const lbdrn_net *net, int32_t batch_size);
+size_t lbdrn_train_stage_bytes(const lbdrn_geom *g, const lbdrn_net *net, int32_t batch_size, size_t *offset,
+                               int32_t *slots);
 #define LBDRN_TRAIN_ALONE 0x800
 int lbdrn_train_prepare(const lbdrn_geom *g, const lbdrn_net *net, const uint16_t *img,
                         const uint16_t *msb, int32_t batch_size, void *workspace,
diff --git a/lbdrn-msic_amd/csrc/cabi.hip b/lbdrn-msic_amd/csrc/cabi.hip
--- a/lbdrn-msic_amd/csrc/cabi.hip
+++ b/lbdrn-msic_amd/csrc/cabi.hip
@@ -8,6 +8,7 @@
 int mfma_train_step_features(const lbdrn_geom& g, const lbdrn_net& net);
 bool mfma_train_takes_groups(const lbdrn_geom& g, const lbdrn_net& net);
 size_t mfma_train_workspace(const lbdrn_geom& g, const lbdrn_net& net, int bs);
+size_t mfma_train_stage_ring(const lbdrn_geom& g, const lbdrn_net& net, int bs, size_t* offset, int* slots);
 int mfma_train_prepare(const lbdrn_geom& g, const lbdrn_net& net, const uint16_t* img,
                        const uint16_t* msb, int bs, void* ws, size_t ws_bytes, hipStream_t s);
 int mfma_train_epoch(const lbdrn_geom& g, const lbdrn_net& net, const uint16_t* img,
@@ -251,6 +252,15 @@
     return a > b ? a : b;
 }
 
+size_t lbdrn_train_stage_bytes(const lbdrn_geom* g, const lbdrn_net* net, int32_t batch_size, size_t* offset, int32_t* slots)
+{
+    if (check_geom(g) || check_net(net) || batch_size < 1) return 0;
+    int n = 0;
+    const size_t bytes = mfma_train_stage_ring(*g, *net, batch_size, offset, &n);
+    if (bytes && slots) *slots = n;
+    return bytes;
+}
+
 int lbdrn_train_prepare(const lbdrn_geom* g, const lbdrn_net* net, const uint16_t* img,
                         const uint16_t* msb, int32_t batch_size, void* workspace, size_t workspace_bytes,
                         int32_t path, void* stream)
diff --git a/lbdrn-msic_amd/csrc/train_mfma.hip b/lbdrn-msic_amd/csrc/train_mfma.hip
--- a/lbdrn-msic_amd/csrc/train_mfma.hip
+++ b/lbdrn-msic_amd/csrc/train_mfma.hip
@@ -20,6 +20,9 @@
 constexpr int RED_SLICES = 8;
 constexpr int RED_LANES = 32;
 constexpr int SLAB_ROT = 4;
+constexpr int STAGE_ROT = 4;
+constexpr int STAGE_THREADS = 256, STAGE_ROWS = STAGE_THREADS / 16;
+constexpr int STAGE_MAX_BLOCKS = 1024;
 constexpr int TRAIN_THREADS = 512;
 
 constexpr int WB = 64;
@@ -168,7 +171,7 @@
 
 
 struct TrainWsLayout {
-    size_t off_rows, off_pack, off_slab, slab_bytes, off_loss, off_stage, stage_bytes, off_map, total;
+    size_t off_rows, off_pack, off_slab, slab_bytes, off_loss, off_stage, stage_bytes, stage_rows, off_map, total;
 };
 
 static TrainWsLayout train_ws_layout(const lbdrn_geom& g, const lbdrn_net& net, const TrainPlan& p, int bs)
@@ -177,12 +180,13 @@
     size_t o = 0;
     L.off_rows = o; o += align_up((size_t)g.H * g.W * p.RP * sizeof(float), 256);
     L.off_pack = o; o += align_up((size_t)p.pack_floats * sizeof(float), 256);
-    const size_t nwg = std::max((size_t)(bs + TB - 1) / TB, 2 * ((size_t)(bs + WB - 1) / WB));
+    const size_t nwg = std::max(((size_t)bs + TB - 1) / TB, 2 * (((size_t)bs + WB - 1) / WB));
     L.slab_bytes = align_up(nwg * (size_t)p.slab_floats * sizeof(float), 256);
     L.off_slab = o; o += SLAB_ROT * L.slab_bytes;
     L.off_loss = o; o += align_up(nwg * sizeof(double), 256);
-    L.stage_bytes = align_up(align_up((size_t)bs, WB) * p.RP * sizeof(float), 256);
-    L.off_stage = o; o += 2 * L.stage_bytes;
+    L.stage_rows = align_up(std::min((size_t)std::max(bs, 0), (size_t)g.H * g.W), WB);
+    L.stage_bytes = align_up(L.stage_rows * p.RP * sizeof(float), 256);
+    L.off_stage = o; o += STAGE_ROT * L.stage_bytes;
     L.off_map = o; o += align_up((size_t)p.slab_floats * 4 * sizeof(int), 256);
     L.total = o;
     return L;
@@ -190,7 +194,7 @@
 
 static bool slabs_addressable(const TrainPlan& p, int bs)
 {
-    const size_t nwg = std::max((size_t)(bs + TB - 1) / TB, 2 * ((size_t)(bs + WB - 1) / WB));
+    const size_t nwg = std::max(((size_t)bs + TB - 1) / TB, 2 * (((size_t)bs + WB - 1) / WB));
     return nwg * (size_t)p.slab_floats * sizeof(float) < ((size_t)1 << 31);
 }
 
@@ -199,6 +203,16 @@
     TrainPlan p;
     if (!make_train_plan(g, net, &p)) return wide_workspace(g, net, bs);
     return train_ws_layout(g, net, p, bs).total;
+}
+
+size_t mfma_train_stage_ring(const lbdrn_geom& g, const lbdrn_net& net, int bs, size_t* offset, int* slots)
+{
+    TrainPlan p;
+    if (!make_train_plan(g, net, &p) || !p.wave || !slabs_addressable(p, bs)) return 0;
+    const TrainWsLayout L = train_ws_layout(g, net, p, bs);
+    if (offset) *offset = L.off_stage;
+    if (slots) *slots = STAGE_ROT;
+    return L.stage_bytes;
 }
 
 
@@ -430,6 +444,43 @@
     tl[slot] = t;
 }
 #endif
+struct StageFit {
+    const float* rows;
+    const int64_t* perm;
+    float* dst;
+};
+struct StageArgs {
+    StageFit fit[MAX_GROUP];
+    int64_t npix;
+    int n;
+    int r4;
+    int blocks;
+};
+__device__ __forceinline__ void stage_rows_block(const StageArgs& S, const StageFit& F, int blk)
+{
+    const int sub = threadIdx.x >> 4, l = threadIdx.x & 15;
+    for (int row = blk * STAGE_ROWS + sub; row < S.n; row += S.blocks * STAGE_ROWS) {
+        const int64_t raw = F.perm[row];
+        const int64_t pix = raw < 0 ? 0 : (raw >= S.npix ? S.npix - 1 : raw);
+        const float4* __restrict__ src = reinterpret_cast<const float4*>(F.rows) + (size_t)pix * S.r4;
+        float4* __restrict__ dst = reinterpret_cast<float4*>(F.dst) + (size_t)row * S.r4;
+        for (int c = l; c < S.r4; c += 64) {
+            float4 t[4];
+#pragma unroll
+            for (int k = 0; k < 4; ++k)
+                if (c + 16 * k < S.r4) t[k] = src[c + 16 * k];
+#pragma unroll
+            for (int k = 0; k < 4; ++k)
+                if (c + 16 * k < S.r4) dst[c + 16 * k] = t[k];
+        }
+    }
+}
+__global__ void __launch_bounds__(STAGE_THREADS) k_stage_rows(StageArgs S)
+{
+    stage_rows_block(S, S.fit[blockIdx.y], blockIdx.x);
+}
+static int stage_blocks_for(int n) { return std::min((n + STAGE_ROWS - 1) / STAGE_ROWS, STAGE_MAX_BLOCKS); }
+
 struct ReduceFit {
     const float* slabs;
     float *params, *m, *v, *packed;
@@ -440,6 +491,8 @@
     ReduceFit fit[MAX_GROUP];
     unsigned long long* tl;
     int nloss;
+    int red_blocks;
+    StageArgs S;
 };
 
 __global__ void __launch_bounds__(RED_SLICES * RED_LANES)
@@ -448,6 +501,10 @@
 {
     __shared__ __attribute__((aligned(16))) float part[RED_SLICES][4 * RED_LANES];
     __builtin_amdgcn_s_setprio(3);
+    if ((int)blockIdx.x >= R.red_blocks) {
+        stage_rows_block(R.S, R.S.fit[blockIdx.y], (int)blockIdx.x - R.red_blocks);
+        return;
+    }
 #ifdef LBDRN_TIMELINE
     if (threadIdx.x == 0 && blockIdx.x == 0 && blockIdx.y == 0) timeline_store(R.tl, 1, false);
 #endif
@@ -537,13 +594,16 @@
 static void launch_reduce(const ReduceArgs& R, int blocks, int count, bool pairs, int nwg, int slab_floats, const int4* map,
                           float step_size, float bc2_sqrt, double loss_count, hipStream_t s)
 {
-    k_reduce_adam<<<dim3((unsigned)blocks, (unsigned)count), RED_SLICES * RED_LANES, 0, s>>>(R, nwg, slab_floats, map, step_size, bc2_sqrt,
+    static_assert(STAGE_THREADS == RED_SLICES * RED_LANES, "staging blocks ride on the reduce launch");
+    const int extra = R.S.n > 0 ? R.S.blocks : 0;
+    k_reduce_adam<<<dim3((unsigned)(blocks + extra), (unsigned)count), RED_SLICES * RED_LANES, 0, s>>>(R, nwg, slab_floats, map, step_size, bc2_sqrt,
                                                                                             loss_count, pairs ? 1 : 0);
 }
 
 
 struct TrainFit {
     const float* rows;
+    const float* stage;
     const int64_t* perm;
     const float* params;
     const float* packed;
@@ -561,12 +621,9 @@
     float* stage_out;
     const int64_t* perm_next;
     int next_n;
-    int touch_row_bytes;
     unsigned long long* stamps;
     unsigned long long* tl;
 };
-constexpr int TOUCH_ROW_BYTES = 256;
-
 
 #ifdef LBDRN_TRAIN_STAMPS
 #define STAMP(k)                                                                        \
@@ -1170,12 +1227,20 @@
         return LBDRN_E_WORKSPACE;
     }
     A.net = net; A.npix = (int64_t)g.H * g.W;
+    if ((size_t)std::min<int64_t>(bs, n) > L.stage_rows) {
+        set_error("minibatch of %lld rows: more than the image has pixels", (long long)std::min<int64_t>(bs, n));
+        return LBDRN_E_UNSUPPORTED;
+    }
     ReduceArgs R;
+    R.red_blocks = A.p.slab_floats / (4 * RED_LANES);
+    R.S.npix = A.npix; R.S.n = 0; R.S.r4 = A.p.RP / 4; R.S.blocks = 1;
     for (int f = 0; f < MAX_GROUP; ++f) {
         const int k = f < count ? f : 0;
         if (!ws[k]) { set_error("null train workspace"); return LBDRN_E_WORKSPACE; }
         float* packed = (float*)((char*)ws[k] + L.off_pack);
         A.fit[f].rows = (float*)((char*)ws[k] + L.off_rows);
+        A.fit[f].stage = nullptr;
+        R.S.fit[f].rows = A.fit[f].rows; R.S.fit[f].perm = perm[k]; R.S.fit[f].dst = nullptr;
         A.fit[f].params = params[k];
         A.fit[f].packed = packed;
         A.fit[f].slabs = (float*)((char*)ws[k] + L.off_slab);
@@ -1193,6 +1258,24 @@
     k_build_map<<<(unsigned)((A.p.slab_floats + 255) / 256), 256, 0, s>>>(A.p, net.F, net.nl, net.C, map);
     LBDRN_LAUNCH_CHECK();
     float* stage[2] = {(float*)((char*)ws[0] + L.off_stage), (float*)((char*)ws[0] + L.off_stage + L.stage_bytes)};
+    auto stage_target = [&](int64_t first, int slot) {
+        for (int f = 0; f < MAX_GROUP; ++f) {
+            const int k = f < count ? f : 0;
+            R.S.fit[f].perm = perm[k] + first;
+            R.S.fit[f].dst = (float*)((char*)ws[k] + L.off_stage + (size_t)slot * L.stage_bytes);
+        }
+        R.S.n = first < n ? (int)std::min<int64_t>(bs, n - first) : 0;
+        R.S.blocks = stage_blocks_for(R.S.n);
+    };
+    auto stage_launch = [&]() {
+        if (R.S.n > 0) k_stage_rows<<<dim3((unsigned)R.S.blocks, (unsigned)count), STAGE_THREADS, 0, s>>>(R.S);
+    };
+    const bool no_reduce = g_prof_mode == 3 || g_prof_mode == 4;
+    if (A.p.wave && n > 0) {
+        stage_target(0, 0);
+        stage_launch();
+        LBDRN_LAUNCH_CHECK();
+    }
     A.stamps = nullptr;
 #ifdef LBDRN_TRAIN_STAMPS
     const int max_wg = (bs + TB - 1) / TB;
@@ -1225,6 +1308,15 @@
             const int k = f < count ? f : 0;
             A.fit[f].slabs = (float*)((char*)ws[k] + L.off_slab + (size_t)(si % SLAB_ROT) * L.slab_bytes);
             R.fit[f].slabs = A.fit[f].slabs;
+            A.fit[f].stage = (const float*)((char*)ws[k] + L.off_stage + (size_t)(si % STAGE_ROT) * L.stage_bytes);
+        }
+        if (A.p.wave) {
+            if (no_reduce) {
+                if (si > 0 && si < STAGE_ROT) { stage_target(first, si); stage_launch(); }
+                R.S.n = 0;
+            } else {
+                stage_target(first + bs, (si + 1) % STAGE_ROT);
+            }
         }
 #ifdef LBDRN_TIMELINE
         A.tl = tl_buf + (size_t)TL_SLOTS * si; R.tl = A.tl;
@@ -1236,7 +1328,6 @@
         if (A.p.wave) A.stage_in = nullptr, A.stage_out = nullptr;
         A.perm_next = perm[0] + first + bs;
         A.next_n = (int)nextB;
-        A.touch_row_bytes = (alone && count == 1) ? TOUCH_ROW_BYTES : 0;
         const bool split_now = split && (B >= 2 || split_only(A.p));
         auto train_launch = [&]() { return split_now ? dispatch_split(A, 2 * nwg, count, s) : dispatch_train(A, nwg, count, s); };
         if (int rc = train_launch()) return rc;
@@ -1245,7 +1336,7 @@
         ++step;
         const double bc1 = 1.0 - std::pow(0.9, (double)step), bc2 = 1.0 - std::pow(0.999, (double)step);
         R.nloss = split_now ? 2 * nwg : nwg;
-        if (g_prof_mode != 3 && g_prof_mode != 4)
+        if (!no_reduce)
                 launch_reduce(R, red_blocks, count, split_now, nwg, A.p.slab_floats, map, (float)(lr / bc1), (float)std::sqrt(bc2), (double)B * net.C, s);
         if (g_prof_mode == 1) {
             ReduceArgs R0 = R;
@@ -1299,7 +1390,7 @@
         else
         fprintf(stderr, A.p.wave == 2 ?
                         "[lbdrn stamps, stream kernel] clock %.0f MHz; wave lifetime %.0f cycles; first start -> last end %.2f us; "
-                        "mean cycles: indices + first requests out %.0f | first stage landed %.0f | layer 0 under the stream %.0f | all landed, barrier %.0f | "
+                        "mean cycles: first requests out %.0f | first stage landed %.0f | layer 0 under the stream %.0f | all landed, barrier %.0f | "
                         "act0 %.0f | hidden+act %.0f | out+loss %.0f | backward %.0f | barrier 3 %.0f | dW0 strips %.0f | dW tail+hidden %.0f | "
                         "bias sums %.0f | drain %.0f\n" :
                         "[lbdrn stamps, wave kernel] clock %.0f MHz; wave lifetime %.0f cycles; first start -> last end %.2f us; "
diff --git a/lbdrn-msic_amd/csrc/train_split.inc b/lbdrn-msic_amd/csrc/train_split.inc
--- a/lbdrn-msic_amd/csrc/train_split.inc
+++ b/lbdrn-msic_amd/csrc/train_split.inc
@@ -9,7 +9,7 @@
 __host__ __device__ constexpr int split_w0_groups(int LQ) { return split_ring(LQ) ? SP_RING : LQ / 4; }
 __host__ __device__ constexpr int split_small_through(int k, int SPI) { return k * SPI < SP_SM / 4 ? k * SPI : SP_SM / 4; }
 
-struct SplitLds { int w0, sm, x, xt, h0, red, idx, bias, h1, e, zo, zt, total; };
+struct SplitLds { int w0, sm, x, xt, h0, red, bias, h1, e, zo, zt, total; };
 __host__ __device__ constexpr SplitLds split_lds(int LQ)
 {
     SplitLds L{};
@@ -22,7 +22,6 @@
     L.x = o; o += 2 * L.xt;
     L.h0 = o; o += SPB * SP_HP;
     L.red = o; o += 4 + 4 * 16 + 12;
-    L.idx = o; o += 4 * 256;
     L.bias = o; o += 4 * 64;
     L.total = o;
     int a = L.w0;
@@ -101,17 +100,10 @@
     STAMP(0);
 
     {
-        const void* a0 = F.perm; const void* a1 = F.params; const void* a2 = F.packed; const void* a3 = F.rows;
+        const void* a0 = F.stage; const void* a1 = F.params; const void* a2 = F.packed;
         int b0 = p.pk_w0, b1 = p.pk_wh, b2 = p.pk_wht, b3 = p.pk_wl, b4 = p.pk_wlt, b5 = A.batch_n;
-        long long c0 = p.offB[0], c1 = p.offB[1], c2 = p.offB[2], c3 = A.npix;
-        asm volatile("" ::"s"(a0), "s"(a1), "s"(a2), "s"(a3), "s"(b0), "s"(b1), "s"(b2), "s"(b3), "s"(b4), "s"(b5), "s"(c0), "s"(c1), "s"(c2), "s"(c3));
-    }
-    if constexpr (RING) {
-        const int64_t* isrc = F.perm + min(grp * WB + lane, A.batch_n - 1);
-        stream_dma_dword(reinterpret_cast<const float*>(isrc), lds0 + 4u * (unsigned)(L.idx + 256 * wv));
-    } else {
-        const int64_t* isrc = F.perm + min(grp * WB + 2 * (lane & 31), A.batch_n - 2);
-        stream_dma(reinterpret_cast<const float*>(isrc), lds0 + 4u * (unsigned)(L.idx + 256 * wv));
+        long long c0 = p.offB[0], c1 = p.offB[1], c2 = p.offB[2];
+        asm volatile("" ::"s"(a0), "s"(a1), "s"(a2), "s"(b0), "s"(b1), "s"(b2), "s"(b3), "s"(b4), "s"(b5), "s"(c0), "s"(c1), "s"(c2));
     }
     {
         const int l = wv < 3 ? wv : 2, n = l < 2 ? 64 : C;
@@ -125,17 +117,12 @@
             stream_dma(fsrc + p.pk_w0 + 256 * (wv * G0 + g), lds0 + 4u * (unsigned)(L.w0 + ((g % RG) * 4 + wv) * 256));
     };
     w0_requests(0, GA);
-    stream_wait_vm<GA + 1>();
-    int64_t raw;
-    if constexpr (RING) {
-        raw = reinterpret_cast<const int*>(lds + L.idx + 256 * wv)[min(grow, A.batch_n - 1) - grp * WB];
-    } else {
-        const int g = min(grow, A.batch_n - 1), l = (g - grp * WB) >> 1;
-        const int pos = 2 * l + (g - min(grp * WB + 2 * l, A.batch_n - 2));
-        raw = reinterpret_cast<const int64_t*>(lds + L.idx + 256 * wv)[pos];
-    }
-    const int pix = (int)(raw < 0 ? 0 : (raw >= A.npix ? A.npix - 1 : raw));
-    const float* rsrc = F.rows + (size_t)__shfl(pix, 16 * q + split_slot(lane >> 2)) * RPM + 4 * (lane & 3);
+    const float* rsrc;
+    {
+        const int si = split_slot(lane >> 2);
+        const int srho = 16 * (2 * st + ((si >> 2) & 1)) + 2 * ((si & 3) + 4 * (si >> 3)) + par;
+        rsrc = F.stage + (size_t)min(grp * WB + srho, A.batch_n - 1) * RPM + 4 * (lane & 3);
+    }
     auto row_requests = [&](int g_lo, int g_hi) {
 #pragma unroll
         for (int g = g_lo; g < g_hi; ++g)
@@ -149,8 +136,6 @@
         const int src = blk < 16 ? p.pk_wh + 256 * blk : blk < 32 ? p.pk_wht + 256 * (blk - 16) : blk < 36 ? p.pk_wl + 256 * (blk - 32) : p.pk_wlt + 256 * (blk - 36);
         stream_dma(fsrc + src, lds0 + 4u * (unsigned)(L.sm + 256 * blk));
     };
-    long long touched = 0;
-    if (A.next_n > 0 && wv == 0 && lane < 8) touched = F.perm[A.batch_n + min(grp * WB + 8 * lane, A.next_n - 1)];
     STAMP(1);
     constexpr int ROWS_B0 = split_row_requests(GA, NGR, 0), ROWS_B1 = split_row_requests(GA, NGR, 1);
     if (uh == 0) stream_wait_vm<W0B + ROWS_B0>(); else stream_wait_vm<W0B + ROWS_B1>();
@@ -465,7 +450,6 @@
     }
     if (w == 3 && lane < 16)
         slab[p.sl_bias + NL * TBC_W + lane] = (red[4 + lane] + red[20 + lane]) + (red[36 + lane] + red[52 + lane]);
-    asm volatile("" ::"v"(touched));
     STAMP(11); STAMP(12);
 #ifdef LBDRN_TIMELINE
     if (lane == 0 && uh == 0 && blockIdx.y == 0) timeline_store(A.tl, 2 + 2 * wg + st, true);
diff --git a/lbdrn-msic_amd/csrc/train_stream.inc b/lbdrn-msic_amd/csrc/train_stream.inc
--- a/lbdrn-msic_amd/csrc/train_stream.inc
+++ b/lbdrn-msic_amd/csrc/train_stream.inc
@@ -12,7 +12,7 @@
 constexpr int SZTSZ = TBC_W * WPT;
 
 constexpr int SRED = 8 + 2 * 64;
-struct StreamLds { int x, stage, h0, red, h1, zo, zt, wh, wht, idx, total, small; };
+struct StreamLds { int x, stage, h0, red, h1, zo, zt, wh, wht, total, small; };
 __host__ __device__ constexpr StreamLds stream_lds(int LQ, int NL)
 {
     StreamLds L{};
@@ -40,7 +40,6 @@
     }
     if (alias) { L.h0 = L.stage; L.red = L.stage + SHSZ; }
     else { L.h0 = total; L.red = total + SHSZ; total += SHSZ + SRED; }
-    L.idx = total; total += 256;
     L.total = total;
     return L;
 }
@@ -76,8 +75,7 @@
 {
     const int NST = (LQ / 4 + 2) / 2;
     int total = 0, last = 0;
-    for (int k = 0; k < PD && k < NST; ++k) { total += 4 * stream_frag_cnt(LQ, k); if (k == s) last = total; }
-    for (int k = 0; k < PD && k < NST; ++k) { total += 4 * stream_row_cnt(LQ, k); if (k == s) last = total; }
+    for (int k = 0; k < PD && k < NST; ++k) { total += 4 * stream_frag_cnt(LQ, k) + 4 * stream_row_cnt(LQ, k); if (k == s) last = total; }
     for (int it = 0; it < s; ++it) {
         if (it + PD < NST) {
             total += 4 * stream_row_cnt(LQ, it + PD) + 4 * stream_frag_cnt(LQ, it + PD);
@@ -201,28 +199,9 @@
 #pragma unroll
                     for (int t = 0; t < 4; ++t) stream_dma(fsrc + 256 * (t * G0 + g), lds0 + 4u * (unsigned)(L.stage + (g * 4 + t) * 256));
         };
-        if (A.batch_n >= 2) {
-            const int64_t* isrc = F.perm + min(first + 2 * (lane & 31), A.batch_n - 2);
-            stream_dma(reinterpret_cast<const float*>(isrc), lds0 + 4u * (unsigned)L.idx);
-        } else {
-            stream_dma_dword(reinterpret_cast<const float*>(F.perm) + (lane & 1), lds0 + 4u * (unsigned)L.idx);
-        }
-        stream_for<PD>([&](auto s_) { if (decltype(s_)::value < NST) issue_frags(decltype(s_)::value); });
-        {
-            constexpr int up = 4 * (stream_frag_cnt(LQ, 0) + (PD > 1 ? stream_frag_cnt(LQ, 1) : 0) + (PD > 2 ? stream_frag_cnt(LQ, 2) : 0) +
-                                    (PD > 3 ? stream_frag_cnt(LQ, 3) : 0));
-            static_assert(PD <= 4, "prefetch depth");
-            stream_wait_vm<up>();
-        }
-        int64_t raw;
-        {
-            const int g = min(first + lane, A.batch_n - 1), l = (g - first) >> 1;
-            raw = reinterpret_cast<const int64_t*>(lds + L.idx)[2 * l + (g - max(min(first + 2 * l, A.batch_n - 2), 0))];
-        }
-        const int pix = (int)(raw < 0 ? 0 : (raw >= A.npix ? A.npix - 1 : raw));
         const float* rsrc[4];
 #pragma unroll
-        for (int v = 0; v < 4; ++v) rsrc[v] = F.rows + (size_t)__shfl(pix, 16 * v + (lane >> 2)) * RPM + 4 * (lane & 3);
+        for (int v = 0; v < 4; ++v) rsrc[v] = F.stage + (size_t)min(first + 16 * v + (lane >> 2), A.batch_n - 1) * RPM + 4 * (lane & 3);
         auto issue_rows = [&](int s) {
 #pragma unroll
             for (int g = 2 * s; g < 2 * s + 2; ++g)
@@ -230,7 +209,8 @@
 #pragma unroll
                     for (int v = 0; v < 4; ++v) stream_dma(rsrc[v] + 16 * g, lds0 + 4u * (unsigned)(L.x + v * WPX + g * SGP));
         };
-        stream_for<PD>([&](auto s_) { if (decltype(s_)::value < NST) issue_rows(decltype(s_)::value); });
+        static_assert(PD <= 4, "prefetch depth");
+        stream_for<PD>([&](auto s_) { if (decltype(s_)::value < NST) { issue_frags(decltype(s_)::value); issue_rows(decltype(s_)::value); } });
         auto issue_small = [&](int k) {
             constexpr int nsw = 2 * NH, per = (nsw + PD - 1) / PD;
             const int b = k + PD - NST;
@@ -250,20 +230,6 @@
         });
         stream_wait_vm<0>();
         stream_barrier();
-        if (A.next_n > 0) {
-            const long long t = F.perm[A.batch_n + min(first + lane, A.next_n - 1)];
-            const int touch_bytes = min(A.touch_row_bytes, RPM * 4);
-            if (touch_bytes > 0) {
-                const int pn = (int)(t < 0 ? 0 : (t >= A.npix ? A.npix - 1 : t));
-                const float* rn = F.rows + (size_t)pn * RPM;
-                float acc = 0.f;
-#pragma unroll
-                for (int k = 0; k < 7; ++k) acc += rn[min(128 * k, touch_bytes - 4) / 4];
-                asm volatile("" ::"v"(acc));
-            } else {
-                asm volatile("" ::"v"(t));
-            }
-        }
         return;
     }
 #ifdef LBDRN_TRAIN_STAMPS
diff --git a/lbdrn-msic_amd/lbdrn_hip/_lib.py b/lbdrn-msic_amd/lbdrn_hip/_lib.py
--- a/lbdrn-msic_amd/lbdrn_hip/_lib.py
+++ b/lbdrn-msic_amd/lbdrn_hip/_lib.py
@@ -54,6 +54,7 @@
     "lbdrn_decode_fused": (ctypes.c_int, [_GP, _NP, _vp, _vp, _vp, _vp, _vp, _sz, _i32, _vp]),
     "lbdrn_eval_sse": (ctypes.c_int, [_GP, _NP, _vp, _vp, _vp, _vp, _vp, _sz, _i32, _vp]),
     "lbdrn_train_workspace": (_sz, [_GP, _NP, _i32]),
+    "lbdrn_train_stage_bytes": (_sz, [_GP, _NP, _i32, ctypes.POINTER(ctypes.c_size_t), ctypes.POINTER(_i32)]),
     "lbdrn_train_prepare": (ctypes.c_int, [_GP, _NP, _vp, _vp, _i32, _vp, _sz, _i32, _vp]),
     "lbdrn_train_epoch": (ctypes.c_int, [_GP, _NP, _vp, _vp, _vp, _i64, _i32, _vp, _vp, _vp, _i64,
                                          _dbl, _vp, _vp, _sz, _i32, _vp]),
diff --git a/lbdrn-msic_amd/lbdrn_hip/ops.py b/lbdrn-msic_amd/lbdrn_hip/ops.py
--- a/lbdrn-msic_amd/lbdrn_hip/ops.py
+++ b/lbdrn-msic_amd/lbdrn_hip/ops.py
@@ -187,6 +187,12 @@
                                         _ptr(msb), self.batch_size, _ptr(self.buf), self.nbytes, path)
         self.prepared_for = (img.data_ptr(), path)
         return self
+
+
+def train_stage_ring(geom, net, batch_size):
+    off, slots = ctypes.c_size_t(0), ctypes.c_int32(0)
+    nbytes = lib().lbdrn_train_stage_bytes(ctypes.byref(geom.c), ctypes.byref(net), batch_size, ctypes.byref(off), ctypes.byref(slots))
+    return int(nbytes), int(off.value), int(slots.value)
 
 
 def train_epoch(geom, net, img, msb, perm, batch_size, params, exp_avg, exp_avg_sq, adam_step0, lr,
```

After: 38.53 Mpixels/s. 44.5% lower.
